# alexandrainst/coral

Hardware: AMD Instinct MI355X
Metric: audio-seconds/sec (CTC finetune step: fwd+bwd+allreduce+clip+AdamW), wav2vec2-large, 10 s utterances (higher is better)
Workload: dtype bf16; 1 GPU; wav2vec2-large (XLS-R shape d=1920 L=48 ffn=7680) CTC finetune, 8 x 10 s per GPU, SpecAugment on, activation_dropout 0.1, layerdrop 0 (multi-GPU rule), fp32 master + AdamW + clip 1.0; global_batch=8, frames_per_utt=499, parallelism=dp1

## Files before the change

### coral_amd/_lib.py

```python

from __future__ import annotations

import ctypes as C
import os
from pathlib import Path

_HERE = Path(__file__).resolve().parent
LIB_PATH = _HERE / "libcoral_amd.so"


class CoralAmdError(RuntimeError):
    """Raised when the HIP library is missing or a call into it fails."""


class CaGemmDesc(C.Structure):

    _fields_ = [
        ("A", C.c_void_p),
        ("B", C.c_void_p),
        ("C", C.c_void_p),
        ("C2", C.c_void_p),
        ("R", C.c_void_p),
        ("bias", C.c_void_p),
        ("M", C.c_int32),
# ... 18 lines not shown
        ("sC1", C.c_int64),
        ("sC2", C.c_int64),
        ("sR1", C.c_int64),
        ("sR2", C.c_int64),
        ("sBias1", C.c_int64),
        ("sBias2", C.c_int64),
        ("epilogue", C.c_int32),
        ("out_f32", C.c_int32),
        ("accumulate", C.c_int32),
        ("alpha", C.c_float),
        ("dropout_p", C.c_float),
        ("dropout_seed", C.c_uint64),
        ("a_colsum", C.c_void_p),
        ("a_colsum_ld", C.c_int64),
        ("c_row_index", C.c_void_p),
        ("c_row_mul", C.c_int64),
        ("c_split_n", C.c_int32),
        ("C_hi", C.c_void_p),
        ("ldc_hi", C.c_int64),
        ("a_scale", C.c_void_p),
        ("b_scale", C.c_void_p),
        ("a_row_scale", C.c_void_p),
        ("c_sumsq", C.c_void_p),
        ("c_stream_out", C.c_int32),
        ("C8", C.c_void_p),
        ("c8_scale", C.c_void_p),
        ("c8_amax", C.c_void_p),
        ("a_ln_gamma", C.c_void_p),
        ("a_ln_beta", C.c_void_p),
        ("a_ln_eps", C.c_float),
        ("xcd_balanced", C.c_int32),
    ]


class CaReduceDesc(C.Structure):
    _fields_ = [("partial", C.c_void_p), ("out", C.c_void_p), ("stride", C.c_int64), ("nparts", C.c_int32),
                ("n", C.c_int32), ("accumulate", C.c_int32)]


class CaDecodeLayer(C.Structure):

    FIELDS = ("ln1_g", "ln1_b", "wqkv", "bqkv", "wo", "bo", "ln2_g", "ln2_b", "wq2", "bq2", "wo2", "bo2", "ln3_g", "ln3_b",
              "w1", "b1", "w2", "b2", "self_kv", "cross_kv")
    _fields_ = [(n, C.c_void_p) for n in FIELDS]


class CaDecodeDesc(C.Structure):

    _fields_ = ([("layers", C.c_void_p)]
                + [(n, C.c_int32) for n in ("n_layers", "B", "d", "f", "H", "Te", "max_len", "V")]
                + [(n, C.c_void_p) for n in ("embed", "embed_pos", "lnf_g", "lnf_b")]
                + [("eps", C.c_float), ("logits", C.c_void_p), ("ld_logits", C.c_int64), ("suppress", C.c_void_p),
                   ("out", C.c_void_p), ("done", C.c_void_p), ("ids", C.c_void_p), ("ld_ids", C.c_int64),
                   ("tok", C.c_void_p), ("pos", C.c_void_p), ("klen", C.c_void_p), ("pad_id", C.c_int32),
                   ("eos_id", C.c_int32), ("ws", C.c_void_p), ("ws_bytes", C.c_int64), ("status", C.c_void_p),
                   ("cross_head_major", C.c_int32)])


DECODE_MAX_B = 16


def decode_ws_bytes(B, d, f, H, n_layers):
    return (8192 + n_layers * 16 * H * 4 + 16 * (7 * d + f) * 2 + 16 * H * 4 * 16 * 66 * 4 + 256 * 16 * 8 + 4096)


class CaAttnDesc(C.Structure):

    _fields_ = ([(n, C.c_void_p) for n in ("Q", "K", "V", "O", "dO", "dQ", "dK", "dV", "lse", "Dq", "klen", "key_slot", "kstart")]
                + [(n, C.c_int64) for n in ("ldq", "ldk", "ldv", "ldo", "lddo", "lddq", "lddk", "lddv",
                                             "sqb", "skb", "svb", "sob", "sdob", "sdqb", "sdkb", "sdvb")]
                + [(n, C.c_int32) for n in ("B", "H", "Tq", "Tk", "hd", "Tqp", "causal")]
                + [("scale", C.c_float), ("dropout_p", C.c_float), ("dropout_seed", C.c_uint64)]
                + [("O8", C.c_void_p), ("o8_scale", C.c_void_p), ("o8_amax", C.c_void_p),
                   ("split_ws", C.c_void_p), ("split_ws_bytes", C.c_int64), ("row_off", C.c_void_p)])


class CaFp8RefreshTask(C.Structure):

    _fields_ = ([(n, C.c_void_p) for n in ("x_bf16", "q_fp8", "q_fp8_t", "scale", "amax_next")]
                + [("rows", C.c_int32), ("cols", C.c_int32)])


class CaCtcBeamDesc(C.Structure):

    _fields_ = [("logits", C.c_void_p), ("ldv", C.c_int64), ("in_len", C.c_void_p),
                ("B", C.c_int32), ("T", C.c_int32), ("V", C.c_int32), ("blank", C.c_int32), ("delimiter", C.c_int32),
                ("forbidden", C.c_void_p), ("pfx_keys", C.c_void_p), ("pfx_wid", C.c_void_p), ("n_pfx", C.c_int64),
                ("ng_keys", C.c_void_p), ("ng_logp", C.c_void_p), ("ng_backoff", C.c_void_p),
                ("ng_count", C.c_int64 * 5),
                ("order", C.c_int32), ("bos_wid", C.c_int32), ("eos_wid", C.c_int32), ("unk_wid", C.c_int32),
                ("beam_width", C.c_int32),
                ("alpha", C.c_float), ("beta", C.c_float), ("unk_score_offset", C.c_float),
                ("token_min_logp", C.c_float), ("beam_prune_logp", C.c_float), ("score_boundary", C.c_int32),
                ("ids_out", C.c_void_p), ("out_len", C.c_void_p), ("score_out", C.c_void_p),
                ("ws", C.c_void_p), ("ws_bytes", C.c_int64)]


class CaBeamDesc(C.Structure):

    _fields_ = ([(n, C.c_int32) for n in ("B", "k", "max_len", "prompt_len", "max_length", "eos_id", "early_stopping")]
                + [(n, C.c_void_p) for n in ("len_pen", "cand_score", "cand_parent", "cand_token", "run_score", "tok", "pos",
                                              "klen", "anc_in", "anc_out", "ids_in", "ids_out", "fin_score", "fin_len",
                                              "fin_seq", "fin_ids", "fin_count", "heur", "done", "tr_parent", "tr_token",
                                              "tr_score")])


BEAM_MAX_BEAMS, BEAM_MAX_ROWS = 16, 128
ALIGN_MAX_TOKENS, ALIGN_MAX_FRAMES, ALIGN_MAX_HEADS, ALIGN_MAX_HEAD_DIM, ALIGN_MAX_FILTER_WIDTH = 447, 1500, 32, 128, 31


def align_ws_bytes_per_clip(A, Lw, Fmax):
    return A * Fmax * (Lw + 4) * 4


FP8_GROUP_MAX = 8
CTC_COLLAPSE_TILE = 4096
CTC_ALIGN_MAX_LABELS = 4095
KMAJOR, MNMAJOR = 0, 1
EPI_NONE, EPI_GELU, EPI_RESIDUAL, EPI_DGELU, EPI_GELU_RESIDUAL = 0, 1, 2, 3, 4

_vp, _i32, _i64, _f32, _u64 = C.c_void_p, C.c_int32, C.c_int64, C.c_float, C.c_uint64

SIGNATURES = {
    "ca_version": (C.c_int, []),
    "ca_last_error": (C.c_char_p, []),
    "ca_device_count": (C.c_int, []),
    "ca_gemm_bf16_group": (C.c_int, [_vp, _i32, _vp]),
    "ca_gemm_bf16": (C.c_int, [C.POINTER(CaGemmDesc), _vp]),
    "ca_gemm_fp8": (C.c_int, [C.POINTER(CaGemmDesc), _vp]),
    "ca_quantize_fp8": (C.c_int, [_vp, _i64, _vp, _vp, _vp, _vp]),
    "ca_quantize_fp8_delayed": (C.c_int, [_vp, _i64, _vp, _vp, _vp, _vp]),
    "ca_fp8_amax_rotate": (C.c_int, [_vp, _vp, _vp, _i32, _f32, _vp]),
    "ca_dropout_rows_fp8": (C.c_int, [_vp, _vp, _vp, _vp, _i64, _i32, _f32, _u64, _vp]),
    "ca_quantize_fp8_transposed": (C.c_int, [_vp, _i32, _i32, _vp, _vp, _vp]),
    "ca_fp8_refresh_group": (C.c_int, [_vp, _i32, _vp]),
    "ca_gemm_force_kernel": (C.c_int, [C.c_int]),
    "ca_gemm_debug_general_epilogue": (C.c_int, [C.c_int]),
    "ca_debug_cu_hog": (C.c_int, [_i32, _i32, _i32, C.c_double, _vp]),
    "ca_gemm_set_compute_cus": (C.c_int, [C.c_int]),
    "ca_background_update_fits": (C.c_int, [C.POINTER(C.c_int32)]),
    "ca_prof_begin": (C.c_int, []),
    "ca_prof_end": (C.c_int, [C.POINTER(C.c_double), C.POINTER(C.c_int64), C.POINTER(C.c_double)]),
    "ca_pack_rows": (C.c_int, [_vp, _vp, _vp, _i32, _i32, _i32, _i32, _vp]),
    "ca_unpack_rows": (C.c_int, [_vp, _vp, _vp, _i32, _i32, _i32, _i32, _vp]),
    "ca_attn_fwd": (C.c_int, [C.POINTER(CaAttnDesc), _vp]),
    "ca_attn_bwd": (C.c_int, [C.POINTER(CaAttnDesc), _vp]),
    "ca_decode_attn_qproj": (C.c_int, [C.POINTER(CaAttnDesc), _vp, _i64, _vp, _vp, _f32, _vp, _i64, _vp, _i32, _vp]),
    "ca_layernorm_fwd": (C.c_int, [_vp, _vp, _vp, _vp, _vp, _i64, _i32, _f32, _i32, _vp]),
    "ca_layernorm_fwd_ex": (C.c_int, [_vp, _vp, _vp, _vp, _vp, _i64, _i32, _f32, _i32, _i32, _i32, _vp]),
    "ca_layernorm_bwd_ex": (
        C.c_int,
        [_vp, _vp, _vp, _vp, _vp, _vp, _vp, _vp, _vp, _vp, _i64, _i32, _i32, _i32, _vp],
    ),
    "ca_layernorm_bwd_dropout": (
        C.c_int,
        [_vp, _vp, _vp, _vp, _vp, _vp, _vp, _vp, _f32, _u64, _vp, _vp, _vp, _i64, _i32, _i32, _vp],
    ),
    "ca_layernorm_fwd_fp8": (C.c_int, [_vp, _vp, _vp, _vp, _vp, _vp, _vp, _i64, _i32, _f32, _vp]),
    "ca_layernorm_bwd_partial_floats": (_i64, [_i64, _i32]),
    "ca_layernorm_bwd": (
        C.c_int,
        [_vp, _vp, _vp, _vp, _vp, _vp, _vp, _vp, _vp, _vp, _i64, _i32, _i32, _vp],
    ),
    "ca_colsum_partial_floats": (_i64, [_i64, _i32]),
    "ca_colsum_bf16": (C.c_int, [_vp, _i64, _i64, _i32, _vp, _vp, _i32, _vp, _vp]),
    "ca_dgelu_mul": (C.c_int, [_vp, _vp, _vp, _i64, _vp]),
    "ca_dropout_bf16": (C.c_int, [_vp, _vp, _i64, _f32, _u64, _vp]),
    "ca_reduce_rows_f32": (C.c_int, [_vp, _i32, _i64, _i32, _vp, _i32, _vp]),
    "ca_reduce_rows_multi": (C.c_int, [C.POINTER(CaReduceDesc), _i32, _vp]),
    "ca_wave_normalize": (C.c_int, [_vp, _vp, _vp, _i32, _i64, _f32, _vp]),
    "ca_frame_lengths": (C.c_int, [_vp, _i32, _i64, C.POINTER(C.c_int32), C.POINTER(C.c_int32), _i32, _vp, _vp]),
    "ca_wave_scale": (C.c_int, [_vp, _vp, _vp, _i32, _i64, _vp]),
    "ca_fir_filter": (C.c_int, [_vp, _vp, _vp, _vp, _vp, _i64, _i32, _vp, _i32, _i64, _vp]),
    "ca_mix_noise": (C.c_int, [_vp, _vp, _vp, _i64, _i64, _vp, _vp, _vp, _vp, _i32, _i64, _vp]),
    "ca_white_noise": (C.c_int, [_vp, _i64, C.c_uint64, _vp]),
    "ca_pcm_prepare": (C.c_int, [_vp, _i32, _i64, _vp, _vp, _vp, _i32, _i64, _i32, _i32, _f32, _vp]),
    "ca_conv0_ln_gelu_fwd": (
        C.c_int,
        [_vp, _vp, _vp, _vp, _vp, _vp, _i32, _i64, _i32, _i32, _i32, _f32, _vp],
    ),
    "ca_conv0_bwd_partial_floats": (_i64, [_i32, _i64, _i32, _i32, _i32]),
    "ca_conv0_ln_gelu_bwd": (
        C.c_int,
        [_vp] * 11 + [_i32, _i64, _i32, _i32, _i32, _f32, _vp],
    ),
    "ca_col2im_1d": (C.c_int, [_vp, _vp, _i32, _i64, _i64, _i32, _i32, _i32, _vp]),
    "ca_ctc_workspace_bytes": (_i64, [_i32, _i32, _i32]),
    "ca_ctc_loss_fwd_bwd": (
        C.c_int,
        [_vp, _vp, _vp, _vp, _vp, _vp, _vp, _i32, _i32, _i32, _i64, _i32, _i32, _i32, _vp],
    ),
    "ca_ctc_greedy_decode": (
        C.c_int,
        [_vp, _vp, _vp, _vp, _vp, _i32, _i32, _i32, _i64, _i32, _vp],
    ),
    "ca_ctc_stitch": (C.c_int, [_vp, _vp, _vp, _vp, _i32, _i32, _i32, _i64, _i32, _i32, _vp]),
    "ca_ctc_collapse_workspace_bytes": (_i64, [_i32, _i32]),
    "ca_ctc_collapse_offsets": (C.c_int, [_vp, _vp, _vp, _vp, _vp, _vp, _vp, _i64, _i32, _i32, _i32, _vp]),
    "ca_ctc_beam_workspace_bytes": (_i64, [_i32, _i32, _i32, _i32]),
    "ca_ctc_beam_decode": (C.c_int, [C.POINTER(CaCtcBeamDesc), _vp]),
    "ca_ctc_align_workspace_bytes": (_i64, [_i32, _i32, _i32]),
    "ca_ctc_align": (C.c_int, [_vp, _i64, _vp, _vp, _vp, _vp, _vp, _vp, _vp, _vp, _i64, _i32, _i32, _i32, _i32, _i32,
                               _vp]),
    "ca_beam_select_workspace_bytes": (_i64, [_i32, _i32, _i32]),
    "ca_beam_select": (C.c_int, [_vp, _i64, _vp, _vp, _i32, _i32, _i32, _vp, _vp, _vp, _vp, _i64, _vp]),
    "ca_beam_advance": (C.c_int, [C.POINTER(CaBeamDesc), _vp]),
    "ca_mask_frames": (C.c_int, [_vp, _vp, _vp, _vp, _vp, _i32, _i32, _i32, _vp]),
    "ca_regroup_pad": (C.c_int, [_vp, _vp, _i32, _i32, _i32, _i32, _i32, _vp]),
    "ca_posconv_partial_floats": (_i64, [_i32]),
    "ca_posconv_weight": (C.c_int, [_vp, _vp, _vp, _vp, _vp, _vp, _i32, _i32, _i32, _vp]),
    "ca_posconv_weight_bwd": (
        C.c_int,
        [_vp, _vp, _vp, _vp, _vp, _vp, _vp, _i32, _i32, _i32, _vp],
    ),
    "ca_cast_f32_bf16": (C.c_int, [_vp, _vp, _i64, _vp]),
    "ca_cast_bf16_f32": (C.c_int, [_vp, _vp, _i64, _vp]),
    "ca_transpose_f32_bf16": (C.c_int, [_vp, _vp, _i32, _i32, _vp]),
    "ca_conv_weight_reorder": (C.c_int, [_vp, _vp, _i32, _i32, _i32, _vp]),
    "ca_conv_weight_grad_reorder": (C.c_int, [_vp, _vp, _i32, _i32, _i32, _vp]),
    "ca_sumsq_f32": (C.c_int, [_vp, _i64, _vp, _i32, _vp, _vp]),
    "ca_sumsq_ranges_f32": (C.c_int, [_vp, _vp, _i32, _vp, _i32, _vp, _vp]),
    "ca_clear_ranges": (C.c_int, [_vp, _vp, _i32, _i64, _vp]),
    "ca_sum_f32": (C.c_int, [_vp, _i64, _vp, _i32, _vp, _vp]),
    "ca_adamw_step": (
        C.c_int,
        [_vp, _vp, _vp, _vp, _vp, _i64, _f32, _f32, _f32, _f32, _f32, _i32, _f32, _f32, _vp, _vp],
    ),
    "ca_adamw_step_ex": (
        C.c_int,
        [_vp, _vp, _vp, _vp, _vp, _i64, _f32, _f32, _f32, _f32, _f32, _i32, _f32, _f32, _vp, _i32, _vp],
    ),
    "ca_adamw_step_g16": (
        C.c_int,
        [_vp, _vp, _vp, _vp, _vp, _i64, _f32, _f32, _f32, _f32, _f32, _i32, _f32, _f32, _vp, _i32, _vp],
    ),
    "ca_logmel_workspace_bytes": (_i64, [_i32]),
    "ca_logmel": (C.c_int, [_vp, _vp, _vp, _vp, _i32, _i64, _i32, _vp]),
    "ca_cross_entropy_fwd_bwd": (
        C.c_int,
        [_vp, _vp, _vp, _vp, _vp, _i64, _i32, _i64, _i32, _vp],
    ),
    "ca_argmax_masked": (C.c_int, [_vp, _vp, _vp, _i64, _i32, _i64, _vp]),
    "ca_whisper_decode_token": (C.c_int, [C.POINTER(CaDecodeDesc), _vp]),
    "ca_whisper_decode_token_supported": (C.c_int, [_i32, _i32, _i32, _i32, _i32]),
    "ca_debug_decode_stamps": (C.c_int, [_vp, _i32]),
    "ca_argmax_advance": (C.c_int, [_vp, _vp, _vp, _i64, _i32, _i64, _vp, _vp, _i64, _vp, _vp, _vp, _i32, _i32, _vp]),
    "ca_argmax_timestamps": (C.c_int, [_vp, _vp, _vp, _i64, _i32, _i64, _vp, _i64, _vp, _i32, _i32, _i32, _i32, _vp]),
    "ca_argmax_timestamps_advance": (C.c_int, [_vp, _vp, _vp, _i64, _i32, _i64, _vp, _vp, _i64, _vp, _vp, _vp, _i32, _i32,
                                               _i32, _i32, _i32, _vp]),
    "ca_pick_scored_advance": (C.c_int, [_vp, _vp, _vp, _i64, _i32, _i64, _f32, _vp, _i64, _vp, _vp, _vp, _vp, _i64, _vp, _vp,
                                         _vp, _i32, _i32, _vp, _i32, _i32, _i32, _vp]),
    "ca_row_token_prob": (C.c_int, [_vp, _vp, _i64, _i32, _i64, _i32, _vp]),
    "ca_whisper_align_cost": (C.c_int, [_vp, C.POINTER(_vp), _i32, C.POINTER(_i32), _i32, _i32, _i32, _i32, _i32, _i32, _i64,
                                        _i64, _vp, _i32, _f32, _i32, _vp, _vp, _i64, _vp]),
    "ca_dtw_token_times": (C.c_int, [_vp, _i32, _i32, _vp, _i32, _vp, _vp, _vp, _vp, _vp, _vp]),
    "ca_embed_tokens": (C.c_int, [_vp, _vp, _vp, _vp, _vp, _i64, _i32, _vp]),
    "ca_embed_tokens_bwd": (C.c_int, [_vp, _vp, _vp, _vp, _vp, _i64, _i32, _vp]),
    "ca_comm_unique_id": (C.c_int, [_vp]),
    "ca_comm_init": (C.c_int, [C.POINTER(_vp), _vp, _i32, _i32]),
    "ca_comm_destroy": (C.c_int, [_vp]),
    "ca_comm_abort": (C.c_int, [_vp]),
    "ca_comm_stream": (_vp, [_vp]),
    "ca_comm_rank": (C.c_int, [_vp]),
    "ca_comm_world": (C.c_int, [_vp]),
    "ca_comm_after": (C.c_int, [_vp, _vp]),
    "ca_comm_before": (C.c_int, [_vp, _vp]),
    "ca_allreduce_bucket": (C.c_int, [_vp, _vp, _i64, _i32]),
    "ca_reduce_scatter_bucket": (C.c_int, [_vp, _vp, _i64, _i32]),
    "ca_allgather_bucket": (C.c_int, [_vp, _vp, _i64, _i32]),
}

_lib = None


def load() -> C.CDLL:
    global _lib
    if _lib is not None:
        return _lib
    path = Path(os.environ.get("CORAL_AMD_LIB", LIB_PATH))
    if not path.exists():
        raise CoralAmdError(
            f"{path} not found: build it with `python -c 'import __graft_entry__ as g; "
            "g.build()'` (or `make -C coral_amd/csrc`). There is no CPU fallback."
        )
    lib = C.CDLL(str(path))
    for name, (res, args) in SIGNATURES.items():
        fn = getattr(lib, name)
        fn.restype = res
        fn.argtypes = args
    _lib = lib
    return lib


def check(rc: int, what: str) -> None:
    if rc != 0:
        msg = load().ca_last_error()
        raise CoralAmdError(f"{what} failed ({rc}): {msg.decode() if msg else ''}")
```

### coral_amd/csrc/misc.hip

```cpp
#include "common.h"
#include <cstdlib>

__global__ __launch_bounds__(256) void mask_frames_kernel(unsigned short* __restrict__ h,
                                                          const uint8_t* __restrict__ tmask,
                                                          const uint8_t* __restrict__ fmask,
                                                          const unsigned short* __restrict__ embed,
                                                          const int32_t* __restrict__ flen, int B,
                                                          int T, int C) {
  const int cch = C >> 3;
  const int64_t total = (int64_t)B * T * cch;
  for (int64_t i = (int64_t)blockIdx.x * 256 + threadIdx.x; i < total;
       i += (int64_t)gridDim.x * 256) {
    const int c8 = (int)(i % cch);
    const int64_t bt = i / cch;
    const int t = (int)(bt % T), b = (int)(bt / T);
    const bool tm = tmask && tmask[bt];
    const bool pad = flen && t >= flen[b];
    bool anyf = false;
    if (fmask) {
#pragma unroll
      for (int e = 0; e < 8; ++e) anyf |= fmask[(int64_t)b * C + c8 * 8 + e] != 0;
    }
    if (!tm && !pad && !anyf) continue;
    unsigned short* p = h + bt * C + c8 * 8;
// ... 202 lines not shown
}

extern "C" int ca_posconv_weight_bwd(const float* dwf, const float* v, const float* g,
                                     const float* norm, float* dv, float* dg, float* partial,
                                     int32_t d, int32_t Cg, int32_t K, void* stream) {
  CA_CHECK_ARG(dwf && v && g && norm && dv && dg && partial, "ca_posconv_weight_bwd: null pointer");
  CA_CHECK_ARG(K > 0 && K <= 256 && (256 % K) == 0, "ca_posconv_weight_bwd: K must divide 256");
  hipStream_t s = (hipStream_t)stream;
  const int64_t nrows = (int64_t)d * Cg;
  float* dot = partial + (int64_t)PCW_SLABS * K;
  hipLaunchKernelGGL(tap_dot_kernel, dim3(PCW_SLABS), dim3(256), 0, s, v, dwf, partial, nrows, K,
                     1, Cg, d / Cg);
  hipLaunchKernelGGL(tap_finish_kernel, dim3((K + 15) / 16), dim3(256), 0, s, partial, PCW_SLABS, K, dot, 0);
  const size_t lds = (size_t)K * (Cg + 1) * sizeof(float);
  hipLaunchKernelGGL(posconv_wbwd_kernel, dim3(d), dim3(256), lds, s, dwf, v, g, norm, dot, dv,
                     Cg, K);
  hipLaunchKernelGGL(posconv_dg_kernel, dim3(1), dim3(256), 0, s, dot, norm, dg, K);
  CA_CHECK_LAUNCH("ca_posconv_weight_bwd");
  return CA_OK;
}

extern "C" int64_t ca_posconv_partial_floats(int32_t K) { return (int64_t)(PCW_SLABS + 1) * K; }

__global__ void cast_f32_bf16_kernel(const float* __restrict__ x, unsigned short* __restrict__ y,
                                     int64_t n) {
  const int64_t n4 = n >> 2;
  for (int64_t i = (int64_t)blockIdx.x * blockDim.x + threadIdx.x; i < n4;
       i += (int64_t)gridDim.x * blockDim.x) {
    const f32x4_t v = *(const f32x4_t*)(x + i * 4);
    *(u16x4_t*)(y + i * 4) = (u16x4_t){f2bf(v[0]), f2bf(v[1]), f2bf(v[2]), f2bf(v[3])};
  }
  if (blockIdx.x == 0 && threadIdx.x < (n & 3)) {
    const int64_t i = (n4 << 2) + threadIdx.x;
    y[i] = f2bf(x[i]);
  }
}
__global__ void cast_bf16_f32_kernel(const unsigned short* __restrict__ x, float* __restrict__ y,
                                     int64_t n) {
  for (int64_t i = (int64_t)blockIdx.x * blockDim.x + threadIdx.x; i < n;
       i += (int64_t)gridDim.x * blockDim.x)
    y[i] = bf2f(x[i]);
}
static int ew_grid(int64_t n, int per) {
  int64_t g = (n / per + 255) / 256;
  if (g > 8192) g = 8192;
  if (g < 1) g = 1;
  return (int)g;
}
extern "C" int ca_cast_f32_bf16(const float* x, void* y, int64_t n, void* stream) {
  CA_CHECK_ARG(x && y && n > 0, "ca_cast_f32_bf16: bad argument");
  CA_CHECK_ARG(((uintptr_t)x % 16) == 0 && ((uintptr_t)y % 8) == 0, "ca_cast_f32_bf16: alignment");
  hipLaunchKernelGGL(cast_f32_bf16_kernel, dim3(ew_grid(n, 4)), dim3(256), 0, (hipStream_t)stream,
                     x, (unsigned short*)y, n);
  CA_CHECK_LAUNCH("ca_cast_f32_bf16");
  return CA_OK;
}
extern "C" int ca_cast_bf16_f32(const void* x, float* y, int64_t n, void* stream) {
  CA_CHECK_ARG(x && y && n > 0, "ca_cast_bf16_f32: bad argument");
  hipLaunchKernelGGL(cast_bf16_f32_kernel, dim3(ew_grid(n, 1)), dim3(256), 0, (hipStream_t)stream,
                     (const unsigned short*)x, y, n);
  CA_CHECK_LAUNCH("ca_cast_bf16_f32");
  return CA_OK;
}

template <bool PACK>
__global__ __launch_bounds__(256) void pack_rows_kernel(const uint4* __restrict__ x, uint4* __restrict__ y,
                                                        const int32_t* __restrict__ row_off, int64_t total, int T, int CPR) {
  const int64_t i = (int64_t)blockIdx.x * 256 + threadIdx.x;
  if (i >= total) return;
  const int64_t row = i / CPR;
  const int ch = (int)(i - row * CPR);
  const int b = (int)(row / T), t = (int)(row - (int64_t)b * T);
  const int r0 = row_off[b];
  int len = row_off[b + 1] - r0;
  len = len < T ? len : T;
  const int64_t j = (int64_t)(r0 + t) * CPR + ch;
  if (PACK) {
    if (t < len) y[j] = x[i];
  } else {
    y[i] = t < len ? x[j] : make_uint4(0u, 0u, 0u, 0u);
  }
}
static int pack_rows_launch(bool pack, const void* x, void* y, const int32_t* row_off, int32_t B, int32_t T, int32_t C,
                            int32_t elt_bytes, void* stream, const char* who) {
  CA_CHECK_ARG(x && y && row_off && x != y && B > 0 && T > 0 && C > 0, "%s: bad argument", who);
  CA_CHECK_ARG(elt_bytes == 2 || elt_bytes == 4, "%s: rows of bf16 (2) or fp32 (4) elements", who);
  const int64_t row_bytes = (int64_t)C * elt_bytes;
  CA_CHECK_ARG((row_bytes % 16) == 0 && ((uintptr_t)x % 16) == 0 && ((uintptr_t)y % 16) == 0,
               "%s: rows must be multiples of 16 bytes, 16-byte aligned", who);
  const int cpr = (int)(row_bytes / 16);
  const int64_t total = (int64_t)B * T * cpr;
  const dim3 grid((unsigned)((total + 255) / 256));
  if (pack)
    hipLaunchKernelGGL(pack_rows_kernel<true>, grid, dim3(256), 0, (hipStream_t)stream, (const uint4*)x, (uint4*)y, row_off,
                       total, T, cpr);
  else
    hipLaunchKernelGGL(pack_rows_kernel<false>, grid, dim3(256), 0, (hipStream_t)stream, (const uint4*)x, (uint4*)y, row_off,
                       total, T, cpr);
  CA_CHECK_LAUNCH(who);
  return CA_OK;
}
extern "C" int ca_pack_rows(const void* x, void* y, const int32_t* row_off, int32_t B, int32_t T, int32_t C,
                            int32_t elt_bytes, void* stream) {
  return pack_rows_launch(true, x, y, row_off, B, T, C, elt_bytes, stream, "ca_pack_rows");
}
extern "C" int ca_unpack_rows(const void* x, void* y, const int32_t* row_off, int32_t B, int32_t T, int32_t C,
                              int32_t elt_bytes, void* stream) {
  return pack_rows_launch(false, x, y, row_off, B, T, C, elt_bytes, stream, "ca_unpack_rows");
}

__global__ __launch_bounds__(256) void transpose_f32_bf16_kernel(const float* __restrict__ x,
                                                                 unsigned short* __restrict__ y,
                                                                 int rows, int cols) {
  __shared__ float tile[32][33];
  const int c0 = blockIdx.x * 32, r0 = blockIdx.y * 32;
  const int tx = threadIdx.x & 31, ty = threadIdx.x >> 5;
  for (int k = ty; k < 32; k += 8) {
    const int r = r0 + k, c = c0 + tx;
    tile[k][tx] = (r < rows && c < cols) ? x[(int64_t)r * cols + c] : 0.f;
  }
  __syncthreads();
  for (int k = ty; k < 32; k += 8) {
    const int c = c0 + k, r = r0 + tx;
    if (c < cols && r < rows) y[(int64_t)c * rows + r] = f2bf(tile[tx][k]);
  }
}
extern "C" int ca_transpose_f32_bf16(const float* x, void* y, int32_t rows, int32_t cols,
                                     void* stream) {
  CA_CHECK_ARG(x && y && rows > 0 && cols > 0, "ca_transpose_f32_bf16: bad argument");
  hipLaunchKernelGGL(transpose_f32_bf16_kernel, dim3((cols + 31) / 32, (rows + 31) / 32),
                     dim3(256), 0, (hipStream_t)stream, x, (unsigned short*)y, rows, cols);
  CA_CHECK_LAUNCH("ca_transpose_f32_bf16");
  return CA_OK;
}

__global__ void conv_w_reorder_kernel(const float* __restrict__ w, unsigned short* __restrict__ wr,
                                      int64_t n, int Ci, int k) {
  for (int64_t i = (int64_t)blockIdx.x * blockDim.x + threadIdx.x; i < n;
       i += (int64_t)gridDim.x * blockDim.x) {
    const int ci = (int)(i % Ci);
    const int64_t r = i / Ci;
    const int j = (int)(r % k);
    const int64_t co = r / k;
    wr[i] = f2bf(w[(co * Ci + ci) * k + j]);
  }
}
extern "C" int ca_conv_weight_reorder(const float* w, void* wr, int32_t Co, int32_t Ci, int32_t k,
                                      void* stream) {
  CA_CHECK_ARG(w && wr && Co > 0 && Ci > 0 && k > 0, "ca_conv_weight_reorder: bad argument");
  const int64_t n = (int64_t)Co * Ci * k;
  hipLaunchKernelGGL(conv_w_reorder_kernel, dim3(ew_grid(n, 1)), dim3(256), 0,
                     (hipStream_t)stream, w, (unsigned short*)wr, n, Ci, k);
  CA_CHECK_LAUNCH("ca_conv_weight_reorder");
  return CA_OK;
}
__global__ void conv_w_grad_reorder_kernel(const float* __restrict__ dwr, float* __restrict__ dw,
                                           int64_t n, int Ci, int k) {
  for (int64_t i = (int64_t)blockIdx.x * blockDim.x + threadIdx.x; i < n;
       i += (int64_t)gridDim.x * blockDim.x) {
    const int ci = (int)(i % Ci);
    const int64_t r = i / Ci;
    const int j = (int)(r % k);
    const int64_t co = r / k;
    dw[(co * Ci + ci) * k + j] += dwr[i];
  }
}
extern "C" int ca_conv_weight_grad_reorder(const float* dwr, float* dw, int32_t Co, int32_t Ci,
                                           int32_t k, void* stream) {
  CA_CHECK_ARG(dwr && dw && Co > 0 && Ci > 0 && k > 0, "ca_conv_weight_grad_reorder: bad arg");
  const int64_t n = (int64_t)Co * Ci * k;
  hipLaunchKernelGGL(conv_w_grad_reorder_kernel, dim3(ew_grid(n, 1)), dim3(256), 0,
                     (hipStream_t)stream, dwr, dw, n, Ci, k);
  CA_CHECK_LAUNCH("ca_conv_weight_grad_reorder");
  return CA_OK;
}

__global__ __launch_bounds__(256) void clear_ranges_kernel(char* __restrict__ base, const int64_t* __restrict__ ranges,
                                                           int nranges) {
  for (int r = blockIdx.y; r < nranges; r += gridDim.y) {
    char* p = base + ranges[2 * r];
    const int64_t nb = ranges[2 * r + 1];
    int64_t head = (16 - ((uintptr_t)p & 15)) & 15;
    head = head < nb ? head : nb;
    const int64_t n16 = (nb - head) >> 4;
    const int64_t tail = nb - head - (n16 << 4);
    if (blockIdx.x == 0) {
      if ((int64_t)threadIdx.x * 4 < head) *(uint32_t*)(p + threadIdx.x * 4) = 0u;
      if ((int64_t)threadIdx.x * 4 < tail) *(uint32_t*)(p + head + (n16 << 4) + threadIdx.x * 4) = 0u;
    }
    uint4* q = (uint4*)(p + head);
    for (int64_t i = (int64_t)blockIdx.x * 256 + threadIdx.x; i < n16; i += (int64_t)gridDim.x * 256)
      q[i] = make_uint4(0, 0, 0, 0);
  }
}
extern "C" int ca_clear_ranges(void* base, const int64_t* ranges_bytes, int32_t nranges, int64_t max_bytes, void* stream) {
  CA_CHECK_ARG(base && ranges_bytes && nranges > 0 && max_bytes >= 0, "ca_clear_ranges: bad argument");
  int64_t gx = (max_bytes / 16 + 256 * 8 - 1) / (256 * 8);
  gx = gx < 1 ? 1 : (gx > 1024 ? 1024 : gx);
  const int gy = nranges < 1024 ? nranges : 1024;
  hipLaunchKernelGGL(clear_ranges_kernel, dim3((unsigned)gx, (unsigned)gy), dim3(256), 0, (hipStream_t)stream, (char*)base,
                     ranges_bytes, nranges);
  CA_CHECK_LAUNCH("ca_clear_ranges");
  return CA_OK;
}

#define SUMSQ_BLOCKS 1024
__global__ __launch_bounds__(256) void sumsq_kernel(const float* __restrict__ g, int64_t n,
                                                    float* __restrict__ partial) {
  __shared__ float red[4];
  float a = 0.f;
  const int64_t n4 = n >> 2;
  for (int64_t i = (int64_t)blockIdx.x * 256 + threadIdx.x; i < n4; i += (int64_t)gridDim.x * 256) {
    const f32x4_t v = *(const f32x4_t*)(g + i * 4);
    a += v[0] * v[0] + v[1] * v[1] + v[2] * v[2] + v[3] * v[3];
  }
  if (blockIdx.x == 0 && threadIdx.x < (n & 3)) {
    const float v = g[(n4 << 2) + threadIdx.x];
    a += v * v;
  }
  a = wave_sum(a);
  if ((threadIdx.x & 63) == 0) red[threadIdx.x >> 6] = a;
  __syncthreads();
  if (threadIdx.x == 0) partial[blockIdx.x] = red[0] + red[1] + red[2] + red[3];
}
__global__ __launch_bounds__(256) void sumsq_finish_kernel(const float* __restrict__ partial,
                                                           int nparts, float* __restrict__ out,
                                                           int accumulate) {
  __shared__ float red[4];
  float a = 0.f;
  for (int i = threadIdx.x; i < nparts; i += 256) a += partial[i];
  a = wave_sum(a);
  if ((threadIdx.x & 63) == 0) red[threadIdx.x >> 6] = a;
  __syncthreads();
  if (threadIdx.x == 0) {
    const float t = red[0] + red[1] + red[2] + red[3];
    out[0] = accumulate ? out[0] + t : t;
  }
}
extern "C" int ca_sumsq_f32(const float* g, int64_t n, float* out, int32_t accumulate,
                            float* partial, void* stream) {
  CA_CHECK_ARG(g && out && partial && n > 0, "ca_sumsq_f32: bad argument");
  CA_CHECK_ARG(((uintptr_t)g % 16) == 0, "ca_sumsq_f32: g must be 16-byte aligned");
  hipStream_t s = (hipStream_t)stream;
  hipLaunchKernelGGL(sumsq_kernel, dim3(SUMSQ_BLOCKS), dim3(256), 0, s, g, n, partial);
  hipLaunchKernelGGL(sumsq_finish_kernel, dim3(1), dim3(256), 0, s, partial, SUMSQ_BLOCKS, out,
                     accumulate);
  CA_CHECK_LAUNCH("ca_sumsq_f32");
  return CA_OK;
}

__global__ __launch_bounds__(256) void sumsq_chunks_kernel(const float* __restrict__ g, const int64_t* __restrict__ chunks,
                                                           int nchunks, float* __restrict__ partial) {
  __shared__ float red[4];
  for (int c = blockIdx.x; c < nchunks; c += gridDim.x) {
    const float* x = g + chunks[2 * c];
    const int64_t n = chunks[2 * c + 1];
    const int64_t n4 = n >> 2;
    float a = 0.f;
    for (int64_t i = threadIdx.x; i < n4; i += 256) {
      const f32x4_t v = *(const f32x4_t*)(x + i * 4);
      a += v[0] * v[0] + v[1] * v[1] + v[2] * v[2] + v[3] * v[3];
    }
    if (threadIdx.x < (n & 3)) {
      const float v = x[(n4 << 2) + threadIdx.x];
      a += v * v;
    }
    a = wave_sum(a);
    __syncthreads();
    if ((threadIdx.x & 63) == 0) red[threadIdx.x >> 6] = a;
    __syncthreads();
    if (threadIdx.x == 0) partial[c] = red[0] + red[1] + red[2] + red[3];
  }
}
extern "C" int ca_sumsq_ranges_f32(const float* g, const int64_t* chunks, int32_t nchunks, float* out,
                                   int32_t accumulate, float* partial, void* stream) {
  CA_CHECK_ARG(g && chunks && out && partial && nchunks > 0, "ca_sumsq_ranges_f32: bad argument");
  CA_CHECK_ARG(((uintptr_t)g % 16) == 0, "ca_sumsq_ranges_f32: g must be 16-byte aligned");
  hipStream_t s = (hipStream_t)stream;
  const int grid = nchunks < 2048 ? nchunks : 2048;
  hipLaunchKernelGGL(sumsq_chunks_kernel, dim3(grid), dim3(256), 0, s, g, chunks, nchunks, partial);
  hipLaunchKernelGGL(sumsq_finish_kernel, dim3(1), dim3(256), 0, s, partial, nchunks, out, accumulate);
  CA_CHECK_LAUNCH("ca_sumsq_ranges_f32");
  return CA_OK;
}
__global__ __launch_bounds__(256) void sum_kernel(const float* __restrict__ x, int64_t n, float* __restrict__ partial) {
  __shared__ float red[4];
  float a = 0.f;
  for (int64_t i = (int64_t)blockIdx.x * 256 + threadIdx.x; i < n; i += (int64_t)gridDim.x * 256) a += x[i];
  a = wave_sum(a);
  if ((threadIdx.x & 63) == 0) red[threadIdx.x >> 6] = a;
  __syncthreads();
  if (threadIdx.x == 0) partial[blockIdx.x] = red[0] + red[1] + red[2] + red[3];
}
extern "C" int ca_sum_f32(const float* x, int64_t n, float* out, int32_t accumulate, float* partial, void* stream) {
  CA_CHECK_ARG(x && out && partial && n > 0, "ca_sum_f32: bad argument");
  hipStream_t s = (hipStream_t)stream;
  const int grid = (int)((n + 255) / 256 < 256 ? (n + 255) / 256 : 256);
  hipLaunchKernelGGL(sum_kernel, dim3(grid), dim3(256), 0, s, x, n, partial);
  hipLaunchKernelGGL(sumsq_finish_kernel, dim3(1), dim3(256), 0, s, partial, grid, out, accumulate);
  CA_CHECK_LAUNCH("ca_sum_f32");
  return CA_OK;
}

template <bool NT, bool G16 = false>
__global__ __launch_bounds__(256) void adamw_kernel(float* __restrict__ p, float* __restrict__ m,
                                                    float* __restrict__ v,
// ... 182 lines not shown
```

### coral_amd/csrc/norm.hip

```cpp
#include "common.h"
#include <cstdlib>

#define LN_MAXCH 8

template <bool F32>
struct LnRow;
template <>
struct LnRow<false> {
  typedef u16x8_t V;
  static __device__ __forceinline__ V load(const void* base, int64_t idx) {
    return *(const u16x8_t*)((const unsigned short*)base + idx);
  }
  static __device__ __forceinline__ V zero() { return (u16x8_t){0, 0, 0, 0, 0, 0, 0, 0}; }
  static __device__ __forceinline__ float at(const V& v, int e) { return bf2f(v[e]); }
};
typedef __attribute__((ext_vector_type(8))) float f32x8_t;
template <>
struct LnRow<true> {
  typedef f32x8_t V;
  static __device__ __forceinline__ V load(const void* base, int64_t idx) {
    const f32x4_t a = *(const f32x4_t*)((const float*)base + idx), b = *(const f32x4_t*)((const float*)base + idx + 4);
    return (f32x8_t){a[0], a[1], a[2], a[3], b[0], b[1], b[2], b[3]};
  }
  static __device__ __forceinline__ V zero() { return (f32x8_t){0.f, 0.f, 0.f, 0.f, 0.f, 0.f, 0.f, 0.f}; }
// ... 123 lines not shown
    if (x_f32 && y_f32) LN_FWD_(N, true, true);    \
    else if (x_f32) LN_FWD_(N, true, false);       \
    else if (y_f32) LN_FWD_(N, false, true);       \
    else LN_FWD_(N, false, false);                 \
  } while (0)
#define LN_FWD(N) LN_FWD_(N, false, false)
  switch (nch) {
    case 1: LN_FWD_T(1); break;
    case 2: LN_FWD_T(2); break;
    case 3: LN_FWD(3); break;
    case 4: LN_FWD(4); break;
    default: LN_FWD(8); break;
  }
#undef LN_FWD
#undef LN_FWD_T
#undef LN_FWD_
  CA_CHECK_LAUNCH("ca_layernorm_fwd");
  return CA_OK;
}
extern "C" int ca_layernorm_fwd(const void* x, const float* gamma, const float* beta, void* y,
                                float* stats, int64_t rows, int32_t C, float eps, int32_t act,
                                void* stream) {
  return ca_layernorm_fwd_ex(x, gamma, beta, y, stats, rows, C, eps, act, 0, 0, stream);
}

template <int NCH>
__global__ __launch_bounds__(256) void ln_fwd_fp8_kernel(const unsigned short* __restrict__ x,
                                                         const float* __restrict__ gamma,
                                                         const float* __restrict__ beta,
                                                         unsigned short* __restrict__ y, unsigned int* __restrict__ q,
                                                         float* __restrict__ row_scale, float* __restrict__ stats,
                                                         int64_t rows, int C, float eps) {
  const int lane = threadIdx.x & 63;
  const int wave = threadIdx.x >> 6;
  const int nchunk = C >> 3;
  for (int64_t row = (int64_t)blockIdx.x * 4 + wave; row < rows; row += (int64_t)gridDim.x * 4) {
    const unsigned short* xr = x + row * C;
    float v[NCH][8];
    float s = 0.f;
#pragma unroll
    for (int c = 0; c < NCH; ++c) {
      const int ch = lane + c * 64;
      if (ch < nchunk) {
        const u16x8_t u = *(const u16x8_t*)(xr + ch * 8);
#pragma unroll
        for (int e = 0; e < 8; ++e) {
          v[c][e] = bf2f(u[e]);
          s += v[c][e];
        }
      } else {
#pragma unroll
        for (int e = 0; e < 8; ++e) v[c][e] = 0.f;
      }
    }
    const float mean = wave_sum(s) / (float)C;
    float s2 = 0.f;
#pragma unroll
    for (int c = 0; c < NCH; ++c) {
      const int ch = lane + c * 64;
      if (ch < nchunk) {
#pragma unroll
        for (int e = 0; e < 8; ++e) {
          const float dlt = v[c][e] - mean;
          s2 += dlt * dlt;
        }
      }
    }
    const float rstd = rsqrtf(wave_sum(s2) / (float)C + eps);
    if (lane == 0 && stats) {
      stats[row * 2] = mean;
      stats[row * 2 + 1] = rstd;
    }
    float am = 0.f;
#pragma unroll
    for (int c = 0; c < NCH; ++c) {
      const int ch = lane + c * 64;
      if (ch < nchunk) {
        const f32x4_t g0 = *(const f32x4_t*)(gamma + ch * 8);
        const f32x4_t g1 = *(const f32x4_t*)(gamma + ch * 8 + 4);
        const f32x4_t b0 = *(const f32x4_t*)(beta + ch * 8);
        const f32x4_t b1 = *(const f32x4_t*)(beta + ch * 8 + 4);
        u16x8_t o;
#pragma unroll
        for (int e = 0; e < 8; ++e) {
          o[e] = f2bf(ln_apply(v[c][e], mean, rstd, e < 4 ? g0[e] : g1[e - 4], e < 4 ? b0[e] : b1[e - 4]));
          v[c][e] = bf2f(o[e]);
          am = fmaxf(am, fabsf(v[c][e]));
        }
        if (y) *(u16x8_t*)(y + row * C + ch * 8) = o;
      }
    }
    am = wave_max(am);
    const float scale = am > 0.f ? 448.0f / am : 1.f;
    if (lane == 0) row_scale[row] = am > 0.f ? am / 448.0f : 1.f;
#pragma unroll
    for (int c = 0; c < NCH; ++c) {
      const int ch = lane + c * 64;
      if (ch < nchunk) {
        float t[8];
#pragma unroll
        for (int e = 0; e < 8; ++e) t[e] = fminf(fmaxf(v[c][e] * scale, -448.0f), 448.0f);
        unsigned int w0 = 0, w1 = 0;
        w0 = __builtin_amdgcn_cvt_pk_fp8_f32(t[0], t[1], w0, false);
        w0 = __builtin_amdgcn_cvt_pk_fp8_f32(t[2], t[3], w0, true);
        w1 = __builtin_amdgcn_cvt_pk_fp8_f32(t[4], t[5], w1, false);
        w1 = __builtin_amdgcn_cvt_pk_fp8_f32(t[6], t[7], w1, true);
        q[(row * C + ch * 8) / 4] = w0;
        q[(row * C + ch * 8) / 4 + 1] = w1;
      }
    }
  }
}

extern "C" int ca_layernorm_fwd_fp8(const void* x, const float* gamma, const float* beta, void* y, void* q_fp8,
                                    float* row_scale, float* stats, int64_t rows, int32_t C, float eps, void* stream) {
  CA_CHECK_ARG(x && gamma && beta && q_fp8 && row_scale, "ca_layernorm_fwd_fp8: null pointer");
  CA_CHECK_ARG(rows > 0 && C > 0 && (C % 16) == 0 && C <= LN_MAXCH * 512,
               "ca_layernorm_fwd_fp8: C=%d must be a multiple of 16 and <= %d", C, LN_MAXCH * 512);
  const int nch = (C / 8 + 63) / 64;
  dim3 grid(ln_grid(rows)), block(256);
  hipStream_t s = (hipStream_t)stream;
#define LN_FP8(N)                                                                                 \
  hipLaunchKernelGGL((ln_fwd_fp8_kernel<N>), grid, block, 0, s, (const unsigned short*)x, gamma, beta, \
                     (unsigned short*)y, (unsigned int*)q_fp8, row_scale, stats, rows, C, eps)
  switch (nch) {
    case 1: LN_FP8(1); break;
    case 2: LN_FP8(2); break;
    case 3: LN_FP8(3); break;
    case 4: LN_FP8(4); break;
    default: LN_FP8(8); break;
  }
#undef LN_FP8
  CA_CHECK_LAUNCH("ca_layernorm_fwd_fp8");
  return CA_OK;
}

static int ln_bwd_grid_max(int C) {
  static const int wide = [] { const char* e = getenv("CA_LN_BWD_GRID"); return e ? atoi(e) : 512; }();
  return C >= 1024 ? wide : 1024;
}
static int ln_bwd_grid(int64_t rows, int C) {
  int64_t g = (rows + 3) / 4;
  if (g > ln_bwd_grid_max(C)) g = ln_bwd_grid_max(C);
  if (g < 1) g = 1;
  return (int)g;
}

template <int NCH, bool ACT, bool DPP, bool XF32 = false, bool DROP = false>
__global__ __launch_bounds__(256, 2) void ln_bwd_kernel(
    const unsigned short* __restrict__ dy, const void* __restrict__ x,
    const float* __restrict__ gamma, const float* __restrict__ beta,
    const float* __restrict__ stats, const unsigned short* __restrict__ dres,
    unsigned short* __restrict__ dx, float* __restrict__ partial, int64_t rows, int C,
    unsigned short* __restrict__ dxd, float drop_p, uint64_t drop_seed) {
  extern __shared__ __attribute__((aligned(16))) char smem_raw[];
  float* red = (float*)smem_raw;
  const int lane = threadIdx.x & 63;
  const int wave = threadIdx.x >> 6;
  const int nchunk = C >> 3;
  float dg[NCH][8], db[NCH][8];
#pragma unroll
  for (int c = 0; c < NCH; ++c)
#pragma unroll
    for (int e = 0; e < 8; ++e) dg[c][e] = db[c][e] = 0.f;
  auto load_gamma = [&](int c, float (&g8)[8]) {
    const int ch = lane + c * 64;
    if (ch < nchunk) {
      const f32x4_t g0 = *(const f32x4_t*)(gamma + ch * 8), g1 = *(const f32x4_t*)(gamma + ch * 8 + 4);
#pragma unroll
      for (int e = 0; e < 8; ++e) g8[e] = e < 4 ? g0[e] : g1[e - 4];
    } else {
#pragma unroll
      for (int e = 0; e < 8; ++e) g8[e] = 0.f;
    }
  };
  auto load_beta = [&](int c, float (&b8)[8]) {
    const int ch = lane + c * 64;
#pragma unroll
    for (int e = 0; e < 8; ++e) b8[e] = 0.f;
    if (ACT && ch < nchunk) {
      const f32x4_t b0 = *(const f32x4_t*)(beta + ch * 8), b1 = *(const f32x4_t*)(beta + ch * 8 + 4);
#pragma unroll
      for (int e = 0; e < 8; ++e) b8[e] = e < 4 ? b0[e] : b1[e - 4];
    }
  };
  const int64_t stride = (int64_t)gridDim.x * 4;
  const u16x8_t zero8 = {0, 0, 0, 0, 0, 0, 0, 0};
  typedef LnRow<XF32> XR;
  typedef typename XR::V xv_t;
  xv_t cx[NCH];
  u16x8_t cd[NCH], cr[NCH];
  float cmean = 0.f, crstd = 0.f;
  auto request = [&](int64_t row, xv_t (&ux)[NCH], u16x8_t (&ud)[NCH], float& mean, float& rstd) {
    mean = stats[row * 2];
    rstd = stats[row * 2 + 1];
#pragma unroll
    for (int c = 0; c < NCH; ++c) {
      const int ch = lane + c * 64;
      ux[c] = XR::zero();
      ud[c] = zero8;
      if (ch < nchunk) {
        ux[c] = XR::load(x, row * C + ch * 8);
        ud[c] = *(const u16x8_t*)(dy + row * C + ch * 8);
      }
    }
  };
  constexpr bool PIPE = NCH <= 4;
  int64_t row = (int64_t)blockIdx.x * 4 + wave;
  if (PIPE && row < rows) request(row, cx, cd, cmean, crstd);
  while (row < rows) {
    const int64_t nrow = row + stride;
    if (!PIPE) request(row, cx, cd, cmean, crstd);
#pragma unroll
    for (int c = 0; c < NCH; ++c) {
      const int ch = lane + c * 64;
      cr[c] = zero8;
      if (dres && ch < nchunk) cr[c] = *(const u16x8_t*)(dres + row * C + ch * 8);
    }
    xv_t nx[PIPE ? NCH : 1];
    u16x8_t nd[PIPE ? NCH : 1];
    float nmean = 0.f, nrstd = 0.f;
    if constexpr (PIPE) {
      if (nrow < rows) request(nrow, nx, nd, nmean, nrstd);
    }
    float du_[ACT ? NCH : 1][8];
    float s1 = 0.f, s2 = 0.f;
#pragma unroll
    for (int c = 0; c < NCH; ++c) {
      float g8[8], b8[8];
      load_gamma(c, g8);
      load_beta(c, b8);
#pragma unroll
      for (int e = 0; e < 8; ++e) {
        const float h = (XR::at(cx[c], e) - cmean) * crstd;
        float du = bf2f(cd[c][e]);
        if (ACT) {
          du *= dgelu_erf(h * g8[e] + b8[e]);
          du_[ACT ? c : 0][e] = du;
        }
        dg[c][e] += du * h;
        db[c][e] += du;
        const float d = du * g8[e];
        s1 += d;
        s2 += d * h;
      }
    }
    const float m1 = (DPP ? wave_sum_dpp(s1) : wave_sum(s1)) / (float)C;
    const float m2 = (DPP ? wave_sum_dpp(s2) : wave_sum(s2)) / (float)C;
    unsigned short* dxr = dx + row * C;
#pragma unroll
    for (int c = 0; c < NCH; ++c) {
      const int ch = lane + c * 64;
      if (ch < nchunk) {
        u16x8_t o;
        float g8[8];
        load_gamma(c, g8);
#pragma unroll
        for (int e = 0; e < 8; ++e) {
          const float h = (XR::at(cx[c], e) - cmean) * crstd;
          const float du = ACT ? du_[ACT ? c : 0][e] : bf2f(cd[c][e]);
          o[e] = f2bf(crstd * (du * g8[e] - m1 - h * m2) + bf2f(cr[c][e]));
        }
        *(u16x8_t*)(dxr + ch * 8) = o;
        if constexpr (DROP) {
          const uint64_t i8 = (uint64_t)row * C + ch * 8;
          const unsigned int keep = ca_dropout_keep4(drop_seed, i8, drop_p) | (ca_dropout_keep4(drop_seed, i8 + 4, drop_p) << 4);
          const float ks = 1.f / (1.f - drop_p);
          u16x8_t od;
#pragma unroll
          for (int e = 0; e < 8; ++e) od[e] = ((keep >> e) & 1u) ? f2bf(bf2f(o[e]) * ks) : (unsigned short)0;
          *(u16x8_t*)(dxd + row * C + ch * 8) = od;
        }
      }
    }
    if constexpr (PIPE) {
#pragma unroll
      for (int c = 0; c < NCH; ++c) {
        cx[c] = nx[c];
        cd[c] = nd[c];
      }
      cmean = nmean;
      crstd = nrstd;
    }
    row = nrow;
  }
#pragma unroll
  for (int c = 0; c < NCH; ++c) {
    const int ch = lane + c * 64;
    if (ch < nchunk) {
#pragma unroll
      for (int e = 0; e < 8; ++e) {
        red[(wave * 2 + 0) * C + ch * 8 + e] = dg[c][e];
        red[(wave * 2 + 1) * C + ch * 8 + e] = db[c][e];
      }
    }
  }
  __syncthreads();
  float* pout = partial + (int64_t)blockIdx.x * 2 * C;
  for (int i = threadIdx.x; i < 2 * C; i += 256) {
    const int which = i / C, ch = i % C;
    float a = 0.f;
#pragma unroll
    for (int w = 0; w < 4; ++w) a += red[(w * 2 + which) * C + ch];
    pout[i] = a;
  }
}

__global__ __launch_bounds__(1024) void reduce_partials_kernel(const float* __restrict__ partial,
                                                               int nparts, int64_t stride, int n,
                                                               float* __restrict__ out,
                                                               int accumulate) {
  __shared__ float red[16][64];
  const int cl = threadIdx.x & 63, pl = threadIdx.x >> 6;
  const int i = blockIdx.x * 64 + cl;
  float a0 = 0.f, a1 = 0.f, a2 = 0.f, a3 = 0.f;
  if (i < n) {
    int p = pl;
    for (; p + 48 < nparts; p += 64) {
      a0 += partial[(int64_t)p * stride + i];
      a1 += partial[(int64_t)(p + 16) * stride + i];
      a2 += partial[(int64_t)(p + 32) * stride + i];
      a3 += partial[(int64_t)(p + 48) * stride + i];
    }
    for (; p < nparts; p += 16) a0 += partial[(int64_t)p * stride + i];
  }
  red[pl][cl] = (a0 + a1) + (a2 + a3);
  __syncthreads();
  if (pl == 0 && i < n) {
    float t = 0.f;
#pragma unroll
    for (int q = 0; q < 16; ++q) t += red[q][cl];
    out[i] = accumulate ? out[i] + t : t;
  }
}

__global__ __launch_bounds__(256) void reduce_few_parts_kernel(const float* __restrict__ partial, int nparts,
                                                               int64_t stride, int n, float* __restrict__ out,
                                                               int accumulate) {
  const int64_t i4 = ((int64_t)blockIdx.x * 256 + threadIdx.x) * 4;
  if (i4 >= n) return;
  if (i4 + 4 <= n) {
    f32x4_t acc = *(const f32x4_t*)(partial + i4);
    for (int p = 1; p < nparts; ++p) {
      const f32x4_t v = *(const f32x4_t*)(partial + (int64_t)p * stride + i4);
      acc[0] += v[0];
      acc[1] += v[1];
      acc[2] += v[2];
      acc[3] += v[3];
    }
    if (accumulate) {
      const f32x4_t o = *(const f32x4_t*)(out + i4);
      acc[0] += o[0];
      acc[1] += o[1];
      acc[2] += o[2];
      acc[3] += o[3];
    }
    *(f32x4_t*)(out + i4) = acc;
  } else {
    for (int64_t i = i4; i < n; ++i) {
      float a = partial[i];
      for (int p = 1; p < nparts; ++p) a += partial[(int64_t)p * stride + i];
      out[i] = accumulate ? out[i] + a : a;
    }
  }
}

void ca_reduce_partials_launch(const float* partial, int nparts, int64_t stride, int n, float* out,
                               int accumulate, hipStream_t s) {
  const bool aligned = ((uintptr_t)partial % 16) == 0 && ((uintptr_t)out % 16) == 0 && (stride % 4) == 0;
  if (nparts <= 16 && n >= 65536 && aligned) {
    hipLaunchKernelGGL(reduce_few_parts_kernel, dim3((unsigned)(((int64_t)n + 1023) / 1024)), dim3(256), 0, s, partial,
                       nparts, stride, n, out, accumulate);
    return;
  }
  hipLaunchKernelGGL(reduce_partials_kernel, dim3((n + 63) / 64), dim3(1024), 0, s, partial, nparts,
                     stride, n, out, accumulate);
}

extern "C" int64_t ca_layernorm_bwd_partial_floats(int64_t rows, int32_t C) {
  return (int64_t)ln_bwd_grid(rows, C) * 2 * C;
}

static int ln_bwd_launch(const void* dy, const void* x, const float* gamma, const float* beta, const float* stats,
                         const void* dres, void* dx, void* dxd, float drop_p, uint64_t drop_seed, float* dgamma,
                         float* dbeta, float* partial, int64_t rows, int32_t C, int32_t act, int32_t x_f32,
                         void* stream) {
  CA_CHECK_ARG(dy && x && gamma && stats && dx && partial, "ca_layernorm_bwd: null pointer");
  CA_CHECK_ARG(!x_f32 || C <= 1024, "ca_layernorm_bwd_ex: fp32 rows are served up to C = 1024 (C=%d)", C);
  CA_CHECK_ARG(!act || beta, "ca_layernorm_bwd: act needs beta");
  CA_CHECK_ARG(rows > 0 && C > 0 && (C % 8) == 0 && C <= LN_MAXCH * 512,
               "ca_layernorm_bwd: bad C=%d", C);
  const int nch = (C / 8 + 63) / 64;
  const int g = ln_bwd_grid(rows, C);
  dim3 grid(g), block(256);
  const size_t lds = (size_t)4 * 2 * C * sizeof(float);
  hipStream_t s = (hipStream_t)stream;
#define LN_BWD_(N, A, D, R)                                                                           \
  do {                                                                                                \
    if (x_f32 && N <= 2)                                                                              \
      hipLaunchKernelGGL((ln_bwd_kernel<(N <= 2 ? N : 1), A, D, true, R>), grid, block, lds, s,       \
                         (const unsigned short*)dy, x, gamma, beta, stats, (const unsigned short*)dres, \
                         (unsigned short*)dx, partial, rows, C, (unsigned short*)dxd, drop_p, drop_seed); \
    else                                                                                              \
      hipLaunchKernelGGL((ln_bwd_kernel<N, A, D, false, R>), grid, block, lds, s,                     \
                         (const unsigned short*)dy, x, gamma, beta, stats, (const unsigned short*)dres, \
                         (unsigned short*)dx, partial, rows, C, (unsigned short*)dxd, drop_p, drop_seed); \
  } while (0)
  static const int use_dpp = [] { const char* e = getenv("CA_LN_BWD_DPP"); return e ? atoi(e) : 1; }();
#define LN_BWD(N)                          \
  do {                                     \
    if (act)                               \
      LN_BWD_(N, true, true, false);       \
    else if (dxd && use_dpp)               \
      LN_BWD_(N, false, true, true);       \
    else if (dxd)                          \
      LN_BWD_(N, false, false, true);      \
    else if (use_dpp)                      \
      LN_BWD_(N, false, true, false);      \
    else                                   \
      LN_BWD_(N, false, false, false);     \
  } while (0)
  switch (nch) {
    case 1: LN_BWD(1); break;
    case 2: LN_BWD(2); break;
    case 3: LN_BWD(3); break;
    case 4: LN_BWD(4); break;
    default: LN_BWD(8); break;
  }
#undef LN_BWD
#undef LN_BWD_
  CA_CHECK_LAUNCH("ca_layernorm_bwd");
  if (dgamma && dbeta == dgamma + C) {
    ca_reduce_partials_launch(partial, g, (int64_t)2 * C, 2 * C, dgamma, 1, s);
  } else {
    if (dgamma) ca_reduce_partials_launch(partial, g, (int64_t)2 * C, C, dgamma, 1, s);
    if (dbeta) ca_reduce_partials_launch(partial + C, g, (int64_t)2 * C, C, dbeta, 1, s);
  }
  CA_CHECK_LAUNCH("ca_layernorm_bwd(reduce)");
  return CA_OK;
}
extern "C" int ca_layernorm_bwd_ex(const void* dy, const void* x, const float* gamma,
                                   const float* beta, const float* stats, const void* dres,
                                   void* dx, float* dgamma, float* dbeta, float* partial,
                                   int64_t rows, int32_t C, int32_t act, int32_t x_f32, void* stream) {
  return ln_bwd_launch(dy, x, gamma, beta, stats, dres, dx, nullptr, 0.f, 0, dgamma, dbeta, partial, rows, C, act, x_f32,
                       stream);
}
extern "C" int ca_layernorm_bwd(const void* dy, const void* x, const float* gamma,
                                const float* beta, const float* stats, const void* dres,
                                void* dx, float* dgamma, float* dbeta, float* partial,
                                int64_t rows, int32_t C, int32_t act, void* stream) {
  return ca_layernorm_bwd_ex(dy, x, gamma, beta, stats, dres, dx, dgamma, dbeta, partial, rows, C, act, 0, stream);
}
extern "C" int ca_layernorm_bwd_dropout(const void* dy, const void* x, const float* gamma, const float* beta,
                                        const float* stats, const void* dres, void* dx, void* dx_drop, float p,
                                        uint64_t seed, float* dgamma, float* dbeta, float* partial, int64_t rows,
                                        int32_t C, int32_t x_f32, void* stream) {
  CA_CHECK_ARG(dx_drop != nullptr && dx_drop != dx, "ca_layernorm_bwd_dropout: dx_drop must be its own buffer");
  CA_CHECK_ARG(p >= 0.f && p < 1.f, "ca_layernorm_bwd_dropout: bad p");
  return ln_bwd_launch(dy, x, gamma, beta, stats, dres, dx, dx_drop, p, seed, dgamma, dbeta, partial, rows, C, 0, x_f32,
                       stream);
}

#define CS_SLAB_MAX 512
static int cs_slabs(int64_t rows) {
  int64_t s = (rows + 63) / 64;
  if (s > CS_SLAB_MAX) s = CS_SLAB_MAX;
  if (s < 1) s = 1;
  return (int)s;
}
__global__ __launch_bounds__(256) void colsum_kernel(const unsigned short* __restrict__ x,
                                                     int64_t ld, int64_t rows, int N,
                                                     const uint8_t* __restrict__ rowmask,
                                                     float* __restrict__ partial) {
  __shared__ float red[8][256 + 8];
  const int cl = threadIdx.x & 31, rl = threadIdx.x >> 5;
  const int col = (blockIdx.x * 32 + cl) * 8;
  const int nslab = gridDim.y;
  const int64_t per = (rows + nslab - 1) / nslab;
  const int64_t r0 = (int64_t)blockIdx.y * per;
  int64_t r1 = r0 + per;
  if (r1 > rows) r1 = rows;
  float a[8] = {0.f, 0.f, 0.f, 0.f, 0.f, 0.f, 0.f, 0.f};
  if (col < N) {
    int64_t r = r0 + rl;
    for (; r + 24 < r1; r += 32) {
      u16x8_t u[4];
#pragma unroll
      for (int k = 0; k < 4; ++k) {
        const bool on = !rowmask || rowmask[r + 8 * k];
        u[k] = on ? *(const u16x8_t*)(x + (r + 8 * k) * ld + col) : (u16x8_t){0, 0, 0, 0, 0, 0, 0, 0};
      }
#pragma unroll
      for (int k = 0; k < 4; ++k)
#pragma unroll
        for (int e = 0; e < 8; ++e) a[e] += bf2f(u[k][e]);
    }
    for (; r < r1; r += 8) {
      if (rowmask && !rowmask[r]) continue;
      const u16x8_t u = *(const u16x8_t*)(x + r * ld + col);
#pragma unroll
      for (int e = 0; e < 8; ++e) a[e] += bf2f(u[e]);
    }
  }
#pragma unroll
  for (int e = 0; e < 8; ++e) red[rl][cl * 8 + e] = a[e];
  __syncthreads();
  const int c = threadIdx.x;
  const int gc = blockIdx.x * 256 + c;
  if (gc < N) {
    float t = 0.f;
#pragma unroll
    for (int r = 0; r < 8; ++r) t += red[r][c];
    partial[(int64_t)blockIdx.y * N + gc] = t;
  }
}

extern "C" int64_t ca_colsum_partial_floats(int64_t rows, int32_t N) {
  return (int64_t)cs_slabs(rows) * N;
}

extern "C" int ca_colsum_bf16(const void* x, int64_t ld, int64_t rows, int32_t N,
                              const uint8_t* rowmask, float* out, int32_t accumulate,
                              float* partial, void* stream) {
  CA_CHECK_ARG(x && out && partial, "ca_colsum_bf16: null pointer");
  CA_CHECK_ARG(rows > 0 && N > 0 && (N % 8) == 0 && (ld % 8) == 0,
               "ca_colsum_bf16: N and ld must be multiples of 8");
  const int ns = cs_slabs(rows);
  hipStream_t s = (hipStream_t)stream;
  hipLaunchKernelGGL(colsum_kernel, dim3((N + 255) / 256, ns), dim3(256), 0, s,
                     (const unsigned short*)x, ld, rows, N, rowmask, partial);
  ca_reduce_partials_launch(partial, ns, (int64_t)N, N, out, accumulate, s);
  CA_CHECK_LAUNCH("ca_colsum_bf16");
  return CA_OK;
}

__global__ void dgelu_mul_kernel(const unsigned short* __restrict__ dy,
                                 const unsigned short* __restrict__ u,
                                 unsigned short* __restrict__ out, int64_t n8) {
  for (int64_t i = (int64_t)blockIdx.x * blockDim.x + threadIdx.x; i < n8;
       i += (int64_t)gridDim.x * blockDim.x) {
    const u16x8_t a = *(const u16x8_t*)(dy + i * 8);
    const u16x8_t b = *(const u16x8_t*)(u + i * 8);
    u16x8_t o;
#pragma unroll
    for (int e = 0; e < 8; ++e) o[e] = f2bf(bf2f(a[e]) * dgelu_erf(bf2f(b[e])));
    *(u16x8_t*)(out + i * 8) = o;
  }
}
extern "C" int ca_dgelu_mul(const void* dy, const void* u, void* out, int64_t n, void* stream) {
  CA_CHECK_ARG(dy && u && out && n > 0 && (n % 8) == 0, "ca_dgelu_mul: n must be a multiple of 8");
  int64_t g = (n / 8 + 255) / 256;
  if (g > 8192) g = 8192;
  hipLaunchKernelGGL(dgelu_mul_kernel, dim3((int)g), dim3(256), 0, (hipStream_t)stream,
                     (const unsigned short*)dy, (const unsigned short*)u, (unsigned short*)out,
                     n / 8);
  CA_CHECK_LAUNCH("ca_dgelu_mul");
  return CA_OK;
}

__global__ void dropout_bf16_kernel(const unsigned short* __restrict__ x, unsigned short* __restrict__ y, int64_t n8,
                                    float p, uint64_t seed) {
  const float ks = 1.f / (1.f - p);
  for (int64_t i = (int64_t)blockIdx.x * blockDim.x + threadIdx.x; i < n8; i += (int64_t)gridDim.x * blockDim.x) {
    const u16x8_t a = *(const u16x8_t*)(x + i * 8);
    const unsigned int keep = ca_dropout_keep4(seed, (uint64_t)i * 8, p) | (ca_dropout_keep4(seed, (uint64_t)i * 8 + 4, p) << 4);
    u16x8_t o;
#pragma unroll
    for (int e = 0; e < 8; ++e) o[e] = ((keep >> e) & 1u) ? f2bf(bf2f(a[e]) * ks) : (unsigned short)0;
    *(u16x8_t*)(y + i * 8) = o;
  }
}
extern "C" int ca_dropout_bf16(const void* x, void* y, int64_t n, float p, uint64_t seed, void* stream) {
  CA_CHECK_ARG(x && y && n > 0 && (n % 8) == 0, "ca_dropout_bf16: n must be a positive multiple of 8");
  CA_CHECK_ARG(p >= 0.f && p < 1.f, "ca_dropout_bf16: bad p");
  int64_t g = (n / 8 + 255) / 256;
  if (g > 8192) g = 8192;
  hipLaunchKernelGGL(dropout_bf16_kernel, dim3((int)g), dim3(256), 0, (hipStream_t)stream, (const unsigned short*)x,
                     (unsigned short*)y, n / 8, p, seed);
  CA_CHECK_LAUNCH("ca_dropout_bf16");
  return CA_OK;
}

struct ReduceMulti {
  CaReduceDesc d[CA_REDUCE_MAX];
  int first[CA_REDUCE_MAX + 1];
  int count;
};
__global__ __launch_bounds__(1024) void reduce_partials_multi_kernel(const ReduceMulti m) {
  __shared__ float red[16][64];
  int which = 0;
#pragma unroll
  for (int i = 1; i < CA_REDUCE_MAX; ++i)
    if (i < m.count && (int)blockIdx.x >= m.first[i]) which = i;
  const CaReduceDesc d = m.d[which];
  const int cl = threadIdx.x & 63, pl = threadIdx.x >> 6;
  const int i = ((int)blockIdx.x - m.first[which]) * 64 + cl;
  float a0 = 0.f, a1 = 0.f, a2 = 0.f, a3 = 0.f;
  if (i < d.n) {
    int p = pl;
    for (; p + 48 < d.nparts; p += 64) {
      a0 += d.partial[(int64_t)p * d.stride + i];
      a1 += d.partial[(int64_t)(p + 16) * d.stride + i];
      a2 += d.partial[(int64_t)(p + 32) * d.stride + i];
      a3 += d.partial[(int64_t)(p + 48) * d.stride + i];
    }
    for (; p < d.nparts; p += 16) a0 += d.partial[(int64_t)p * d.stride + i];
  }
  red[pl][cl] = (a0 + a1) + (a2 + a3);
  __syncthreads();
  if (pl == 0 && i < d.n) {
    float t = 0.f;
#pragma unroll
    for (int q = 0; q < 16; ++q) t += red[q][cl];
    d.out[i] = d.accumulate ? d.out[i] + t : t;
  }
}
extern "C" int ca_reduce_rows_multi(const CaReduceDesc* descs, int32_t count, void* stream) {
  CA_CHECK_ARG(descs && count >= 1 && count <= CA_REDUCE_MAX, "ca_reduce_rows_multi: 1..%d reductions", CA_REDUCE_MAX);
  ReduceMulti m;
  int blocks = 0;
  for (int i = 0; i < count; ++i) {
    CA_CHECK_ARG(descs[i].partial && descs[i].out && descs[i].nparts > 0 && descs[i].n > 0 && descs[i].stride >= descs[i].n,
                 "ca_reduce_rows_multi: bad reduction %d", i);
    m.d[i] = descs[i];
    m.first[i] = blocks;
    blocks += (descs[i].n + 63) / 64;
  }
  for (int i = count; i < CA_REDUCE_MAX; ++i) {
    m.d[i] = descs[0];
    m.first[i] = blocks;
  }
  m.first[CA_REDUCE_MAX] = blocks;
  m.count = count;
  hipLaunchKernelGGL(reduce_partials_multi_kernel, dim3(blocks), dim3(1024), 0, (hipStream_t)stream, m);
  CA_CHECK_LAUNCH("ca_reduce_rows_multi");
  return CA_OK;
}

extern "C" int ca_reduce_rows_f32(const float* partial, int32_t nparts, int64_t stride, int32_t n, float* out,
                                  int32_t accumulate, void* stream) {
  CA_CHECK_ARG(partial && out && nparts > 0 && n > 0 && stride >= n, "ca_reduce_rows_f32: bad argument");
  ca_reduce_partials_launch(partial, nparts, stride, n, out, accumulate, (hipStream_t)stream);
  CA_CHECK_LAUNCH("ca_reduce_rows_f32");
  return CA_OK;
}
```

### coral_amd/ops.py

```python

from __future__ import annotations

import ctypes as C
import os

import torch

from . import _lib
from ._lib import (CaAttnDesc, EPI_DGELU, EPI_GELU, EPI_GELU_RESIDUAL, EPI_NONE, EPI_RESIDUAL, KMAJOR,
                   MNMAJOR, CaGemmDesc, CoralAmdError, check)

__all__ = ["KMAJOR", "MNMAJOR", "EPI_NONE", "EPI_GELU", "EPI_RESIDUAL", "EPI_DGELU",
           "EPI_GELU_RESIDUAL", "CoralAmdError"]

_ELT = {torch.bfloat16: 2, torch.float32: 4, torch.int32: 4, torch.uint8: 1, torch.int64: 8, torch.int16: 2,
        torch.uint32: 4}


def _stream() -> int:
    return torch.cuda.current_stream().cuda_stream


def _p(t: torch.Tensor | None, off: int = 0) -> int | None:
    if t is None:
# ... 159 lines not shown
    if g16 and accumulate:
        raise CoralAmdError("wgrad_gemm: a bf16 gradient buffer is written, never accumulated into")
    if bias_off is not None:
        colsum(dY, lda, K, M, Gb if g16 else G, part, x_off=a_off, out_off=bias_off)
    if splits == 1:
        kw = dict(a_colsum=cs[0], a_colsum_off=cs[1], a_colsum_ld=cs[2]) if cs is not None else {}
        if sq is not None:
            kw.update(c_sumsq=sq[0], c_sumsq_off=sq[1])
        gemm(dY, X, G, M=M, N=N, K=K, a_layout=MNMAJOR, lda=lda, b_layout=MNMAJOR, ldb=ldb, ldc=N, c_off=c_off,
             a_off=a_off, b_off=b_off, out_f32=not g16, accumulate=accumulate, stream_out=STREAM_WGRAD, **kw)
        return
    ws = _SPLITK_WS.get(G.device)
    need = max(splits * M * N, M * N + 4096)
    if ws is None or ws.numel() < need:
        ws = torch.empty(need, dtype=torch.float32, device=G.device)
        _SPLITK_WS[G.device] = ws
    Kc = K // splits
    gemm(dY, X, ws, M=M, N=N, K=Kc, a_layout=MNMAJOR, lda=lda, b_layout=MNMAJOR, ldb=ldb, ldc=N, a_off=a_off,
         b_off=b_off, out_f32=True, batch2=splits, sA=(0, Kc * lda), sB=(0, Kc * ldb), sC=(0, M * N))
    if g16:
        reduce_rows(ws, splits, M * N, M * N, ws, accumulate=False)
        cast_f32_bf16(ws, G, M * N, y_off=c_off)
        if sq is not None:
            cast_bf16_f32(G[c_off:], ws, M * N)
            sumsq(ws, M * N, sq[0][sq[1]:], ws[M * N:])
    else:
        reduce_rows(ws, splits, M * N, M * N, G[c_off:], accumulate=accumulate)
        if sq is not None:
            sumsq(G[c_off:], M * N, sq[0][sq[1]:], ws)
    if sq is not None:
        ns = sumsq_slots(M, N)
        if ns > 1:
            clear_f32(sq[0], ns - 1, off=sq[1] + 1)


def _xtiles(p):
    return ((p["M"] + 255) // 256) * ((p["N"] + 255) // 256)


def _fill(t):
    return t / (256.0 * ((t + 255) // 256))


GROUP_MAX = 8


_PLAN_CACHE: dict = {}
_CS_DIRTY: dict = {}


def _wgrad_plan_idx(shapes: tuple):
    import itertools

    xt = [((m + 255) // 256) * ((n + 255) // 256) for m, n, _ in shapes]
    big = [i for i, (_, _, k) in enumerate(shapes) if _fill(xt[i]) >= 0.85 and k >= 512]
    rest = [i for i in range(len(shapes)) if i not in big and shapes[i][2] >= 512]
    small_k = [i for i in range(len(shapes)) if i not in big and shapes[i][2] < 512]
    groups = []
    if 1 < len(rest) <= GROUP_MAX and _fill(sum(xt[i] for i in rest)) >= 0.6:
        groups.append(list(rest))
        rest = []
    while len(rest) > 1:
        best, best_fill = None, 0.0
        for r in range(min(GROUP_MAX, len(rest)), 1, -1):
            for combo in itertools.combinations(rest, r):
                total = sum(xt[i] for i in combo)
                alone = sum(xt[i] / _fill(xt[i]) for i in combo)
                f = _fill(total)
                if f >= 0.7 and total / f < 0.9 * alone and (f > best_fill + 1e-9 or (abs(f - best_fill) < 1e-9 and best is not None
                                                                                 and len(combo) > len(best))):
                    best, best_fill = combo, f
        if best is None:
            break
        groups.append(list(best))
        rest = [i for i in rest if i not in best]
    return big, groups, rest + small_k


def wgrad_plan(problems: list):
    key = tuple((p["M"], p["N"], p["K"]) for p in problems)
    plan = _PLAN_CACHE.get(key)
    if plan is None:
        if len(_PLAN_CACHE) > 4096:
            _PLAN_CACHE.clear()
        plan = _PLAN_CACHE[key] = _wgrad_plan_idx(key)
    solo, groups, fallback = plan
    return [problems[i] for i in solo], [[problems[i] for i in g] for g in groups], [problems[i] for i in fallback]


def wgrad_gemm_group(problems: list, G, colsum_ws=None, colsum_ld=0, Gb=None) -> bool:
    solo, groups, fallback = wgrad_plan(problems)
    fused = (FUSE_BIAS_GRAD and colsum_ws is not None and bool(solo or groups) and all("cs_off" in p for p in problems)
             and (not fallback or min(p["K"] for p in problems) >= FUSE_BIAS_PARTIAL_MIN_K))

    def bias_kw(p):
        return dict(cs=(colsum_ws, p["cs_off"], colsum_ld)) if fused else dict(bias_off=p.get("bias_off"), part=p.get("part"))

    def base(p):
        return {k: p[k] for k in ("M", "N", "K", "lda", "ldb", "c_off", "accumulate", "sq") if p.get(k) is not None or k != "sq"}

    dirty = _CS_DIRTY.setdefault(colsum_ws.data_ptr(), set()) if fused else None
    g16 = G.dtype == torch.bfloat16
    Gbias = Gb if g16 else G
    for p in solo:
        wgrad_gemm(p["dY"], p["X"], G, **base(p), **bias_kw(p), Gb=Gbias)
        if fused:
            dirty.add((p["cs_off"], p["M"]))
    for p in fallback:
        if fused:
            key = (p["cs_off"], p["M"])
            if key in dirty:
                clear_ranges(colsum_ws, tuple((r * colsum_ld + p["cs_off"], p["M"]) for r in range(1, COLSUM_PARTS)))
                dirty.discard(key)
            colsum(p["dY"], p["lda"], p["K"], p["M"], colsum_ws, p["part"], accumulate=False, out_off=p["cs_off"])
            wgrad_gemm(p["dY"], p["X"], G, **base(p), Gb=Gbias)
        else:
            wgrad_gemm(p["dY"], p["X"], G, **base(p), **bias_kw(p), Gb=Gbias)
    for chunk in groups:
        arr = (CaGemmDesc * len(chunk))()
        for i, p in enumerate(chunk):
            if not fused and p.get("bias_off") is not None:
                colsum(p["dY"], p["lda"], p["K"], p["M"], Gbias, p["part"], out_off=p["bias_off"])
            kw = dict(a_colsum=colsum_ws, a_colsum_off=p["cs_off"], a_colsum_ld=colsum_ld) if fused else {}
            if p.get("sq") is not None:
                kw.update(c_sumsq=p["sq"][0], c_sumsq_off=p["sq"][1])
            arr[i] = _gemm_desc(p["dY"], p["X"], G, M=p["M"], N=p["N"], K=p["K"], a_layout=MNMAJOR, lda=p["lda"],
                                b_layout=MNMAJOR, ldb=p["ldb"], ldc=p["N"], c_off=p["c_off"], out_f32=not g16,
                                accumulate=p["accumulate"], stream_out=STREAM_WGRAD, **kw)
        check(lib().ca_gemm_bf16_group(arr, len(chunk), _stream()), "ca_gemm_bf16_group")
        if fused:
            dirty.update((p["cs_off"], p["M"]) for p in chunk)
    return fused


def layernorm_fwd(x, gamma, beta, y, stats, rows, Cn, eps=1e-5, act=0, x_off=0, y_off=0):
    xf, yf = x.dtype == torch.float32, y.dtype == torch.float32
    if xf or yf:
        check(lib().ca_layernorm_fwd_ex(_p(x, x_off), _p(gamma), _p(beta), _p(y, y_off), _p(stats), rows, Cn, eps, act,
                                        int(xf), int(yf), _stream()), "ca_layernorm_fwd_ex")
        return
    check(lib().ca_layernorm_fwd(_p(x, x_off), _p(gamma), _p(beta), _p(y, y_off), _p(stats), rows,
                                 Cn, eps, act, _stream()), "ca_layernorm_fwd")


def layernorm_fwd_fp8(x, gamma, beta, y, q, row_scale, rows, Cn, eps=1e-5, stats=None):
    check(lib().ca_layernorm_fwd_fp8(_p(x), _p(gamma), _p(beta), _p(y), _p(q), _p(row_scale), _p(stats), rows, Cn, eps,
                                     _stream()), "ca_layernorm_fwd_fp8")


def layernorm_bwd_partial_floats(rows, Cn):
    return lib().ca_layernorm_bwd_partial_floats(rows, Cn)


def layernorm_bwd(dy, x, gamma, beta, stats, dres, dx, dgamma, dbeta, partial, rows, Cn, act=0):
    if x.dtype == torch.float32:
        check(lib().ca_layernorm_bwd_ex(_p(dy), _p(x), _p(gamma), _p(beta), _p(stats), _p(dres), _p(dx), _p(dgamma),
                                        _p(dbeta), _p(partial), rows, Cn, act, 1, _stream()), "ca_layernorm_bwd_ex")
        return
    check(lib().ca_layernorm_bwd(_p(dy), _p(x), _p(gamma), _p(beta), _p(stats), _p(dres), _p(dx),
                                 _p(dgamma), _p(dbeta), _p(partial), rows, Cn, act, _stream()),
          "ca_layernorm_bwd")


def layernorm_bwd_dropout(dy, x, gamma, beta, stats, dres, dx, dx_drop, p, seed, dgamma, dbeta, partial, rows, Cn):
    check(lib().ca_layernorm_bwd_dropout(_p(dy), _p(x), _p(gamma), _p(beta), _p(stats), _p(dres), _p(dx), _p(dx_drop),
                                         float(p), int(seed), _p(dgamma), _p(dbeta), _p(partial), rows, Cn,
                                         int(x.dtype == torch.float32), _stream()), "ca_layernorm_bwd_dropout")


def colsum_partial_floats(rows, N):
    return lib().ca_colsum_partial_floats(rows, N)


def colsum(x, ld, rows, N, out, partial, accumulate=True, rowmask=None, x_off=0, out_off=0):
    check(lib().ca_colsum_bf16(_p(x, x_off), ld, rows, N, _p(rowmask), _p(out, out_off),
                               int(accumulate), _p(partial), _stream()), "ca_colsum_bf16")


def reduce_rows(partial, nparts, stride, n, out, accumulate=False):
    check(lib().ca_reduce_rows_f32(_p(partial), nparts, stride, n, _p(out), int(accumulate), _stream()),
          "ca_reduce_rows_f32")


def reduce_rows_multi(items):
    from ._lib import CaReduceDesc

    arr = (CaReduceDesc * len(items))()
    for k, (partial, nparts, stride, n, out, accumulate) in enumerate(items):
        arr[k].partial, arr[k].out = _p(partial), _p(out)
        arr[k].stride, arr[k].nparts, arr[k].n, arr[k].accumulate = stride, nparts, n, int(accumulate)
    check(lib().ca_reduce_rows_multi(arr, len(items), _stream()), "ca_reduce_rows_multi")


def dgelu_mul(dy, u, out, n):
    check(lib().ca_dgelu_mul(_p(dy), _p(u), _p(out), n, _stream()), "ca_dgelu_mul")


def dropout(x, y, n, p, seed):
    check(lib().ca_dropout_bf16(_p(x), _p(y), n, float(p), int(seed), _stream()), "ca_dropout_bf16")


def wave_normalize(x, lengths, y, B, N, eps=1e-7):
    check(lib().ca_wave_normalize(_p(x), _p(lengths), _p(y), B, N, eps, _stream()),
          "ca_wave_normalize")


def frame_lengths(attention_mask, kernels, strides, out):
    B, N = attention_mask.shape
    n = len(kernels)
    k = (C.c_int32 * n)(*kernels)
    s = (C.c_int32 * n)(*strides)
    check(lib().ca_frame_lengths(_p(attention_mask), B, N, k, s, n, _p(out), _stream()), "ca_frame_lengths")


def pcm_prepare(pcm, lengths, y, mask, B, N, ld_in, peak_normalize=False, zero_mean_unit_var=True, eps=1e-7):
    if pcm.dtype not in (torch.int16, torch.float32):
        raise CoralAmdError("pcm_prepare: PCM must be int16 or float32")
    check(lib().ca_pcm_prepare(_p(pcm), int(pcm.dtype == torch.int16), ld_in, _p(lengths), _p(y), _p(mask), B, N,
                               int(peak_normalize), int(zero_mean_unit_var), eps, _stream()), "ca_pcm_prepare")


def wave_scale(x, scale, y, B, N):
    check(lib().ca_wave_scale(_p(x), _p(scale), _p(y), B, N, _stream()), "ca_wave_scale")


def fir_filter(x, lengths, taps, ntaps, mode, y, B, N, max_taps):
    check(lib().ca_fir_filter(_p(x), _p(lengths), _p(taps), _p(ntaps), _p(mode), taps.shape[1], max_taps, _p(y), B, N,
                              _stream()), "ca_fir_filter")


def mix_noise(x, lengths, noise, noise_ld, noise_len, noise_off, snr_db, active, y, B, N):
    check(lib().ca_mix_noise(_p(x), _p(lengths), _p(noise), noise_ld, noise_len, _p(noise_off), _p(snr_db), _p(active),
                             _p(y), B, N, _stream()), "ca_mix_noise")


def white_noise(out, n, seed):
    check(lib().ca_white_noise(_p(out), n, seed, _stream()), "ca_white_noise")


def conv0_fwd(x, w, bias, gamma, beta, y, B, N, Cn, k, stride, eps=1e-5):
    check(lib().ca_conv0_ln_gelu_fwd(_p(x), _p(w), _p(bias), _p(gamma), _p(beta), _p(y), B, N, Cn,
                                     k, stride, eps, _stream()), "ca_conv0_ln_gelu_fwd")


def conv0_bwd_partial_floats(B, N, Cn, k, stride):
    return lib().ca_conv0_bwd_partial_floats(B, N, Cn, k, stride)


def conv0_bwd(x, w, bias, gamma, beta, dy, dw, dbias, dgamma, dbeta, partial, B, N, Cn, k,
              stride, eps=1e-5):
    check(lib().ca_conv0_ln_gelu_bwd(_p(x), _p(w), _p(bias), _p(gamma), _p(beta), _p(dy), _p(dw),
                                     _p(dbias), _p(dgamma), _p(dbeta), _p(partial), B, N, Cn, k,
                                     stride, eps, _stream()), "ca_conv0_ln_gelu_bwd")


def col2im_1d(dcol, dx, B, T, L, Cn, k, stride):
    check(lib().ca_col2im_1d(_p(dcol), _p(dx), B, T, L, Cn, k, stride, _stream()), "ca_col2im_1d")


def ctc_workspace_bytes(B, T, Lmax):
    return lib().ca_ctc_workspace_bytes(B, T, Lmax)


def ctc_loss_fwd_bwd(logits, labels, in_len, nll, grad, gscale, ws, B, T, V, ldv, Lmax, blank,
                     zero_infinity=True):
    check(lib().ca_ctc_loss_fwd_bwd(_p(logits), _p(labels), _p(in_len), _p(nll), _p(grad),
                                    _p(gscale), _p(ws), B, T, V, ldv, Lmax, blank,
                                    int(zero_infinity), _stream()), "ca_ctc_loss_fwd_bwd")


def ctc_greedy_decode(logits, in_len, raw, ids, out_len, B, T, V, ldv, blank):
    check(lib().ca_ctc_greedy_decode(_p(logits), _p(in_len), _p(raw), _p(ids), _p(out_len), B, T,
                                     V, ldv, blank, _stream()), "ca_ctc_greedy_decode")


def ctc_stitch(logits, seg, raw_out, logits_out, C_, T, V, ldv, R, Tout):
    check(lib().ca_ctc_stitch(_p(logits), _p(seg), _p(raw_out), _p(logits_out), C_, T, V, ldv, R, Tout, _stream()),
          "ca_ctc_stitch")


def ctc_collapse_workspace_bytes(B, T):
    return lib().ca_ctc_collapse_workspace_bytes(B, T)


def ctc_collapse_offsets(raw, in_len, ids, start, end, out_len, ws, B, T, blank):
    check(lib().ca_ctc_collapse_offsets(_p(raw), _p(in_len), _p(ids), _p(start), _p(end), _p(out_len), _p(ws),
                                        ws.numel() * _ELT[ws.dtype], B, T, blank, _stream()), "ca_ctc_collapse_offsets")


def ctc_beam_workspace_bytes(B, T, V, beam_width):
    return lib().ca_ctc_beam_workspace_bytes(B, T, V, beam_width)


def ctc_beam_decode(logits, in_len, ids_out, out_len, score_out, ws, B, T, V, ldv, blank, delimiter, forbidden=None,
                    tables=None, beam_width=100, alpha=0.5, beta=1.5, unk_score_offset=-10.0, token_min_logp=-5.0,
                    beam_prune_logp=-10.0, score_boundary=True):
    d = _lib.CaCtcBeamDesc()
    d.logits, d.ldv, d.in_len = _p(logits), ldv, _p(in_len)
    d.B, d.T, d.V, d.blank, d.delimiter = B, T, V, blank, delimiter
    d.forbidden = _p(forbidden)
    if tables is not None:
        d.pfx_keys, d.pfx_wid, d.n_pfx = _p(tables["pfx_keys"]), _p(tables["pfx_wid"]), tables["pfx_keys"].numel()
        d.ng_keys, d.ng_logp, d.ng_backoff = _p(tables["ng_keys"]), _p(tables["ng_logp"]), _p(tables["ng_backoff"])
        for k, n in enumerate(tables["ng_count"]):
            d.ng_count[k] = n
        d.order, d.bos_wid, d.eos_wid, d.unk_wid = tables["order"], tables["bos_wid"], tables["eos_wid"], tables["unk_wid"]
    else:
        d.order, d.bos_wid, d.eos_wid, d.unk_wid = 0, -1, -1, -1
    d.beam_width = beam_width
    d.alpha, d.beta, d.unk_score_offset = alpha, beta, unk_score_offset
    d.token_min_logp, d.beam_prune_logp, d.score_boundary = token_min_logp, beam_prune_logp, int(bool(score_boundary))
    d.ids_out, d.out_len, d.score_out = _p(ids_out), _p(out_len), _p(score_out)
    d.ws, d.ws_bytes = _p(ws), ws.numel() * _ELT[ws.dtype]
    check(lib().ca_ctc_beam_decode(C.byref(d), _stream()), "ca_ctc_beam_decode")


def ctc_align_workspace_bytes(B, T, Lmax):
    return lib().ca_ctc_align_workspace_bytes(B, T, Lmax)


def ctc_align(logits, in_len, labels, lab_len, start, end, tok_score, score, ws, B, T, V, ldv, Lmax, blank):
    labels = torch.as_tensor(labels, dtype=torch.int32).reshape(B, Lmax)
    lab_len = torch.as_tensor(lab_len, dtype=torch.int32).reshape(B)
    if labels.is_cuda or lab_len.is_cuda:
        raise ValueError("ctc_align: labels and lab_len are host tensors (their values are checked on the host)")
    if Lmax > _lib.CTC_ALIGN_MAX_LABELS:
        raise ValueError(f"ctc_align: {Lmax} labels per row, the limit is {_lib.CTC_ALIGN_MAX_LABELS}")
    if B and (int(lab_len.min()) < 0 or int(lab_len.max()) > Lmax):
        raise ValueError(f"ctc_align: lab_len must lie in [0, Lmax = {Lmax}]")
    used = labels[torch.arange(Lmax)[None, :] < lab_len[:, None]]
    if used.numel() and (int(used.min()) < 0 or int(used.max()) >= V or bool((used == blank).any())):
        raise ValueError(f"ctc_align: labels must lie in [0, {V}) and differ from the blank id {blank}")
    dev = logits.device
    lab_d, len_d = labels.contiguous().to(dev), lab_len.to(dev)
    check(lib().ca_ctc_align(_p(logits), ldv, _p(in_len), _p(lab_d), _p(len_d), _p(start), _p(end), _p(tok_score),
                             _p(score), _p(ws), ws.numel() * _ELT[ws.dtype], B, T, V, Lmax, blank, _stream()),
          "ca_ctc_align")


def mask_frames(h, tmask, fmask, embed, flen, B, T, Cn):
    check(lib().ca_mask_frames(_p(h), _p(tmask), _p(fmask), _p(embed), _p(flen), B, T, Cn,
                               _stream()), "ca_mask_frames")


def regroup_pad(x, xg, B, T, G, Cg, pad):
    check(lib().ca_regroup_pad(_p(x), _p(xg), B, T, G, Cg, pad, _stream()), "ca_regroup_pad")


def posconv_partial_floats(K):
    return lib().ca_posconv_partial_floats(K)


def posconv_weight(v, g, wf, wb, norm, partial, d, Cg, K):
    check(lib().ca_posconv_weight(_p(v), _p(g), _p(wf), _p(wb), _p(norm), _p(partial), d, Cg, K,
                                  _stream()), "ca_posconv_weight")


def posconv_weight_bwd(dwf, v, g, norm, dv, dg, partial, d, Cg, K):
    check(lib().ca_posconv_weight_bwd(_p(dwf), _p(v), _p(g), _p(norm), _p(dv), _p(dg),
                                      _p(partial), d, Cg, K, _stream()), "ca_posconv_weight_bwd")


def cast_f32_bf16(x, y, n, x_off=0, y_off=0):
    check(lib().ca_cast_f32_bf16(_p(x, x_off), _p(y, y_off), n, _stream()), "ca_cast_f32_bf16")


def pack_rows(x, y, row_off, B, T, Cn):
    if x.dtype != y.dtype:
        raise CoralAmdError("pack_rows: x and y must have the same dtype")
    check(lib().ca_pack_rows(_p(x), _p(y), _p(row_off), B, T, Cn, _ELT[x.dtype], _stream()), "ca_pack_rows")


def unpack_rows(x, y, row_off, B, T, Cn):
    if x.dtype != y.dtype:
        raise CoralAmdError("unpack_rows: x and y must have the same dtype")
    check(lib().ca_unpack_rows(_p(x), _p(y), _p(row_off), B, T, Cn, _ELT[x.dtype], _stream()), "ca_unpack_rows")


def cast_bf16_f32(x, y, n):
    check(lib().ca_cast_bf16_f32(_p(x), _p(y), n, _stream()), "ca_cast_bf16_f32")


def transpose_f32_bf16(x, y, rows, cols):
    check(lib().ca_transpose_f32_bf16(_p(x), _p(y), rows, cols, _stream()), "ca_transpose_f32_bf16")


def conv_weight_reorder(w, wr, Co, Ci, k, w_off=0):
    check(lib().ca_conv_weight_reorder(_p(w, w_off), _p(wr), Co, Ci, k, _stream()),
          "ca_conv_weight_reorder")


def conv_weight_grad_reorder(dwr, dw, Co, Ci, k, dw_off=0):
    check(lib().ca_conv_weight_grad_reorder(_p(dwr), _p(dw, dw_off), Co, Ci, k, _stream()),
          "ca_conv_weight_grad_reorder")


def clear_f32(x, n, off=0):
    clear_ranges(x, [(off, n)])


_CLEAR_TABLES: dict = {}


def clear_ranges(x, ranges):
    elt = _ELT[x.dtype]
    key = (x.data_ptr(), elt, tuple(ranges))
    ent = _CLEAR_TABLES.get(key)
    if ent is None:
        if len(_CLEAR_TABLES) > 4096:
            torch.cuda.synchronize()
            _CLEAR_TABLES.clear()
        rows = [[int(a) * elt, int(n) * elt] for a, n in ranges if n > 0]
        if any(a % 4 or n % 4 for a, n in rows):
            raise CoralAmdError("clear_ranges: ranges must be multiples of 4 bytes")
        big = [r for r in rows if r[1] >= (1 << 20)]
        small = [r for r in rows if r[1] < (1 << 20)]
        ent = tuple((torch.tensor(part, dtype=torch.int64, device=x.device), len(part), max(n for _, n in part))
                    for part in (big, small) if part)
        _CLEAR_TABLES[key] = ent
    for table, count, longest in ent:
        check(lib().ca_clear_ranges(_p(x), _p(table), count, longest, _stream()), "ca_clear_ranges")


def sumsq(g, n, out, partial, accumulate=False):
    check(lib().ca_sumsq_f32(_p(g), n, _p(out), int(accumulate), _p(partial), _stream()),
          "ca_sumsq_f32")


def sumsq_ranges(g, chunks, nchunks, out, partial, accumulate=False):
    check(lib().ca_sumsq_ranges_f32(_p(g), _p(chunks), nchunks, _p(out), int(accumulate), _p(partial), _stream()),
          "ca_sumsq_ranges_f32")


def sum_f32(x, n, out, partial, accumulate=False):
    check(lib().ca_sum_f32(_p(x), n, _p(out), int(accumulate), _p(partial), _stream()), "ca_sum_f32")


def adamw_step(p, m, v, g, p16, n, lr, beta1, beta2, eps, weight_decay, step, grad_scale=1.0,
               max_norm=0.0, gnorm_sq=None, max_blocks=0):
    fn = lib().ca_adamw_step_g16 if g.dtype == torch.bfloat16 else lib().ca_adamw_step_ex
    check(fn(_p(p), _p(m), _p(v), _p(g), _p(p16), n, lr, beta1, beta2, eps,
             weight_decay, step, grad_scale, max_norm, _p(gnorm_sq), int(max_blocks), _stream()),
          "ca_adamw_step")


def logmel_workspace_bytes(B):
    return lib().ca_logmel_workspace_bytes(B)


def logmel(wave, mel_filters, out, ws, B, N, n_mels):
    check(lib().ca_logmel(_p(wave), _p(mel_filters), _p(out), _p(ws), B, N, n_mels, _stream()),
          "ca_logmel")


def cross_entropy_fwd_bwd(logits, labels, loss_sum, count, grad, rows, V, ldv, ignore_index=-100):
    check(lib().ca_cross_entropy_fwd_bwd(_p(logits), _p(labels), _p(loss_sum), _p(count), _p(grad),
                                         rows, V, ldv, ignore_index, _stream()),
          "ca_cross_entropy_fwd_bwd")


def argmax_masked(logits, suppress, out, rows, V, ldv):
    check(lib().ca_argmax_masked(_p(logits), _p(suppress), _p(out), rows, V, ldv, _stream()),
          "ca_argmax_masked")


def argmax_advance(logits, suppress, out, rows, V, ldv, done, ids, tok, pos, klen, pad_id, eos_id):
    if done.dtype != torch.bool or ids.dtype != torch.int64 or ids.dim() != 2 or ids.stride(1) != 1:
        raise CoralAmdError("argmax_advance: done must be bool, ids a row-major int64 matrix")
    check(lib().ca_argmax_advance(_p(logits), _p(suppress), _p(out), rows, V, ldv, done.data_ptr(), _p(ids), ids.stride(0),
                                  _p(tok), _p(pos), _p(klen), int(pad_id), int(eos_id), _stream()), "ca_argmax_advance")


def _cap(max_initial_timestamp_index):
    return -1 if max_initial_timestamp_index is None else int(max_initial_timestamp_index)


def argmax_timestamps(logits, suppress, out, rows, V, ldv, ids, pos, begin_index, timestamp_begin, eos_id,
                      max_initial_timestamp_index=None):
    if ids.dtype != torch.int64 or ids.dim() != 2 or ids.stride(1) != 1 or pos.dtype != torch.int32:
        raise CoralAmdError("argmax_timestamps: ids must be a row-major int64 matrix, pos int32")
    check(lib().ca_argmax_timestamps(_p(logits), _p(suppress), _p(out), rows, V, ldv, _p(ids), ids.stride(0), _p(pos),
                                     int(begin_index), int(timestamp_begin), int(eos_id),
                                     _cap(max_initial_timestamp_index), _stream()), "ca_argmax_timestamps")


def argmax_timestamps_advance(logits, suppress, out, rows, V, ldv, done, ids, tok, pos, klen, pad_id, eos_id, begin_index,
                              timestamp_begin, max_initial_timestamp_index=None):
    if done.dtype != torch.bool or ids.dtype != torch.int64 or ids.dim() != 2 or ids.stride(1) != 1:
        raise CoralAmdError("argmax_timestamps_advance: done must be bool, ids a row-major int64 matrix")
    check(lib().ca_argmax_timestamps_advance(_p(logits), _p(suppress), _p(out), rows, V, ldv, done.data_ptr(), _p(ids),
                                             ids.stride(0), _p(tok), _p(pos), _p(klen), int(pad_id), int(eos_id),
                                             int(begin_index), int(timestamp_begin), _cap(max_initial_timestamp_index),
                                             _stream()), "ca_argmax_timestamps_advance")


def pick_scored_advance(logits, suppress, out, rows, V, ldv, inv_temperature, uniforms, sum_logprob, n_scored, done, ids, tok,
                        pos, klen, pad_id, eos_id, timestamps=None):
    if done.dtype != torch.bool or ids.dtype != torch.int64 or ids.dim() != 2 or ids.stride(1) != 1:
        raise CoralAmdError("pick_scored_advance: done must be bool, ids a row-major int64 matrix")
    if sum_logprob.dtype != torch.float32 or n_scored.dtype != torch.int32 or pos.dtype != torch.int32:
        raise CoralAmdError("pick_scored_advance: sum_logprob must be float32, n_scored and pos int32")
    ld_u = 0
    if inv_temperature > 0:
        if uniforms is None or uniforms.dtype != torch.float32 or uniforms.dim() != 2 or uniforms.stride(1) != 1 \
                or uniforms.shape[0] < rows:
            raise CoralAmdError("pick_scored_advance: sampling needs uniforms, a row-major float32 matrix [rows, length]")
        ld_u = uniforms.stride(0)
    begin, tb, cap = timestamps if timestamps is not None else (0, 0, None)
    check(lib().ca_pick_scored_advance(_p(logits), _p(suppress), _p(out), rows, V, ldv, float(inv_temperature), _p(uniforms),
                                       ld_u, _p(sum_logprob), _p(n_scored), done.data_ptr(), _p(ids), ids.stride(0), _p(tok),
                                       _p(pos), _p(klen), int(pad_id), int(eos_id),
                                       _p(ids) if timestamps is not None else None, int(begin), int(tb), _cap(cap), _stream()),
          "ca_pick_scored_advance")


def row_token_prob(logits, out, rows, V, ldv, token):
    check(lib().ca_row_token_prob(_p(logits), _p(out), rows, V, ldv, int(token), _stream()), "ca_row_token_prob")


ALIGN_WS_CAP_BYTES = 64 << 20


def whisper_align_cost(q, cross_k, layer_head, B, Lw, Te, H, hd, ldk, skb, frames, Fmax, scale, filter_width,
                       ws_cap_bytes=None):
    from .whisper_align import check_align_limits

    A = len(layer_head)
    check_align_limits(A, Lw, Fmax, hd, Te, filter_width)
    if q.dtype != torch.bfloat16 or not q.is_contiguous() or q.numel() != A * B * Lw * hd:
        raise CoralAmdError("whisper_align_cost: q must be a contiguous bf16 [A, B, Lw, hd]")
    if frames.dtype != torch.int32 or frames.numel() != B or any(k.dtype != torch.bfloat16 for k in cross_k):
        raise CoralAmdError("whisper_align_cost: frames must be int32 [B], the keys bf16")
    per_clip = _lib.align_ws_bytes_per_clip(A, Lw, Fmax)
    cap = ALIGN_WS_CAP_BYTES if ws_cap_bytes is None else int(ws_cap_bytes)
    nbytes = per_clip * max(1, min(B, cap // per_clip))
    ws = torch.empty(nbytes, dtype=torch.uint8, device=q.device)
    cost = torch.empty(B, Lw, Fmax, dtype=torch.float32, device=q.device)
    kptr = (C.c_void_p * len(cross_k))(*[_p(k) for k in cross_k])
    lh = (C.c_int32 * (2 * A))(*[int(v) for pair in layer_head for v in pair])
    check(lib().ca_whisper_align_cost(_p(q), kptr, len(cross_k), lh, A, B, Lw, Te, H, hd, ldk, skb, _p(frames), Fmax,
                                      float(scale), int(filter_width), _p(cost), _p(ws), nbytes, _stream()),
          "ca_whisper_align_cost")
    return cost

# ... 120 lines not shown
```

### coral_amd/stem_blocks.py

```python

from __future__ import annotations

import torch

from . import ops
from .blocks import layernorm_bwd
from .ops import EPI_GELU_RESIDUAL, EPI_RESIDUAL, MNMAJOR

F32 = torch.float32


class ConvScratch:

    def __init__(self, z, B, wgrad, dgrad, part):
        nw = max(c.Co * c.k * c.Ci for c in wgrad)
        self.dwr_part, self.dwr = z(B * nw, F32), z(nw, F32)
        self.dcol = z(max(B * c.T * c.k * c.Ci for c in dgrad))
        self.part = part


class StridedConvBlock:

    def __init__(self, store, weight: str, bias: str, Ci: int, Co: int, k: int, stride: int, rows_in=None, rows_out=None,
                 y_off: int = 0):
        self.st, self.Ci, self.Co, self.k, self.stride, self.y_off = store, Ci, Co, k, stride, y_off
        self.w_off, self.b_off = store.off(weight), store.off(bias)
        self.wr = torch.zeros(Co * k * Ci, dtype=torch.bfloat16, device=store.device)
        if rows_in is not None:
            self.set_rows(rows_in, rows_out)

    def set_rows(self, rows_in: int, rows_out=None):
        self.rows_in = rows_in
        self.T = (rows_in - self.k) // self.stride + 1
        self.rows_out = self.T if rows_out is None else rows_out
        assert self.y_off + self.T <= self.rows_out

    def refresh(self):
        ops.conv_weight_reorder(self.st.p32, self.wr, self.Co, self.Ci, self.k, w_off=self.w_off)

    def forward(self, x, y, B, **epilogue):
        Ci, Co, k = self.Ci, self.Co, self.k
        ops.gemm(x, self.wr, y, c_off=self.y_off * Co, M=self.T, N=Co, K=k * Ci, lda=self.stride * Ci, ldb=k * Ci, ldc=Co,
                 bias=self.st.p32, bias_off=self.b_off, batch2=B, sA=(0, self.rows_in * Ci), sC=(0, self.rows_out * Co),
                 **epilogue)

    def backward(self, dy, x, B, sc: ConvScratch, dx=None):
        Ci, Co, k, T = self.Ci, self.Co, self.k, self.T
        g32, nw = self.st.g32, Co * k * Ci
        clips, rows = (1, B * T) if self.rows_out == T else (B, T)
        for b in range(clips):
            ops.colsum(dy, Co, rows, Co, g32, sc.part, x_off=(b * self.rows_out + self.y_off) * Co, out_off=self.b_off)
        ops.gemm(dy, x, sc.dwr_part, M=Co, N=k * Ci, K=T, a_layout=MNMAJOR, lda=Co, a_off=self.y_off * Co, b_layout=MNMAJOR,
                 ldb=self.stride * Ci, ldc=k * Ci, out_f32=True, batch2=B, sA=(0, self.rows_out * Co),
                 sB=(0, self.rows_in * Ci), sC=(0, nw))
        ops.reduce_rows(sc.dwr_part, B, nw, nw, sc.dwr)
        ops.conv_weight_grad_reorder(sc.dwr, g32, Co, Ci, k, dw_off=self.w_off)
        if dx is not None:
            assert self.rows_out == T, "the data gradient reads dy as one [B * T, Co] matrix"
            ops.gemm(dy, self.wr, sc.dcol, M=B * T, N=k * Ci, K=Co, lda=Co, b_layout=MNMAJOR, ldb=k * Ci, ldc=k * Ci)
            ops.col2im_1d(sc.dcol, dx, B, T, self.rows_in, Ci, k, self.stride)


class ConvFeatureEncoder:

    def __init__(self, store, prefix: str, conv_dim, conv_kernel, conv_stride, eps: float, f32: bool):
        assert conv_dim[0] == 512 and conv_kernel[0] == 10, "layer-0 kernel expects C=512,k=10"
        self.st, self.eps, self.f32 = store, eps, f32
        self.dims, self.k0, self.stride0 = tuple(conv_dim), conv_kernel[0], conv_stride[0]
        names = [[f"{prefix}{i}.{n}" for n in ("conv.weight", "conv.bias", "layer_norm.weight", "layer_norm.bias")]
                 for i in range(len(conv_dim))]
        self.p = [[store.view(n) for n in ns] for ns in names]
        self.g = [[store.view(n, "g32") for n in ns] for ns in names]
        self.convs = [None] + [StridedConvBlock(store, names[i][0], names[i][1], conv_dim[i - 1], conv_dim[i], conv_kernel[i],
                                                conv_stride[i]) for i in range(1, len(conv_dim))]

    def refresh(self):
        for c in self.convs[1:]:
            c.refresh()

    def alloc(self, B, Ts, z, part):
        n = [B * T * C for T, C in zip(Ts, self.dims)]
        bf, cdt = torch.bfloat16, F32 if self.f32 else torch.bfloat16
        for i, c in enumerate(self.convs[1:], 1):
            c.set_rows(Ts[i - 1])
        return dict(Ts=Ts, a=[z(m, dt=bf) for m in n[:-1]] + [z(n[-1], dt=cdt)], y=[None] + [z(m, dt=cdt) for m in n[1:]],
                    cstats=[None] + [z(B * T * 2, dt=F32) for T in Ts[1:]], dconv=[z(m) for m in n], dy=z(max(n[1:])),
                    sc=ConvScratch(z, B, self.convs[1:], self.convs[1:], part))

    def forward(self, x, sv, B, N):
        a, y, Ts = sv["a"], sv["y"], sv["Ts"]
        ops.conv0_fwd(x, *self.p[0], a[0], B, N, self.dims[0], self.k0, self.stride0, self.eps)
        for i, c in enumerate(self.convs[1:], 1):
            c.set_rows(Ts[i - 1])
            c.forward(a[i - 1], y[i], B)
            ops.layernorm_fwd(y[i], self.p[i][2], self.p[i][3], a[i], sv["cstats"][i], B * Ts[i], c.Co, self.eps, act=1)
        return a[-1]

    def backward(self, x, sv, B, N):
        dconv, dy, sc, Ts = sv["dconv"], sv["dy"], sv["sc"], sv["Ts"]
        for i in range(len(self.convs) - 1, 0, -1):
            c, (_, _, gamma, beta), (_, _, dgamma, dbeta) = self.convs[i], self.p[i], self.g[i]
            ops.layernorm_bwd(dconv[i], sv["y"][i], gamma, beta, sv["cstats"][i], None, dy, dgamma, dbeta, sc.part,
                              B * Ts[i], c.Co, act=1)
            c.backward(dy, sv["a"][i - 1], B, sc, dx=dconv[i - 1])
        ops.conv0_bwd(x, *self.p[0], dconv[0], *self.g[0], sc.part, B, N, self.dims[0], self.k0, self.stride0, self.eps)


class FeatureProjection:

    def __init__(self, store, prefix: str, C: int, d: int, eps: float):
        self.st, self.C, self.d, self.eps = store, C, d, eps
        ln = prefix + "layer_norm."
        self.gamma, self.beta = store.view(ln + "weight"), store.view(ln + "bias")
        self.dgamma, self.dbeta = store.view(ln + "weight", "g32"), store.view(ln + "bias", "g32")
        self.w_off, self.b_off = store.off(prefix + "projection.weight"), store.off(prefix + "projection.bias")

    def alloc(self, M, z):
        return dict(xln=z(M * self.C), st=z(M * 2, dt=F32))

    def forward(self, x, h0, sv, M, drop=(0.0, 0)):
        st, C, d = self.st, self.C, self.d
        ops.layernorm_fwd(x, self.gamma, self.beta, sv["xln"], sv["st"], M, C, self.eps)
        ops.gemm(sv["xln"], st.p16, h0, M=M, N=d, K=C, lda=C, ldb=C, ldc=d, b_off=self.w_off, bias=st.p32, bias_off=self.b_off)
        if drop[0] > 0:
            ops.dropout(h0, h0, M * d, *drop)

    def backward(self, dh0, x, dxln, dx, sv, M, part, drop=(0.0, 0)):
        st, C, d = self.st, self.C, self.d
        if drop[0] > 0:
            ops.dropout(dh0, dh0, M * d, *drop)
        ops.colsum(dh0, d, M, d, st.g32, part, out_off=self.b_off)
        ops.gemm(dh0, sv["xln"], st.g32, M=d, N=C, K=M, a_layout=MNMAJOR, lda=d, b_layout=MNMAJOR, ldb=C, ldc=C,
                 c_off=self.w_off, out_f32=True, accumulate=True)
        ops.gemm(dh0, st.p16, dxln, M=M, N=C, K=d, lda=d, b_layout=MNMAJOR, ldb=C, ldc=C, b_off=self.w_off)
        ops.layernorm_bwd(dxln, x, self.gamma, None, sv["st"], None, dx, self.dgamma, self.dbeta, part, M, C)


class PosConvEmbed:

    def __init__(self, store, prefix: str, d: int, G: int, K: int):
        self.st, self.d, self.G, self.K, self.Cg = store, d, G, K, d // G
        dev = store.device
        self.wf = torch.zeros(d * K * self.Cg, dtype=torch.bfloat16, device=dev)
        self.wb = torch.zeros(d * K * self.Cg, dtype=torch.bfloat16, device=dev)
        self.norm = torch.zeros(K, dtype=F32, device=dev)
        self.partial = torch.zeros(ops.posconv_partial_floats(K), dtype=F32, device=dev)
        w = prefix + "parametrizations.weight."
        self.v, self.g = store.view(w + "original1"), store.view(w + "original0")
        self.dv, self.dg = store.view(w + "original1", "g32"), store.view(w + "original0", "g32")
        self.b_off = store.off(prefix + "bias")

    def refresh(self):
        ops.posconv_weight(self.v, self.g, self.wf, self.wb, self.norm, self.partial, self.d, self.Cg, self.K)

    def alloc(self, B, T, z):
        n = B * self.G * (T + self.K) * self.Cg + 8 * self.Cg
        return dict(xg=z(n), pc_pre=z(B * T * self.d), dxg=z(n), dwf=z(self.d * self.K * self.Cg, dt=F32))

    def _conv(self, T, Tpad):
        G, K, Cg, d = self.G, self.K, self.Cg, self.d
        return dict(M=T, N=Cg, K=K * Cg, lda=Cg, ldb=K * Cg, ldc=d, ldr=d, batch2=G, sA=(G * Tpad * Cg, Tpad * Cg),
                    sB=(0, Cg * K * Cg), sC=(T * d, Cg), sR=(T * d, Cg))

    def forward(self, h0, h, sv, B, T):
        st, G, K, Cg = self.st, self.G, self.K, self.Cg
        ops.regroup_pad(h0, sv["xg"], B, T, G, Cg, K // 2)
        ops.gemm(sv["xg"], self.wf, sv["pc_pre"], C2=h, R=h0, bias=st.p32, bias_off=self.b_off, epilogue=EPI_GELU_RESIDUAL,
                 batch1=B, sBias=(0, Cg), **self._conv(T, T + K))

    def backward(self, dh, dpc, dh0, sv, B, T, part):
        st, d, G, K, Cg = self.st, self.d, self.G, self.K, self.Cg
        M, Tpad = B * T, T + K
        ops.dgelu_mul(dh, sv["pc_pre"], dpc, M * d)
        ops.colsum(dpc, d, M, d, st.g32, part, out_off=self.b_off)
        ops.gemm(dpc, sv["xg"], sv["dwf"], M=Cg, N=K * Cg, K=M, a_layout=MNMAJOR, lda=d, b_layout=MNMAJOR, ldb=Cg, b_kseg=T,
                 b_kseg_stride=G * Tpad * Cg, ldc=K * Cg, batch2=G, sA=(0, Cg), sB=(0, Tpad * Cg), sC=(0, Cg * K * Cg),
                 out_f32=True)
        ops.posconv_weight_bwd(sv["dwf"], self.v, self.g, self.norm, self.dv, self.dg, self.partial, d, Cg, K)
        ops.regroup_pad(dpc, sv["dxg"], B, T, G, Cg, K // 2)
        ops.gemm(sv["dxg"], self.wb, dh0, a_off=Cg, epilogue=EPI_RESIDUAL, R=dh, batch1=B, **self._conv(T, Tpad))


class LMHead:

    def __init__(self, store, ln: str, weight: str, bias: str | None, d: int, V: int, eps: float):
        self.st, self.d, self.V, self.Vp, self.eps = store, d, V, (V + 7) // 8 * 8, eps
        self.gamma, self.beta = store.view(ln + ".weight"), store.view(ln + ".bias")
        self.dgamma, self.dbeta = store.view(ln + ".weight", "g32"), store.view(ln + ".bias", "g32")
        self.w_off = store.off(weight)
        self.b_off = store.off(bias) if bias is not None else None

    def alloc(self, M, z, train=True):
        return dict(hf=z(M * self.d), st=z(M * 2, dt=F32) if train else None)

    def forward(self, h, sv, M, logits=None, last_of=None, drop=(0.0, 0)):
        d, hf = self.d, sv["hf"]
        ops.layernorm_fwd(h, self.gamma, self.beta, hf, sv["st"], M, d, self.eps)
        if drop[0] > 0:
            ops.dropout(hf, hf, M * d, *drop)
        if last_of is None:
            return self.project(hf, M, logits)
        return self.project(hf.view(last_of, M // last_of, d)[:, -1, :].contiguous(), last_of, logits)

    def project(self, rows, n, logits=None):
        if logits is None:
            logits = torch.empty(n, self.Vp, dtype=F32, device=rows.device)
        d = self.d
        ops.gemm(rows, self.st.p16, logits, M=n, N=self.V, K=d, lda=d, ldb=d, ldc=self.Vp, b_off=self.w_off,
                 bias=None if self.b_off is None else self.st.p32, bias_off=self.b_off or 0)
        return logits

    def backward(self, dl, h, dhf, dh, sv, M, part, freeze=False, drop=(0.0, 0), xdrop=None):
        st, d, V, Vp = self.st, self.d, self.V, self.Vp
        ops.gemm(dl, sv["hf"], st.g32, M=V, N=d, K=M, a_layout=MNMAJOR, lda=Vp, b_layout=MNMAJOR, ldb=d, ldc=d,
                 c_off=self.w_off, out_f32=True, accumulate=True)
        if self.b_off is not None:
            ops.colsum(dl, Vp, M, Vp, st.g32, part, out_off=self.b_off)
        if freeze:
            return
        ops.gemm(dl, st.p16, dhf, M=M, N=d, K=V, lda=Vp, b_layout=MNMAJOR, ldb=d, ldc=d, b_off=self.w_off)
        if drop[0] > 0:
            ops.dropout(dhf, dhf, M * d, *drop)
        layernorm_bwd(dhf, h, self.gamma, sv["st"], None, dh, self.dgamma, self.dbeta, part, M, d, xdrop)
```

### coral_amd/wav2vec2.py

```python

from __future__ import annotations

import math
import os
from dataclasses import dataclass

import torch

from . import ops
from .blocks import FFNBlock, Scratch, SelfAttnBlock, encoder_backward, wgrad_stream
from .engine import Engine
from .staging import PinnedStager
from .stem_blocks import ConvFeatureEncoder, FeatureProjection, LMHead, PosConvEmbed


@dataclass
class Wav2Vec2Shape:

    hidden_size: int = 1024
    num_hidden_layers: int = 24
    num_attention_heads: int = 16
    intermediate_size: int = 4096
    conv_dim: tuple = (512,) * 7
    conv_kernel: tuple = (10, 3, 3, 3, 3, 2, 2)
# ... 190 lines not shown
                           s.layer_norm_eps)
        self.blocks = []
        for l in range(s.num_hidden_layers):
            p = f"wav2vec2.encoder.layers.{l}."
            self.blocks.append((
                SelfAttnBlock(self.store, p + "layer_norm", p + "attention.", s.num_attention_heads, s.hidden_size,
                              s.layer_norm_eps, False, p + "attention.q_proj.bias"),
                FFNBlock(self.store, p + "final_layer_norm", p + "feed_forward.intermediate_dense",
                         p + "feed_forward.output_dense", s.hidden_size, s.intermediate_size, s.layer_norm_eps)))
        self.freeze_base = freeze_base
        self.pack_frames = os.environ.get("CA_PACK_FRAMES", "0") not in ("", "0")
        self.last_rows = 0
        self.last_frames = 0
        self._ws = None
        self._ws_key = None
        self._ctc_key = None
        self._stager = PinnedStager(self.device)
        self._saved = None
        self.zero_embed = torch.zeros(d, dtype=torch.bfloat16, device=self.device)

    def load_state_dict(self, P: dict, strict: bool = True, seed: int = 4242, init_missing: bool = True) -> dict:
        if not strict:
            if not any(k.startswith("wav2vec2.") or k.startswith("lm_head.") for k in P):
                P = {"wav2vec2." + k: v for k, v in P.items()}
            ren = {}
            for k, v in P.items():
                if k.endswith("pos_conv_embed.conv.weight_g"):
                    k = k[:-len("weight_g")] + "parametrizations.weight.original0"
                elif k.endswith("pos_conv_embed.conv.weight_v"):
                    k = k[:-len("weight_v")] + "parametrizations.weight.original1"
                ren[k] = v
            P = ren
        names = self.store.names()
        fresh_ok = ("lm_head.weight", "lm_head.bias", "wav2vec2.masked_spec_embed")
        missing = [n for n in names if n not in P]
        if not strict:
            missing += [n for n in fresh_ok if n in P and int(P[n].numel()) != int(math.prod(self.store.index[n][1]))]
        hard = [n for n in missing if strict or n not in fresh_ok]
        if hard:
            raise KeyError(f"missing parameters: {hard[:4]}...")
        g = torch.Generator(device=self.device).manual_seed(seed)
        for n in names:
            v = self.store.view(n)
            if n in missing:
                if not init_missing:
                    continue
                if n == "lm_head.weight":
                    v.normal_(0.0, 0.02, generator=g)
                elif n == "lm_head.bias":
                    v.zero_()
                else:
                    v.uniform_(0.0, 1.0, generator=g)
                continue
            v.copy_(P[n].to(self.device, torch.float32).reshape(self.store.index[n][1]))
        self.refresh_compute_weights()
        return dict(missing=missing, unexpected=[k for k in P if k not in self.store.index])

    def state_dict(self) -> dict:
        return {n: self.store.view(n).detach().clone() for n in self.store.names()}

    def grad_dict(self) -> dict:
        return {n: self.store.view(n, "g32") for n in self.store.names()}

    def _layer_matrices(self, l: int):
        d, f = self.s.hidden_size, self.s.intermediate_size
        pl = f"wav2vec2.encoder.layers.{l}."
        return [("qkv", pl + "attention.q_proj.weight", 3 * d, d), ("o", pl + "attention.out_proj.weight", d, d),
                ("fc1", pl + "feed_forward.intermediate_dense.weight", f, d),
                ("fc2", pl + "feed_forward.output_dense.weight", d, f)]

    def norm_matrices(self):
        return [(l, *m) for l in range(self.s.num_hidden_layers) for m in self._layer_matrices(l)]

    def shard_ranges(self) -> dict:
        st = self.store
        return {f"layer{l}": (st.off(f"wav2vec2.encoder.layers.{l}.attention.q_proj.weight"), st.buckets[f"layer{l}"][1])
                for l in range(self.s.num_hidden_layers)}

    def bf16_grad_ranges(self) -> dict:
        return self.shard_ranges()

    def zero_grad(self, matrices: bool = True):
        st = self.store
        if matrices:
            st.g32.zero_()
            self.pre_zeroed = False
            return
        if self.pre_zeroed:
            self.pre_zeroed = False
            return
        self.clear_small_grads()

    preclear_small_grads = True

    def clear_small_grads(self):
        st = self.store
        if self._small_ranges is None:
            rs = [(lo, hi - lo) for lo, hi in (st.buckets[n] for n in ("front", "head"))]
            for l in range(self.s.num_hidden_layers):
                lo = st.off(f"wav2vec2.encoder.layers.{l}.layer_norm.weight")
                rs.append((lo, st.off(f"wav2vec2.encoder.layers.{l}.attention.q_proj.weight") - lo))
            self._small_ranges = tuple(rs)
        ops.clear_ranges(st.g32, self._small_ranges)

    def dropout_site(self, site: str, l: int = 0, training: bool | None = None) -> tuple:
        code, key = DROPOUT_SITES[site]
        shape = self.s
        p = float(getattr(shape, key)) if (self.training if training is None else training) else 0.0
        if p <= 0.0:
            return 0.0, 0
        return p, self.step_seed * 1000 + 100 * code + l

    def refresh_compute_weights(self):
        self.store.refresh_bf16()
        self.refresh_derived()

    derived_parts = ("conv", "posconv")

    def refresh_derived(self, part: str | None = None):
        if part in (None, "conv"):
            self.feature_encoder.refresh()
        if part in (None, "posconv"):
            self.pos_conv.refresh()

    def conv_lengths(self, N: int) -> list[int]:
        out, n = [], N
        for k, st in zip(self.s.conv_kernel, self.s.conv_stride):
            n = (n - k) // st + 1
            out.append(n)
        return out

    def feat_lengths(self, sample_lengths: torch.Tensor) -> torch.Tensor:
        n = sample_lengths.clone().long()
        for k, st in zip(self.s.conv_kernel, self.s.conv_stride):
            n = torch.div(n - k, st, rounding_mode="floor") + 1
        return n

    def _workspace(self, B: int, N: int):
        key = (B, N)
        if self._ws_key == key:
            return self._ws
        s, dev = self.s, self.device
        d, f = s.hidden_size, s.intermediate_size
        L = s.num_hidden_layers
        Ts = self.conv_lengths(N)
        T = Ts[-1]
        M = B * T
        bf, f32 = torch.bfloat16, torch.float32

        def build(z):
            w = {"B": B, "N": N, "Ts": Ts, "T": T, "M": M}
            pf = max(
                ops.layernorm_bwd_partial_floats(B * Ts[1], 512), ops.layernorm_bwd_partial_floats(M, d),
                ops.colsum_partial_floats(M, max(f, 3 * d)), ops.colsum_partial_floats(B * Ts[1], 512),
                ops.conv0_bwd_partial_floats(B, N, s.conv_dim[0], s.conv_kernel[0], s.conv_stride[0]), 4096)
            w["partial"] = z(pf, dt=f32)
            w["fe"] = self.feature_encoder.alloc(B, Ts, z, w["partial"])
            w["fp"] = self.feature_projection.alloc(M, z)
            w["h0"] = z(M * d)
            w["pc"] = self.pos_conv.alloc(B, T, z)
            w["h"] = [z(M * d) for _ in range(L + 1)]
            w["hpk"] = z(M * d)
            w["h1"] = [z(M * d) for _ in range(L)]
            w["sv"] = [(sa.alloc(B, T, z), ff.alloc(M, z)) for sa, ff in self.blocks]
            w["head"] = self.head.alloc(M, z)
            Vp = w["Vp"] = self.head.Vp
            w["logits"] = z(M * Vp, dt=f32)
            w["dlogits"] = z(M * Vp, dt=f32)
            w["dlogits16"] = z(M * Vp)
            w["dlogits16p"] = z(M * Vp)
            w["nll"] = z(B, dt=f32)
            w["dA"] = z(M * d)
            w["ring"] = [z(M * d) for _ in range(6)]
            w["mring"] = [z(M * d) for _ in range(6)] if s.hidden_dropout > 0 else None
            w["scs"] = [Scratch(M, d, f, z, masks=False) for _ in range(2)]
            w["bias_ws"] = [z(ops.COLSUM_PARTS * (5 * d + f), dt=f32) for _ in range(2)]
            w["ln_partial"] = [[z(ops.layernorm_bwd_partial_floats(M, d), dt=f32) for _ in range(2)] for _ in range(2)]
            return w

        w = _arena_build(build, dev, bf)
        self._ws, self._ws_key = w, key
        return w

    def __call__(self, input_values, attention_mask=None, labels=None, mask_time=None,
                 mask_feature=None, layer_keep=None):
        return self.forward(input_values, attention_mask, labels, mask_time, mask_feature, layer_keep)

    def forward(self, input_values, attention_mask=None, labels=None, mask_time=None,
                mask_feature=None, layer_keep=None) -> CTCOutput:
        s, st = self.s, self.store
        dev = self.device
        x = self._stager.to_device(input_values, torch.float32, "x")
        B, N = x.shape
        w = self._workspace(B, N)
        d = s.hidden_size
        L = s.num_hidden_layers
        T, M, Vp = w["T"], w["M"], w["Vp"]

        if attention_mask is not None:
            am = self._stager.to_device(attention_mask, torch.int32, "am")
            flen = torch.empty(B, dtype=torch.int32, device=dev)
            ops.frame_lengths(am, s.conv_kernel, s.conv_stride, flen)
        else:
            if w.get("flen_full") is None:
                w["flen_full"] = torch.full((B,), T, dtype=torch.int32, device=dev)
            flen = w["flen_full"]
        keep = [True] * L if layer_keep is None else list(layer_keep)
        w["flen"] = flen
        rows = None
        if self.pack_frames and self.training and labels is not None and attention_mask is not None:
            if attention_mask.device.type == "cpu":
                fl, row_off = frame_row_offsets(attention_mask, s.conv_kernel, s.conv_stride)
            else:
                fl = flen.cpu().to(torch.int64)
                row_off = torch.zeros(B + 1, dtype=torch.int32)
                row_off[1:] = torch.cumsum(fl, 0)
            Mp = int(row_off[B])
            if int(fl.min()) >= 1 and int(fl.max()) <= T and Mp < M:
                rows = (self._stager.to_device(row_off, torch.int32, "row_off"), Mp)
        Me = M if rows is None else rows[1]
        kw_rows = {} if rows is None else dict(rows=rows)
        self.last_rows, self.last_frames = Me, M
        self._await("front")

        feats = self.feature_encoder.forward(x, w["fe"], B, N)
        self.feature_projection.forward(feats, w["h0"], w["fp"], M, self.dropout_site("feat_proj"))
        tm = self._stager.to_device(mask_time, torch.uint8, "tm") if mask_time is not None else None
        fm = self._stager.to_device(mask_feature, torch.uint8, "fm") if mask_feature is not None else None
        ops.mask_frames(w["h0"], tm, fm, st.p16[st.off("wav2vec2.masked_spec_embed"):], flen, B, T, d)
        self._await("front_posconv")
        self.pos_conv.forward(w["h0"], w["h"][0], w["pc"], B, T)
        pa = self.dropout_site("pos_conv")
        if pa[0] > 0:
            ops.dropout(w["h"][0], w["h"][0], M * d, *pa)
        hs = w["h"]
        if rows is not None:
            ops.pack_rows(w["h"][0], w["hpk"], rows[0], B, T, d)
            hs = [w["hpk"]] + w["h"][1:]
        drop_p = s.activation_dropout if self.training else 0.0
        for l, (sa, ff) in enumerate(self.blocks):
            hin, hout = hs[l], hs[l + 1]
            if not keep[l]:
                hout[:Me * d].copy_(hin[:Me * d])
                continue
            self._await(f"layer{l}")
            sv_a, sv_f = w["sv"][l]
            sa.forward(hin, w["h1"][l], sv_a, B, T, klen=flen, hdrop=self.dropout_site("attn_out", l),
                       adrop=self.dropout_site("attention", l), **kw_rows)
            ff.forward(w["h1"][l], hout, sv_f, Me, drop_p, self.step_seed * 1000 + l, hdrop=self.dropout_site("ffn_out", l))
        self._await("head")
        for l in range(L):
            if not keep[l]:
                self._await(f"layer{l}")
        V = s.vocab_size
        self.head.forward(hs[L], w["head"], Me, logits=w["logits"] if rows is None else w["dlogits"],
                          drop=self.dropout_site("final"))
        if rows is not None:
            ops.unpack_rows(w["dlogits"], w["logits"], rows[0], B, T, Vp)
        logits = w["logits"].view(B, T, Vp)[:, :, :V]
        out = CTCOutput(logits=logits, loss=None)
        self._saved = dict(w=w, x=x, flen=flen, keep=keep, tm=tm, fm=fm, B=B, N=N,
                           has_loss=False, training=self.training, rows=rows, hs=hs)
        if labels is not None:
            lab = self._stager.to_device(labels, torch.int32, "lab")
            Lmax = lab.shape[1]
            in_len = flen
            key = (B, T, Lmax)
            if self._ctc_key != key:
                self._ctc_ws = torch.zeros(ops.ctc_workspace_bytes(B, T, Lmax), dtype=torch.uint8, device=dev)
                self._ctc_key = key
            gscale = None
            if s.ctc_loss_reduction == "mean":
                tl = (lab >= 0).sum(-1).clamp(min=1).to(torch.float32)
                gscale = (1.0 / (tl * B)).contiguous()
            ops.ctc_loss_fwd_bwd(w["logits"], lab, in_len, w["nll"], w["dlogits"], gscale, self._ctc_ws,
                                 B, T, V, Vp, Lmax, s.pad_token_id, s.ctc_zero_infinity)
            nll = w["nll"]
            out["nll"] = nll
            out["loss"] = nll.sum() if gscale is None else (nll * gscale).sum()
            self._saved["has_loss"] = True
        return out

    def backward(self, loss_scale: float = 1.0, overwrite_matrices: bool = False, bucket_done=None):
        done = bucket_done if bucket_done is not None else (lambda name: None)
        sv = self._saved
        if sv is None or not sv["has_loss"]:
            raise RuntimeError("backward() needs a forward pass with labels")
        s, st = self.s, self.store
        w, x, flen, keep = sv["w"], sv["x"], sv["flen"], sv["keep"]
        B, N = sv["B"], sv["N"]
        d = s.hidden_size
        L = s.num_hidden_layers
        T, M, Vp = w["T"], w["M"], w["Vp"]
        part = w["partial"]
        lacc = not overwrite_matrices
        self.matrix_grads_bf16 = bool(overwrite_matrices and self.wgrad_bf16)
        gm = st.g16 if self.matrix_grads_bf16 else st.g32

        dl = w["dlogits"]
        if isinstance(loss_scale, torch.Tensor):
            ops.wave_scale(dl, loss_scale.reshape(1).to(torch.float32), dl, 1, M * Vp)
        elif loss_scale != 1.0:
            ops.wave_scale(dl, self._scale_scalar(loss_scale), dl, 1, M * Vp)
        ops.cast_f32_bf16(dl, w["dlogits16"], M * Vp)
        d16 = w["dlogits16"]
        rows, hs = sv["rows"], sv["hs"]
        Me = M if rows is None else rows[1]
# ... 140 lines not shown
```

### coral_amd/whisper_train.py

```python

from __future__ import annotations

import torch

from . import ops
from .staging import PinnedStager
from .blocks import Scratch, _z, encoder_backward, wgrad_stream, zeros_on
from .stem_blocks import ConvScratch
from .whisper import WhisperEngine, WhisperShape, shift_tokens_right


class WhisperTrainEngine(WhisperEngine):

    def __init__(self, shape: WhisperShape, device="cuda:0", activation_dropout: float = 0.0,
                 freeze_base: bool = False, dropout: float = 0.0, attention_dropout: float = 0.0):
        super().__init__(shape, device)
        self.dropout = dropout
        self.attention_dropout = attention_dropout
        self._stager = PinnedStager(self.device)
        self.freeze_base = freeze_base
        self.activation_dropout = activation_dropout
        self.training = True
        self._tw = None
        self._tw_key = None

    _fp8_train = None

    def enable_fp8_forward(self, on: bool = True, ffn2: bool | None = None):
        import os

        self.background_optimizer = not on
        if not on:
            self._fp8_train = None
            return
        st, dev, L = self.store, self.device, self.s.encoder_layers
        if ffn2 is None:
            ffn2 = os.environ.get("CA_FP8_FC2", "1") == "1"
        out8 = os.environ.get("CA_FP8_OUT", "1") == "1"
        dgrad = os.environ.get("CA_FP8_DGRAD", "1") == "1" and ffn2 and out8
        d_, f_ = self.s.d_model, self.s.encoder_ffn_dim
        nw = 4 * L
        na = 3 * L
        f8 = dict(p8=torch.zeros(st.numel, dtype=torch.uint8, device=dev), nw=nw, na=na, ffn2=ffn2, out8=out8,
                  amax=torch.zeros((nw + na) * ops.FP8_AMAX_SLOTS, dtype=torch.int32, device=dev),
                  scale=torch.ones(nw + na, dtype=torch.float32, device=dev),
                  inv=torch.ones(nw + na, dtype=torch.float32, device=dev), x8=None, rs=None, g8=None, c8=None,
                  dgrad=dgrad, dy8=None, drs=None, du8=None, du_ready=[False], bwd_seen=False,
                  dgrad_fc1=dgrad and os.environ.get("CA_FP8_DGRAD_FC1", "1") == "1",
                  p8t=torch.zeros(L * (2 * f_ * d_ + d_ * d_), dtype=torch.uint8, device=dev) if dgrad else None)
        f8["scale"][nw:] = 448.0 / 16.0
        f8["inv"][nw:] = 16.0 / 448.0
        self._fp8_train = f8
        self._tw_key = None
        self.refresh_fp8()
        ops.fp8_amax_rotate(f8["amax"], f8["scale"], f8["inv"], nw, margin=1.0)
        self.refresh_fp8()
        ops.fp8_amax_rotate(f8["amax"], f8["scale"], f8["inv"], nw, margin=1.0)

    def _fp8_weights(self, l: int):
        s = self.s
        d, f = s.d_model, s.encoder_ffn_dim
        p = f"model.encoder.layers.{l}."
        return ((p + "self_attn.q_proj.weight", 3 * d * d), (p + "self_attn.out_proj.weight", d * d), (p + "fc1.weight", f * d),
                (p + "fc2.weight", f * d))

    def refresh_fp8(self, layer: int | None = None):
        f8 = self._fp8_train
        if f8 is None:
            return
        st = self.store
        d, f = self.s.d_model, self.s.encoder_ffn_dim
        S = ops.FP8_AMAX_SLOTS
        shapes = ((3 * d, d), (d, d), (f, d), (d, f))
        for l in (range(self.s.encoder_layers) if layer is None else (layer,)):
            tasks = []
            base = l * (2 * f * d + d * d)
            t_off = {3: base, 1: base + f * d, 2: base + f * d + d * d}
            for k, (name, n) in enumerate(self._fp8_weights(l)):
                if (k == 3 and not f8["ffn2"]) or (k == 1 and not f8["out8"]):
                    continue
                off, i = st.off(name), 4 * l + k
                tr = f8["dgrad"] and (k in (1, 3) or (k == 2 and f8["dgrad_fc1"]))
                rows, cols = shapes[k]
                tasks.append((st.p16, off, rows, cols, f8["p8"], off, f8["p8t"] if tr else None, t_off.get(k, 0),
                              f8["scale"][i:i + 1], f8["amax"][i * S:]))
            ops.fp8_refresh_group(tasks)

    bucket_copies = True

    def refresh_bucket(self, name: str):
        f8 = self._fp8_train
        if f8 is None:
            return
        if name == next(iter(self.store.buckets)):
            nw, L = f8["nw"], self.s.encoder_layers
            S = ops.FP8_AMAX_SLOTS
            ops.fp8_amax_rotate(f8["amax"], f8["scale"], f8["inv"], nw, margin=1.0)
            ops.fp8_amax_rotate(f8["amax"][nw * S:], f8["scale"][nw:], f8["inv"][nw:], 2 * L, margin=2.0)
            ops.fp8_amax_rotate(f8["amax"][(nw + 2 * L) * S:], f8["scale"][nw + 2 * L:], f8["inv"][nw + 2 * L:], L, margin=4.0)
            if f8["bwd_seen"]:
                f8["du_ready"][0] = True
        if name.startswith("enc") and name[3:].isdigit():
            self.refresh_fp8(int(name[3:]))

    def trainable_range(self):
        if not self.freeze_base:
            return 0, self.store.numel
        lo = self.store.off("model.decoder.embed_tokens.weight")
        return lo, lo + self.s.vocab_size * self.s.d_model

    def _enc_matrix_range(self, l: int):
        st = self.store
        p = f"model.encoder.layers.{l}."
        lo = st.off(p + "self_attn.q_proj.weight")
        hi = st.off(p + "fc2.weight") + self.s.d_model * self.s.encoder_ffn_dim
        return lo, hi

    def _dec_matrix_range(self, l: int):
        st = self.store
        return st.off(f"model.decoder.layers.{l}.self_attn.q_proj.weight"), st.buckets[f"dec{l}"][1]

    def shard_ranges(self) -> dict:
        st = self.store
        out = {}
        for l in range(self.s.encoder_layers):
            lo, hi = self._enc_matrix_range(l)
            if hi == st.buckets[f"enc{l}"][1]:
                out[f"enc{l}"] = (lo, hi)
        for l in range(self.s.decoder_layers):
            out[f"dec{l}"] = (st.off(f"model.decoder.layers.{l}.self_attn.q_proj.weight"), st.buckets[f"dec{l}"][1])
        return out

    def bf16_grad_ranges(self) -> dict:
        return {f"enc{l}": self._enc_matrix_range(l) for l in range(self.s.encoder_layers)}

    def _enc_matrices(self, l: int):
        d, f = self.s.d_model, self.s.encoder_ffn_dim
        p = f"model.encoder.layers.{l}."
        return [("qkv", p + "self_attn.q_proj.weight", 3 * d, d), ("o", p + "self_attn.out_proj.weight", d, d),
                ("fc1", p + "fc1.weight", f, d), ("fc2", p + "fc2.weight", d, f)]

    def zero_grad(self, matrices: bool = True):
        st, Le = self.store, self.s.encoder_layers
        if matrices or self.freeze_base or Le == 0:
            st.g32.zero_()
        else:
            if self._small_ranges is None:
                rs, pos = [], 0
                spans = [self._enc_matrix_range(l) for l in range(Le)] + [self._dec_matrix_range(l) for l in range(self.s.decoder_layers)]
                for lo, hi in sorted(spans):
                    rs.append((pos, lo - pos))
                    pos = hi
                rs.append((pos, st.numel - pos))
                self._small_ranges = tuple(r for r in rs if r[1] > 0)
            ops.clear_ranges(st.g32, self._small_ranges)
        if self._norm_plan is not None:
            ops.clear_f32(self._norm_plan["slots"], self._norm_plan["nslots"])

    def norm_matrices(self):
        return [(l, *m) for l in range(self.s.encoder_layers) for m in self._enc_matrices(l)]

    def __call__(self, input_features, labels, mask_time=None, mask_feature=None, enc_keep=None, dec_keep=None):
        from .wav2vec2 import CTCOutput

        out = self.forward_train(input_features, labels, mask_time, mask_feature, enc_keep, dec_keep)
        return CTCOutput(loss=out["loss"], logits=out["logits"])

    def clear_internal_grads(self):
        for n in self.store.names():
            if n.endswith("__zero"):
                self.store.view(n, "g32").zero_()

    def _train_ws(self, B, L):
        key = (B, L)
        if self._tw_key == key:
            return self._tw
        s, dev = self.s, self.device
        d, T = s.d_model, s.max_source_positions
        Tin = 2 * T
        Me, Md = B * T, B * L
        f32 = torch.float32
        z = zeros_on(dev)
        w = dict(
            xin=_z(B * (Tin + 2) * s.num_mel_bins + 64, dev), pre1=_z(B * (Tin + 2) * d + 64, dev),
            c1=_z(B * (Tin + 2) * d + 64, dev), pre2=_z(Me * d, dev),
            eh=[_z(Me * d, dev) for _ in range(2 * s.encoder_layers + 1)], enc_out=_z(Me * d, dev),
            enc_st=_z(Me * 2, dev, f32),
            enc_sv=[(sa.alloc(B, T, z), ff.alloc(Me, z)) for sa, ff in self.enc_blocks],
            dh=[_z(Md * d, dev) for _ in range(3 * s.decoder_layers + 1)], head=self.head.alloc(Md, z),
            dec_sv=[(sa.alloc(B, L, z), ca.alloc(B, L, T, z), ff.alloc(Md, z)) for sa, ca, ff in self.dec_blocks],
            logits=_z(Md * self.head.Vp, dev, f32), dlogits=_z(Md * self.head.Vp, dev, f32),
            dlogits16=_z(Md * self.head.Vp, dev),
            loss_cnt=_z(2, dev, f32),
            sc_e=Scratch(Me, d, s.encoder_ffn_dim, z), sc_d=Scratch(Md, d, s.decoder_ffn_dim, z, Mkv=Me),
            sc_e2=Scratch(Me, d, s.encoder_ffn_dim, z),
            g_e=[_z(Me * d, dev) for _ in range(6)], g_d=[_z(Md * d, dev) for _ in range(4)], dec_bias_ws=_z(ops.COLSUM_PARTS * (9 * d + s.decoder_ffn_dim), dev, f32),
            ln_part_e=[[_z(ops.layernorm_bwd_partial_floats(Me, d), dev, f32) for _ in range(2)] for _ in range(2)],
            ln_part_d=[_z(ops.layernorm_bwd_partial_floats(Md, d), dev, f32) for _ in range(3)],
            bias_ws=_z(ops.COLSUM_PARTS * (5 * d + s.encoder_ffn_dim), dev, f32),
            bias_ws2=_z(ops.COLSUM_PARTS * (5 * d + s.encoder_ffn_dim), dev, f32), denc32=_z(Me * d, dev, f32), dpre=_z(B * (Tin + 2) * d + 64, dev))
        w["conv_sc"] = ConvScratch(z, B, (self.conv1, self.conv2), (self.conv2,), w["sc_e"].part)
        f8 = self._fp8_train
        if f8 is not None:
            Me = B * s.max_source_positions
            f8["x8"] = torch.zeros(Me * s.d_model, dtype=torch.uint8, device=dev)
            f8["rs"] = torch.zeros(Me, dtype=torch.float32, device=dev)
            f8["g8"] = torch.zeros(Me * s.encoder_ffn_dim, dtype=torch.uint8, device=dev) if f8["ffn2"] else None
            f8["c8"] = torch.zeros(Me * s.d_model, dtype=torch.uint8, device=dev) if f8["out8"] else None
            f8["dy8"] = torch.zeros(Me * s.d_model, dtype=torch.uint8, device=dev) if f8["dgrad"] else None
            f8["drs"] = torch.zeros(Me, dtype=torch.float32, device=dev) if f8["dgrad"] else None
            f8["du8"] = torch.zeros(Me * s.encoder_ffn_dim, dtype=torch.uint8, device=dev) if f8["dgrad_fc1"] else None
            nw, S = f8["nw"], ops.FP8_AMAX_SLOTS

            def act(i, buf, w):
                return (buf, f8["scale"][nw + i:nw + i + 1], f8["inv"][nw + i:nw + i + 1], f8["amax"][(nw + i) * S:], f8["inv"][w:w + 1])

            f8["blocks"] = []
            for l in range(s.encoder_layers):
                a8 = dict(w=(f8["p8"], f8["inv"][4 * l:4 * l + 1], f8["x8"], f8["rs"]),
                          out=act(2 * l + 1, f8["c8"], 4 * l + 1) if f8["out8"] else None)
                m8 = dict(w=(f8["p8"], f8["inv"][4 * l + 2:4 * l + 3], f8["x8"], f8["rs"]),
                          fc2=act(2 * l, f8["g8"], 4 * l + 3) if f8["ffn2"] else None)
                if f8["dgrad"]:
                    fd, dd = s.encoder_ffn_dim * s.d_model, s.d_model * s.d_model
                    base = l * (2 * fd + dd)
                    m8["bwd"] = (f8["p8t"], base, f8["dy8"], f8["drs"], f8["inv"][4 * l + 3:4 * l + 4])
                    a8["bwd"] = (f8["p8t"], base + fd, f8["dy8"], f8["drs"], f8["inv"][4 * l + 1:4 * l + 2])
                    if f8["dgrad_fc1"]:
                        i = nw + 2 * s.encoder_layers + l
                        m8["du"] = dict(buf=f8["du8"], scale=f8["scale"][i:i + 1], inv=f8["inv"][i:i + 1], amax=f8["amax"][i * S:],
                                        inv_w=f8["inv"][4 * l + 2:4 * l + 3], w_off=base + fd + dd, ready=f8["du_ready"])
                f8["blocks"].append((a8, m8))
        self._tw, self._tw_key = w, key
        return w

    def forward_train(self, input_features, labels, mask_time=None, mask_feature=None, enc_keep=None, dec_keep=None):
        s, st = self.s, self.store
        dev = self.device
        x = self._stager.to_device(input_features, torch.float32, "x")
        B, mels, Tin = x.shape
        T, d = s.max_source_positions, s.d_model
        if mels != s.num_mel_bins or Tin != 2 * T:
            raise ValueError(f"Whisper expects mel input features of shape [B, {s.num_mel_bins}, {2 * T}]")
        lab = labels.to(torch.int64)
        L = lab.shape[1]
        if L > s.max_target_positions:
            raise ValueError(f"Labels' sequence length {L} cannot exceed the maximum allowed length of {s.max_target_positions} tokens.")
        dec_in = shift_tokens_right(lab, s.pad_token_id, s.decoder_start_token_id)
        w = self._train_ws(B, L)
        Me, Md = B * T, B * L
        drop = self.activation_dropout if self.training else 0.0
        hp = self.dropout if self.training else 0.0
        base = self.step_seed * 4096

        def hd(site):
            return (hp, base + site)

        apd = self.attention_dropout if self.training else 0.0

        def ad(site):
            return (apd, base + site)
        mask_time_d = self._stager.to_device(mask_time, torch.uint8, "tm") if mask_time is not None else None
        mask_feature_d = self._stager.to_device(mask_feature, torch.uint8, "fm") if mask_feature is not None else None
        self._await("front")
        self.encoder_stem(x, w, w["eh"][0], pre=(w["pre1"], w["pre2"]), mask_time=mask_time_d, mask_feature=mask_feature_d)
        if hp > 0.0:
            ops.dropout(w["eh"][0], w["eh"][0], Me * d, *hd(1000))
        ek = [True] * s.encoder_layers if enc_keep is None else [bool(k) for k in enc_keep]
        dk = [True] * s.decoder_layers if dec_keep is None else [bool(k) for k in dec_keep]
        f8 = self._fp8_train
        for l, (sa, ff) in enumerate(self.enc_blocks):
            self._await(f"enc{l}")
            if not ek[l]:
                w["eh"][2 * l + 2].copy_(w["eh"][2 * l])
                continue
            sv_a, sv_f = w["enc_sv"][l]
            a8, m8 = f8["blocks"][l] if f8 is not None else (None, None)
            sa.forward(w["eh"][2 * l], w["eh"][2 * l + 1], sv_a, B, T, hdrop=hd(256 + l), adrop=ad(768 + l), fp8=a8)
            ff.forward(w["eh"][2 * l + 1], w["eh"][2 * l + 2], sv_f, Me, drop, self.step_seed * 4096 + l, hdrop=hd(512 + l),
                       fp8=m8)
        self._await("encf")
        self._await("emb")
        ops.layernorm_fwd(w["eh"][-1], st.view("model.encoder.layer_norm.weight"), st.view("model.encoder.layer_norm.bias"),
                          w["enc_out"], w["enc_st"], Me, d, s.layer_norm_eps)
        ids = self._stager.to_device(dec_in, torch.int32, "ids").view(-1)
        pos = torch.arange(L, dtype=torch.int32, device=dev).repeat(B)
        self._embed(ids, pos, w["dh"][0], Md)
        if hp > 0.0:
            ops.dropout(w["dh"][0], w["dh"][0], Md * d, *hd(3000))
        for l, (sa, ca, ff) in enumerate(self.dec_blocks):
            self._await(f"dec{l}")
            if not dk[l]:
                w["dh"][3 * l + 3].copy_(w["dh"][3 * l])
                continue
            sv_a, sv_c, sv_f = w["dec_sv"][l]
            ca.project_kv(w["enc_out"], sv_c, B, T)
            sa.forward(w["dh"][3 * l], w["dh"][3 * l + 1], sv_a, B, L, hdrop=hd(2304 + l), adrop=ad(3072 + l))
            ca.forward(w["dh"][3 * l + 1], w["dh"][3 * l + 2], sv_c, B, L, T, hdrop=hd(2560 + l), adrop=ad(3328 + l))
            ff.forward(w["dh"][3 * l + 2], w["dh"][3 * l + 3], sv_f, Md, drop, self.step_seed * 4096 + 2048 + l,
                       hdrop=hd(2816 + l))
        self._await_all()
        self.head.forward(w["dh"][-1], w["head"], Md, logits=w["logits"])
        V, Vp = s.vocab_size, self.head.Vp
        ops.clear_ranges(w["loss_cnt"], ((0, 2),))
        w["loss_sum"], w["count"] = w["loss_cnt"][0:1], w["loss_cnt"][1:2].view(torch.int32)
        lab32 = self._stager.to_device(lab, torch.int32, "lab").view(-1)
        ops.cross_entropy_fwd_bwd(w["logits"], lab32, w["loss_sum"], w["count"], w["dlogits"], Md, V, Vp, -100)
        cnt = w["count"].clamp(min=1).to(torch.float32)
        loss = (w["loss_sum"] / cnt)[0]
        self._saved = dict(w=w, B=B, L=L, ids=ids, pos=pos, inv_count=(1.0 / cnt), x=x, ek=ek, dk=dk,
                           embed_drop=(hd(1000), hd(3000)))
        return dict(loss=loss, logits=w["logits"].view(B, L, Vp)[:, :, :V])

    def backward(self, loss_scale: float = 1.0, overwrite_matrices: bool = False, bucket_done=None):
        done = bucket_done if bucket_done is not None else (lambda name: None)
        sv = self._saved
        s, st = self.s, self.store
        w, B, L = sv["w"], sv["B"], sv["L"]
        g32, o = st.g32, st.off
        if self._fp8_train is not None:
            self._fp8_train["bwd_seen"] = True
        T, d = s.max_source_positions, s.d_model
        Tin = 2 * T
        Me, Md = B * T, B * L
        Vp = self.head.Vp
        sc_e, sc_d = w["sc_e"], w["sc_d"]
        w["dlogits"].mul_(sv["inv_count"] * loss_scale)
        ops.cast_f32_bf16(w["dlogits"], w["dlogits16"], Md * Vp)
        dl = w["dlogits16"]
        ga, gb = w["g_d"][:2]
        self.head.backward(dl, w["dh"][-1], ga, gb, w["head"], Md, sc_d.part)
        ops.clear_f32(w["denc32"], w["denc32"].numel())
        ringd, r = w["g_d"], 1
        nbd = 9 * d + s.decoder_ffn_dim
        dacc = not overwrite_matrices
        for l in reversed(range(s.decoder_layers)):
            if not sv["dk"][l]:
                if overwrite_matrices:
                    lo, hi = self._dec_matrix_range(l)
                    g32[lo:hi].zero_()
                done(f"dec{l}")
                continue
            sa, ca, ff = self.dec_blocks[l]
            sv_a, sv_c, sv_f = w["dec_sv"][l]
            g0, g1, g2, g3 = (ringd[(r + i) % 4] for i in range(4))
            wg, second = [], []
            lpd = w["ln_part_d"]
            ff.backward(g0, g1, sv_f, sc_d, Md, defer=wg, acc=dacc, ln_part=lpd[0], pending=second)
            ca.backward(g1, g2, sv_c, sc_d, w["denc32"], B, L, T, defer=wg, cs=ca.cs, ln_part=lpd[1], pending=second, acc=dacc)
            sa.backward(g2, g3, sv_a, sc_d, B, L, defer=wg, acc=dacc, ln_part=lpd[2], pending=second)
            if ops.wgrad_gemm_group(wg, g32, colsum_ws=w["dec_bias_ws"], colsum_ld=nbd):
                second.append((w["dec_bias_ws"], ops.COLSUM_PARTS, nbd, nbd,
                               g32[o(f"model.decoder.layers.{l}.self_attn.q_proj.bias"):], True))
            ops.reduce_rows_multi(second)
            r = (r + 3) % 4
            self.clear_internal_grads_of(f"model.decoder.layers.{l}.")
            done(f"dec{l}")
        cur = ringd[r]
        done("decf")
        (ep, eseed), (dp, dseed) = sv["embed_drop"]
        if dp > 0.0:
            ops.dropout(cur, cur, Md * d, dp, dseed)
        ops.embed_tokens_bwd(cur, sv["ids"], sv["pos"], g32, g32, Md, d, dtable_off=o("model.decoder.embed_tokens.weight"),
                             dpos_off=o("model.decoder.embed_positions.weight"))
        done("emb")
        ring = w["g_e"]
        ea = ring[1]
        ops.cast_f32_bf16(w["denc32"], ea, Me * d)
        ops.layernorm_bwd(ea, w["eh"][-1], st.view("model.encoder.layer_norm.weight"), None, w["enc_st"], None, ring[0],
                          st.view("model.encoder.layer_norm.weight", "g32"), st.view("model.encoder.layer_norm.bias", "g32"),
                          sc_e.part, Me, d)
        xt = lambda m, n: ((m + 255) // 256) * ((n + 255) // 256)
        fe = s.encoder_ffn_dim
        group_tiles = xt(3 * d, d) + xt(d, d) + xt(fe, d) + xt(d, fe)
        plan = self.norm_plan()
        self.matrix_grads_bf16 = bool(overwrite_matrices and self.wgrad_bf16 and plan is not None)
        cur, _, other = encoder_backward(
            self.enc_blocks, w["enc_sv"], sv["ek"], B, T, ring, (sc_e, w["sc_e2"]), (w["bias_ws"], w["bias_ws2"]),
            w["ln_part_e"], gm=st.g16 if self.matrix_grads_bf16 else g32, acc=not overwrite_matrices, plan=plan,
            names=[f"enc{l}" for l in range(s.encoder_layers)], side=wgrad_stream(self) if group_tiles >= 256 else None,
            wgrad_early=False, matrix_range=self._enc_matrix_range, done=done,
            epilogue=lambda l: self.clear_internal_grads_of(f"model.encoder.layers.{l}."))
        done("encf")
        if ep > 0.0:
            ops.dropout(cur, cur, Me * d, ep, eseed)
        dpre2 = other
        ops.dgelu_mul(cur, w["pre2"], dpre2, Me * d)
        self.conv2.backward(dpre2, w["c1"], B, w["conv_sc"], dx=w["dpre"])
        ops.dgelu_mul(w["dpre"], w["pre1"], w["dpre"], B * (Tin + 2) * d)
        self.conv1.backward(w["dpre"], w["xin"], B, w["conv_sc"])
        done("front")

    def clear_internal_grads_of(self, prefix: str):
        cache = self.__dict__.setdefault("_zero_slot_ranges", {})
        rs = cache.get(prefix)
        if rs is None:
            st = self.store
            rs = cache[prefix] = tuple((st.off(n), int(st.view(n).numel())) for n in st.names()
                                       if n.startswith(prefix) and n.endswith("__zero"))
        if rs:
            ops.clear_ranges(self.store.g32, rs)

    def grad_dict(self):
        return {n: self.store.view(n, "g32") for n in self.exported_names()}
```

### include/coral_amd.h

```cpp
#ifndef CORAL_AMD_H
#define CORAL_AMD_H

#include <stdint.h>

#ifdef __cplusplus
extern "C" {
#endif

#define CA_OK 0
#define CA_ERR_ARG (-1)
#define CA_ERR_LAUNCH (-2)
#define CA_ERR_UNSUPPORTED (-3)

int ca_version(void);
const char* ca_last_error(void);
int ca_device_count(void);

#define CA_KMAJOR 0
#define CA_MNMAJOR 1

#define CA_EPI_NONE 0
#define CA_EPI_GELU 1
#define CA_EPI_RESIDUAL 2
#define CA_EPI_DGELU 3
#define CA_EPI_GELU_RESIDUAL 4

typedef struct CaGemmDesc {
  const void* A;
  const void* B;
  void* C;
  void* C2;
  const void* R;
  const float* bias;
  int32_t M, N, K;
  int32_t a_layout, b_layout;
  int64_t lda, ldb, ldc, ldr;
  int32_t a_kseg, b_kseg;
  int64_t a_kseg_stride, b_kseg_stride;
  int32_t batch1, batch2;
  int64_t sA1, sA2, sB1, sB2, sC1, sC2, sR1, sR2;
  int64_t sBias1, sBias2;
  int32_t epilogue;
  int32_t out_f32;
  int32_t accumulate;
  float alpha;
  float dropout_p;
  uint64_t dropout_seed;
  float* a_colsum;
  int64_t a_colsum_ld;
  const int32_t* c_row_index;
  int64_t c_row_mul;
  int32_t c_split_n;
  void* C_hi;
  int64_t ldc_hi;
  const float* a_scale;
  const float* b_scale;
  const float* a_row_scale;
  float* c_sumsq;
  int32_t c_stream_out;
  void* C8;
  const float* c8_scale;
  uint32_t* c8_amax;
  const float* a_ln_gamma;
  const float* a_ln_beta;
  float a_ln_eps;
  int32_t xcd_balanced;
} CaGemmDesc;

int ca_gemm_bf16(const CaGemmDesc* desc, void* stream);
int ca_gemm_fp8(const CaGemmDesc* desc, void* stream);
int ca_quantize_fp8(const void* x_bf16, int64_t n, void* q_fp8, float* inv_scale, float* amax_ws, void* stream);
#define CA_FP8_AMAX_SLOTS 64
int ca_quantize_fp8_delayed(const void* x_bf16, int64_t n, void* q_fp8, const float* scale, uint32_t* amax_next,
                            void* stream);
int ca_fp8_amax_rotate(uint32_t* amax_next, float* scale, float* inv_scale, int32_t count, float margin, void* stream);
int ca_dropout_rows_fp8(const void* x, void* y, void* q_fp8, float* row_scale, int64_t rows, int32_t C, float p,
                        uint64_t seed, void* stream);
int ca_quantize_fp8_transposed(const void* x_bf16, int32_t rows, int32_t cols, void* q_fp8_t, const float* scale,
                               void* stream);
#define CA_FP8_GROUP_MAX 8
typedef struct CaFp8RefreshTask {
  const void* x_bf16;
  void* q_fp8;
  void* q_fp8_t;
  const float* scale;
  uint32_t* amax_next;
  int32_t rows, cols;
} CaFp8RefreshTask;
int ca_fp8_refresh_group(const CaFp8RefreshTask* tasks, int32_t count, void* stream);
int ca_gemm_bf16_group(const CaGemmDesc* descs, int32_t count, void* stream);

int ca_prof_begin(void);
int ca_prof_end(double* ms, int64_t* count, double* flops);

int ca_gemm_force_kernel(int which);
int ca_gemm_debug_general_epilogue(int on);
int ca_debug_cu_hog(int32_t blocks, int32_t threads, int32_t lds_bytes, double ms, void* stream);

int ca_gemm_set_compute_cus(int n);

int ca_layernorm_fwd(const void* x, const float* gamma, const float* beta, void* y,
                     float* stats, int64_t rows, int32_t C, float eps, int32_t act,
                     void* stream);
int ca_layernorm_fwd_ex(const void* x, const float* gamma, const float* beta, void* y,
                        float* stats, int64_t rows, int32_t C, float eps, int32_t act,
                        int32_t x_f32, int32_t y_f32, void* stream);
int ca_layernorm_fwd_fp8(const void* x, const float* gamma, const float* beta, void* y, void* q_fp8,
                         float* row_scale, float* stats, int64_t rows, int32_t C, float eps, void* stream);
int64_t ca_layernorm_bwd_partial_floats(int64_t rows, int32_t C);
int ca_layernorm_bwd(const void* dy, const void* x, const float* gamma, const float* beta,
                     const float* stats, const void* dres, void* dx, float* dgamma,
                     float* dbeta, float* partial, int64_t rows, int32_t C, int32_t act,
                     void* stream);

int ca_layernorm_bwd_ex(const void* dy, const void* x, const float* gamma, const float* beta,
                        const float* stats, const void* dres, void* dx, float* dgamma,
                        float* dbeta, float* partial, int64_t rows, int32_t C, int32_t act,
                        int32_t x_f32, void* stream);

int ca_layernorm_bwd_dropout(const void* dy, const void* x, const float* gamma, const float* beta,
                             const float* stats, const void* dres, void* dx, void* dx_drop, float p, uint64_t seed,
                             float* dgamma, float* dbeta, float* partial, int64_t rows, int32_t C, int32_t x_f32,
                             void* stream);

int64_t ca_colsum_partial_floats(int64_t rows, int32_t N);
int ca_colsum_bf16(const void* x, int64_t ld, int64_t rows, int32_t N, const uint8_t* rowmask,
                   float* out, int32_t accumulate, float* partial, void* stream);
int ca_reduce_rows_f32(const float* partial, int32_t nparts, int64_t stride, int32_t n, float* out,
                       int32_t accumulate, void* stream);
#define CA_REDUCE_MAX 4
typedef struct CaReduceDesc {
  const float* partial;
  float* out;
  int64_t stride;
  int32_t nparts, n, accumulate;
} CaReduceDesc;
int ca_reduce_rows_multi(const CaReduceDesc* descs, int32_t count, void* stream);
int ca_dgelu_mul(const void* dy, const void* u, void* out, int64_t n, void* stream);
int ca_dropout_bf16(const void* x, void* y, int64_t n, float p, uint64_t seed, void* stream);

int ca_wave_normalize(const float* x, const int32_t* lengths, float* y, int32_t B,
                      int64_t N, float eps, void* stream);

int ca_frame_lengths(const int32_t* attention_mask, int32_t B, int64_t N, const int32_t* kernels,
                     const int32_t* strides, int32_t nconv, int32_t* out, void* stream);
int ca_pcm_prepare(const void* pcm, int32_t is_int16, int64_t ld_in, const int32_t* lengths, float* y,
                   int32_t* mask, int32_t B, int64_t N, int32_t peak_normalize, int32_t zero_mean_unit_var,
                   float eps, void* stream);
int ca_wave_scale(const float* x, const float* scale, float* y, int32_t B, int64_t N, void* stream);
int ca_fir_filter(const float* x, const int32_t* lengths, const float* taps, const int32_t* ntaps,
                  const int32_t* mode, int64_t ld_taps, int32_t max_taps, float* y, int32_t B, int64_t N,
                  void* stream);
int ca_mix_noise(const float* x, const int32_t* lengths, const float* noise, int64_t noise_ld, int64_t noise_len,
                 const int64_t* noise_off, const float* snr_db, const int32_t* active, float* y, int32_t B,
                 int64_t N, void* stream);
int ca_white_noise(float* out, int64_t n, uint64_t seed, void* stream);

int ca_conv0_ln_gelu_fwd(const float* x, const float* w, const float* bias,
                         const float* gamma, const float* beta, void* y, int32_t B,
                         int64_t N, int32_t C, int32_t k, int32_t stride, float eps,
                         void* stream);
int64_t ca_conv0_bwd_partial_floats(int32_t B, int64_t N, int32_t C, int32_t k,
                                    int32_t stride);
int ca_conv0_ln_gelu_bwd(const float* x, const float* w, const float* bias,
                         const float* gamma, const float* beta, const void* dy, float* dw,
                         float* dbias, float* dgamma, float* dbeta, float* partial,
                         int32_t B, int64_t N, int32_t C, int32_t k, int32_t stride,
                         float eps, void* stream);

int ca_col2im_1d(const void* dcol, void* dx, int32_t B, int64_t T, int64_t L, int32_t C,
                 int32_t k, int32_t stride, void* stream);

typedef struct CaAttnDesc {
  const void *Q, *K, *V;
  void* O;
  const void* dO;
  void *dQ, *dK, *dV;
  float* lse;
  float* Dq;
  const int32_t* klen;
  const int32_t* key_slot;
  const int32_t* kstart;
  int64_t ldq, ldk, ldv, ldo, lddo, lddq, lddk, lddv;
  int64_t sqb, skb, svb, sob, sdob, sdqb, sdkb, sdvb;
  int32_t B, H, Tq, Tk, hd, Tqp, causal;
  float scale;
  float dropout_p;
  uint64_t dropout_seed;
  void* O8;
  const float* o8_scale;
  uint32_t* o8_amax;
  void* split_ws;
  int64_t split_ws_bytes;
  const int32_t* row_off;
} CaAttnDesc;
#define CA_ATTN_SPLIT_MAX 4
#define CA_ATTN_SPLIT_WS_BYTES(B, H) \
  ((((int64_t)(B) * (H) * 4 + 255) / 256 * 256) + (int64_t)(B) * (H) * CA_ATTN_SPLIT_MAX * 16 * 66 * 4)
int ca_attn_fwd(const CaAttnDesc* desc, void* stream);
int ca_attn_bwd(const CaAttnDesc* desc, void* stream);
int ca_decode_attn_qproj(const CaAttnDesc* desc, const void* x, int64_t ldx, const float* ln_gamma,
                         const float* ln_beta, float ln_eps, const void* Wq, int64_t ldw, const float* bq,
                         int32_t d_model, void* stream);

#define CA_BEAM_MAX_BEAMS 16
#define CA_BEAM_MAX_ROWS 128
typedef struct CaBeamDesc {
  int32_t B, k, max_len, prompt_len, max_length, eos_id, early_stopping;
  const float* len_pen;
  const float* cand_score;
  const int32_t* cand_parent;
  const int32_t* cand_token;
  float* run_score;
  int32_t *tok, *pos, *klen;
  const int32_t* anc_in;
  int32_t* anc_out;
  const int32_t* ids_in;
  int32_t* ids_out;
  float* fin_score;
  int32_t *fin_len, *fin_seq;
  int32_t* fin_ids;
  int32_t* fin_count;
  int32_t* heur;
  uint8_t* done;
  int32_t *tr_parent, *tr_token;
  float* tr_score;
} CaBeamDesc;
int64_t ca_beam_select_workspace_bytes(int32_t B, int32_t k, int32_t V);
int ca_beam_select(const float* logits, int64_t ldv, const uint8_t* suppress, const float* run_score, int32_t B,
                   int32_t k, int32_t V, float* cand_score, int32_t* cand_parent, int32_t* cand_token, void* ws,
                   int64_t ws_bytes, void* stream);
int ca_beam_advance(const CaBeamDesc* desc, void* stream);

int64_t ca_ctc_workspace_bytes(int32_t B, int32_t T, int32_t Lmax);
int ca_ctc_loss_fwd_bwd(const float* logits, const int32_t* labels, const int32_t* in_len,
                        float* nll, float* grad, const float* gscale, void* ws, int32_t B,
                        int32_t T, int32_t V, int64_t ldv, int32_t Lmax, int32_t blank,
                        int32_t zero_infinity, void* stream);
int ca_ctc_greedy_decode(const float* logits, const int32_t* in_len, int32_t* raw,
                         int32_t* ids, int32_t* out_len, int32_t B, int32_t T, int32_t V,
                         int64_t ldv, int32_t blank, void* stream);

#define CA_CTC_COLLAPSE_TILE 4096
int ca_ctc_stitch(const float* logits, const int32_t* seg, int32_t* raw_out, float* logits_out, int32_t C, int32_t T,
                  int32_t V, int64_t ldv, int32_t R, int32_t Tout, void* stream);
int64_t ca_ctc_collapse_workspace_bytes(int32_t B, int32_t T);
int ca_ctc_collapse_offsets(const int32_t* raw, const int32_t* in_len, int32_t* ids, int32_t* start, int32_t* end,
                            int32_t* out_len, void* ws, int64_t ws_bytes, int32_t B, int32_t T, int32_t blank,
                            void* stream);

typedef struct CaCtcBeamDesc {
  const float* logits;
  int64_t ldv;
  const int32_t* in_len;
  int32_t B, T, V, blank, delimiter;
  const uint8_t* forbidden;
  const uint64_t* pfx_keys;
  const int32_t* pfx_wid;
  int64_t n_pfx;
  const uint64_t* ng_keys;
  const float* ng_logp;
  const float* ng_backoff;
  int64_t ng_count[5];
  int32_t order, bos_wid, eos_wid, unk_wid;
  int32_t beam_width;
  float alpha, beta, unk_score_offset, token_min_logp, beam_prune_logp;
  int32_t score_boundary;
  int32_t* ids_out;
  int32_t* out_len;
  float* score_out;
  void* ws;
  int64_t ws_bytes;
} CaCtcBeamDesc;
int64_t ca_ctc_beam_workspace_bytes(int32_t B, int32_t T, int32_t V, int32_t beam_width);
int ca_ctc_beam_decode(const CaCtcBeamDesc* desc, void* stream);

#define CA_CTC_ALIGN_MAX_LABELS 4095
int64_t ca_ctc_align_workspace_bytes(int32_t B, int32_t T, int32_t Lmax);
int ca_ctc_align(const float* logits, int64_t ldv, const int32_t* in_len, const int32_t* labels,
                 const int32_t* lab_len, int32_t* start, int32_t* end, float* tok_score, float* score, void* ws,
                 int64_t ws_bytes, int32_t B, int32_t T, int32_t V, int32_t Lmax, int32_t blank, void* stream);

int ca_mask_frames(void* h, const uint8_t* tmask, const uint8_t* fmask, const void* embed,
                   const int32_t* flen, int32_t B, int32_t T, int32_t C, void* stream);
int ca_regroup_pad(const void* x, void* xg, int32_t B, int32_t T, int32_t G, int32_t Cg,
                   int32_t pad, void* stream);
int64_t ca_posconv_partial_floats(int32_t K);
int ca_posconv_weight(const float* v, const float* g, void* wf, void* wb, float* norm,
                      float* partial, int32_t d, int32_t Cg, int32_t K, void* stream);
int ca_posconv_weight_bwd(const float* dwf, const float* v, const float* g,
                          const float* norm, float* dv, float* dg, float* partial, int32_t d,
                          int32_t Cg, int32_t K, void* stream);

int ca_pack_rows(const void* x, void* y, const int32_t* row_off, int32_t B, int32_t T, int32_t C, int32_t elt_bytes,
                 void* stream);
int ca_unpack_rows(const void* x, void* y, const int32_t* row_off, int32_t B, int32_t T, int32_t C, int32_t elt_bytes,
                   void* stream);

int ca_cast_f32_bf16(const float* x, void* y, int64_t n, void* stream);
int ca_cast_bf16_f32(const void* x, float* y, int64_t n, void* stream);
int ca_transpose_f32_bf16(const float* x, void* y, int32_t rows, int32_t cols, void* stream);
int ca_conv_weight_reorder(const float* w, void* wr, int32_t Co, int32_t Ci, int32_t k,
                           void* stream);
int ca_conv_weight_grad_reorder(const float* dwr, float* dw, int32_t Co, int32_t Ci,
                                int32_t k, void* stream);

int ca_sumsq_f32(const float* g, int64_t n, float* out, int32_t accumulate, float* partial,
                 void* stream);
int ca_clear_ranges(void* base, const int64_t* ranges_bytes, int32_t nranges, int64_t max_bytes, void* stream);
int ca_sumsq_ranges_f32(const float* g, const int64_t* chunks, int32_t nchunks, float* out, int32_t accumulate,
                        float* partial, void* stream);
int ca_sum_f32(const float* x, int64_t n, float* out, int32_t accumulate, float* partial, void* stream);
int ca_adamw_step(float* p, float* m, float* v, const float* g, void* p16, int64_t n,
                  float lr, float beta1, float beta2, float eps, float weight_decay,
                  int32_t step, float grad_scale, float max_norm, const float* gnorm_sq,
                  void* stream);
int ca_adamw_step_ex(float* p, float* m, float* v, const float* g, void* p16, int64_t n,
                     float lr, float beta1, float beta2, float eps, float weight_decay,
                     int32_t step, float grad_scale, float max_norm, const float* gnorm_sq,
                     int32_t max_blocks, void* stream);
int ca_adamw_step_g16(float* p, float* m, float* v, const void* g_bf16, void* p16, int64_t n,
// ... 117 lines not shown
```

Measured before the change: 1112 audio-seconds/sec.

## Compute strided conv data gradient via polyphase GEMMs writing dx directly

Replaces the im2col-style data-gradient GEMM followed by col2im scatter with a polyphase decomposition. The weights are pre-split into stride phases, and the LN/GELU backward writes dy into a padded per-clip layout so each phase is a plain GEMM that writes dx directly. This removes the large dcol intermediate buffer and the col2im pass in the conv feature encoder backward, at the cost of more GEMM launches, an extra weight-phase reorder at refresh, and padded dy buffers.

```diff
diff --git a/coral_amd/_lib.py b/coral_amd/_lib.py
--- a/coral_amd/_lib.py
+++ b/coral_amd/_lib.py
@@ -194,6 +194,10 @@
         C.c_int,
         [_vp, _vp, _vp, _vp, _vp, _vp, _vp, _vp, _vp, _vp, _i64, _i32, _i32, _i32, _vp],
     ),
+    "ca_layernorm_bwd_pitch": (
+        C.c_int,
+        [_vp, _vp, _vp, _vp, _vp, _vp, _vp, _vp, _vp, _i64, _i32, _i32, _i32, _i32, _i32, _vp],
+    ),
     "ca_layernorm_bwd_dropout": (
         C.c_int,
         [_vp, _vp, _vp, _vp, _vp, _vp, _vp, _vp, _f32, _u64, _vp, _vp, _vp, _i64, _i32, _i32, _vp],
@@ -207,6 +211,7 @@
     "ca_colsum_partial_floats": (_i64, [_i64, _i32]),
     "ca_colsum_bf16": (C.c_int, [_vp, _i64, _i64, _i32, _vp, _vp, _i32, _vp, _vp]),
     "ca_dgelu_mul": (C.c_int, [_vp, _vp, _vp, _i64, _vp]),
+    "ca_dgelu_mul_pitch": (C.c_int, [_vp, _vp, _vp, _i64, _i32, _i32, _i32, _i32, _vp]),
     "ca_dropout_bf16": (C.c_int, [_vp, _vp, _i64, _f32, _u64, _vp]),
     "ca_reduce_rows_f32": (C.c_int, [_vp, _i32, _i64, _i32, _vp, _i32, _vp]),
     "ca_reduce_rows_multi": (C.c_int, [C.POINTER(CaReduceDesc), _i32, _vp]),
@@ -226,6 +231,7 @@
         C.c_int,
         [_vp] * 11 + [_i32, _i64, _i32, _i32, _i32, _f32, _vp],
     ),
+    "ca_conv_weight_phases": (C.c_int, [_vp, _vp, _i32, _i32, _i32, _i32, _vp]),
     "ca_col2im_1d": (C.c_int, [_vp, _vp, _i32, _i64, _i64, _i32, _i32, _i32, _vp]),
     "ca_ctc_workspace_bytes": (_i64, [_i32, _i32, _i32]),
     "ca_ctc_loss_fwd_bwd": (
diff --git a/coral_amd/csrc/misc.hip b/coral_amd/csrc/misc.hip
--- a/coral_amd/csrc/misc.hip
+++ b/coral_amd/csrc/misc.hip
@@ -378,6 +378,32 @@
   hipLaunchKernelGGL(conv_w_reorder_kernel, dim3(ew_grid(n, 1)), dim3(256), 0,
                      (hipStream_t)stream, w, (unsigned short*)wr, n, Ci, k);
   CA_CHECK_LAUNCH("ca_conv_weight_reorder");
+  return CA_OK;
+}
+__global__ void conv_w_phase_kernel(const float* __restrict__ w, unsigned short* __restrict__ wp,
+                                    int64_t n, int Co, int Ci, int k, int stride) {
+  for (int64_t i = (int64_t)blockIdx.x * blockDim.x + threadIdx.x; i < n;
+       i += (int64_t)gridDim.x * blockDim.x) {
+    int64_t e = i;
+    int r = 0, nr = (k + stride - 1) / stride;
+    while (e >= (int64_t)Ci * nr * Co) {
+      e -= (int64_t)Ci * nr * Co;
+      ++r;
+      nr = (k - r + stride - 1) / stride;
+    }
+    const int ci = (int)(e / ((int64_t)nr * Co));
+    const int c = (int)(e % ((int64_t)nr * Co));
+    const int j = r + stride * (nr - 1 - c / Co);
+    wp[i] = f2bf(w[((int64_t)(c % Co) * Ci + ci) * k + j]);
+  }
+}
+extern "C" int ca_conv_weight_phases(const float* w, void* wp, int32_t Co, int32_t Ci, int32_t k, int32_t stride,
+                                     void* stream) {
+  CA_CHECK_ARG(w && wp && Co > 0 && Ci > 0 && stride > 0 && k >= stride, "ca_conv_weight_phases: bad argument");
+  const int64_t n = (int64_t)Co * Ci * k;
+  hipLaunchKernelGGL(conv_w_phase_kernel, dim3(ew_grid(n, 1)), dim3(256), 0,
+                     (hipStream_t)stream, w, (unsigned short*)wp, n, Co, Ci, k, stride);
+  CA_CHECK_LAUNCH("ca_conv_weight_phases");
   return CA_OK;
 }
 __global__ void conv_w_grad_reorder_kernel(const float* __restrict__ dwr, float* __restrict__ dw,
diff --git a/coral_amd/csrc/norm.hip b/coral_amd/csrc/norm.hip
--- a/coral_amd/csrc/norm.hip
+++ b/coral_amd/csrc/norm.hip
@@ -299,7 +299,7 @@
     const float* __restrict__ gamma, const float* __restrict__ beta,
     const float* __restrict__ stats, const unsigned short* __restrict__ dres,
     unsigned short* __restrict__ dx, float* __restrict__ partial, int64_t rows, int C,
-    unsigned short* __restrict__ dxd, float drop_p, uint64_t drop_seed) {
+    unsigned short* __restrict__ dxd, float drop_p, uint64_t drop_seed, int clip_rows, int out_pitch, int out_first) {
   extern __shared__ __attribute__((aligned(16))) char smem_raw[];
   float* red = (float*)smem_raw;
   const int lane = threadIdx.x & 63;
@@ -394,7 +394,12 @@
     }
     const float m1 = (DPP ? wave_sum_dpp(s1) : wave_sum(s1)) / (float)C;
     const float m2 = (DPP ? wave_sum_dpp(s2) : wave_sum(s2)) / (float)C;
-    unsigned short* dxr = dx + row * C;
+    int64_t orow = row;
+    if (ACT && out_pitch) {
+      const unsigned b = (unsigned)row / (unsigned)clip_rows;
+      orow = (int64_t)b * out_pitch + out_first + ((unsigned)row - b * (unsigned)clip_rows);
+    }
+    unsigned short* dxr = dx + orow * C;
 #pragma unroll
     for (int c = 0; c < NCH; ++c) {
       const int ch = lane + c * 64;
@@ -531,8 +536,11 @@
 static int ln_bwd_launch(const void* dy, const void* x, const float* gamma, const float* beta, const float* stats,
                          const void* dres, void* dx, void* dxd, float drop_p, uint64_t drop_seed, float* dgamma,
                          float* dbeta, float* partial, int64_t rows, int32_t C, int32_t act, int32_t x_f32,
-                         void* stream) {
+                         void* stream, int32_t clip_rows = 0, int32_t out_pitch = 0, int32_t out_first = 0) {
   CA_CHECK_ARG(dy && x && gamma && stats && dx && partial, "ca_layernorm_bwd: null pointer");
+  CA_CHECK_ARG(out_pitch == 0 || (act && !dres && clip_rows > 0 && out_first >= 0 && out_first + clip_rows <= out_pitch &&
+                                  rows % clip_rows == 0 && rows < ((int64_t)1 << 31)),
+               "ca_layernorm_bwd_pitch: the conv form (act, no dres), rows = clips x clip_rows, first_row + clip_rows <= rows_per_clip");
   CA_CHECK_ARG(!x_f32 || C <= 1024, "ca_layernorm_bwd_ex: fp32 rows are served up to C = 1024 (C=%d)", C);
   CA_CHECK_ARG(!act || beta, "ca_layernorm_bwd: act needs beta");
   CA_CHECK_ARG(rows > 0 && C > 0 && (C % 8) == 0 && C <= LN_MAXCH * 512,
@@ -547,11 +555,13 @@
     if (x_f32 && N <= 2)                                                                              \
       hipLaunchKernelGGL((ln_bwd_kernel<(N <= 2 ? N : 1), A, D, true, R>), grid, block, lds, s,       \
                          (const unsigned short*)dy, x, gamma, beta, stats, (const unsigned short*)dres, \
-                         (unsigned short*)dx, partial, rows, C, (unsigned short*)dxd, drop_p, drop_seed); \
+                         (unsigned short*)dx, partial, rows, C, (unsigned short*)dxd, drop_p, drop_seed, \
+                         clip_rows, out_pitch, out_first);                                            \
     else                                                                                              \
       hipLaunchKernelGGL((ln_bwd_kernel<N, A, D, false, R>), grid, block, lds, s,                     \
                          (const unsigned short*)dy, x, gamma, beta, stats, (const unsigned short*)dres, \
-                         (unsigned short*)dx, partial, rows, C, (unsigned short*)dxd, drop_p, drop_seed); \
+                         (unsigned short*)dx, partial, rows, C, (unsigned short*)dxd, drop_p, drop_seed, \
+                         clip_rows, out_pitch, out_first);                                            \
   } while (0)
   static const int use_dpp = [] { const char* e = getenv("CA_LN_BWD_DPP"); return e ? atoi(e) : 1; }();
 #define LN_BWD(N)                          \
@@ -593,6 +603,13 @@
   return ln_bwd_launch(dy, x, gamma, beta, stats, dres, dx, nullptr, 0.f, 0, dgamma, dbeta, partial, rows, C, act, x_f32,
                        stream);
 }
+extern "C" int ca_layernorm_bwd_pitch(const void* dy, const void* x, const float* gamma, const float* beta,
+                                      const float* stats, void* dx, float* dgamma, float* dbeta, float* partial,
+                                      int64_t rows, int32_t C, int32_t x_f32, int32_t clip_rows, int32_t rows_per_clip,
+                                      int32_t first_row, void* stream) {
+  return ln_bwd_launch(dy, x, gamma, beta, stats, nullptr, dx, nullptr, 0.f, 0, dgamma, dbeta, partial, rows, C, 1, x_f32,
+                       stream, clip_rows, rows_per_clip, first_row);
+}
 extern "C" int ca_layernorm_bwd(const void* dy, const void* x, const float* gamma,
                                 const float* beta, const float* stats, const void* dres,
                                 void* dx, float* dgamma, float* dbeta, float* partial,
@@ -684,7 +701,8 @@
 
 __global__ void dgelu_mul_kernel(const unsigned short* __restrict__ dy,
                                  const unsigned short* __restrict__ u,
-                                 unsigned short* __restrict__ out, int64_t n8) {
+                                 unsigned short* __restrict__ out, int64_t n8, int64_t clip8, int64_t pitch8,
+                                 int64_t first8) {
   for (int64_t i = (int64_t)blockIdx.x * blockDim.x + threadIdx.x; i < n8;
        i += (int64_t)gridDim.x * blockDim.x) {
     const u16x8_t a = *(const u16x8_t*)(dy + i * 8);
@@ -692,18 +710,32 @@
     u16x8_t o;
 #pragma unroll
     for (int e = 0; e < 8; ++e) o[e] = f2bf(bf2f(a[e]) * dgelu_erf(bf2f(b[e])));
-    *(u16x8_t*)(out + i * 8) = o;
-  }
-}
-extern "C" int ca_dgelu_mul(const void* dy, const void* u, void* out, int64_t n, void* stream) {
-  CA_CHECK_ARG(dy && u && out && n > 0 && (n % 8) == 0, "ca_dgelu_mul: n must be a multiple of 8");
+    const int64_t j = clip8 ? (i / clip8) * pitch8 + first8 + i % clip8 : i;
+    *(u16x8_t*)(out + j * 8) = o;
+  }
+}
+static int dgelu_mul_launch(const void* dy, const void* u, void* out, int64_t n, int64_t clip8, int64_t pitch8,
+                            int64_t first8, void* stream) {
   int64_t g = (n / 8 + 255) / 256;
   if (g > 8192) g = 8192;
   hipLaunchKernelGGL(dgelu_mul_kernel, dim3((int)g), dim3(256), 0, (hipStream_t)stream,
                      (const unsigned short*)dy, (const unsigned short*)u, (unsigned short*)out,
-                     n / 8);
+                     n / 8, clip8, pitch8, first8);
   CA_CHECK_LAUNCH("ca_dgelu_mul");
   return CA_OK;
+}
+extern "C" int ca_dgelu_mul(const void* dy, const void* u, void* out, int64_t n, void* stream) {
+  CA_CHECK_ARG(dy && u && out && n > 0 && (n % 8) == 0, "ca_dgelu_mul: n must be a multiple of 8");
+  return dgelu_mul_launch(dy, u, out, n, 0, 0, 0, stream);
+}
+extern "C" int ca_dgelu_mul_pitch(const void* dy, const void* u, void* out, int64_t rows, int32_t C, int32_t clip_rows,
+                                  int32_t rows_per_clip, int32_t first_row, void* stream) {
+  CA_CHECK_ARG(dy && u && out && out != dy && out != u && rows > 0 && C > 0 && (C % 8) == 0 && clip_rows > 0 &&
+                   rows % clip_rows == 0 && first_row >= 0 && first_row + clip_rows <= rows_per_clip,
+               "ca_dgelu_mul_pitch: rows = clips x clip_rows of C (a multiple of 8) elements, first_row + clip_rows <= rows_per_clip, "
+               "out its own buffer");
+  const int64_t c8 = C / 8;
+  return dgelu_mul_launch(dy, u, out, rows * C, clip_rows * c8, rows_per_clip * c8, first_row * c8, stream);
 }
 
 __global__ void dropout_bf16_kernel(const unsigned short* __restrict__ x, unsigned short* __restrict__ y, int64_t n8,
diff --git a/coral_amd/ops.py b/coral_amd/ops.py
--- a/coral_amd/ops.py
+++ b/coral_amd/ops.py
@@ -335,7 +335,13 @@
     return lib().ca_layernorm_bwd_partial_floats(rows, Cn)
 
 
-def layernorm_bwd(dy, x, gamma, beta, stats, dres, dx, dgamma, dbeta, partial, rows, Cn, act=0):
+def layernorm_bwd(dy, x, gamma, beta, stats, dres, dx, dgamma, dbeta, partial, rows, Cn, act=0, out_rows=None):
+    if out_rows is not None:
+        assert act == 1 and dres is None
+        check(lib().ca_layernorm_bwd_pitch(_p(dy), _p(x), _p(gamma), _p(beta), _p(stats), _p(dx), _p(dgamma), _p(dbeta),
+                                           _p(partial), rows, Cn, int(x.dtype == torch.float32), *out_rows, _stream()),
+              "ca_layernorm_bwd_pitch")
+        return
     if x.dtype == torch.float32:
         check(lib().ca_layernorm_bwd_ex(_p(dy), _p(x), _p(gamma), _p(beta), _p(stats), _p(dres), _p(dx), _p(dgamma),
                                         _p(dbeta), _p(partial), rows, Cn, act, 1, _stream()), "ca_layernorm_bwd_ex")
@@ -375,7 +381,10 @@
     check(lib().ca_reduce_rows_multi(arr, len(items), _stream()), "ca_reduce_rows_multi")
 
 
-def dgelu_mul(dy, u, out, n):
+def dgelu_mul(dy, u, out, n, Cn=None, out_rows=None):
+    if out_rows is not None:
+        check(lib().ca_dgelu_mul_pitch(_p(dy), _p(u), _p(out), n // Cn, Cn, *out_rows, _stream()), "ca_dgelu_mul_pitch")
+        return
     check(lib().ca_dgelu_mul(_p(dy), _p(u), _p(out), n, _stream()), "ca_dgelu_mul")
 
 
@@ -573,6 +582,10 @@
           "ca_conv_weight_reorder")
 
 
+def conv_weight_phases(w, wp, Co, Ci, k, stride, w_off=0):
+    check(lib().ca_conv_weight_phases(_p(w, w_off), _p(wp), Co, Ci, k, stride, _stream()), "ca_conv_weight_phases")
+
+
 def conv_weight_grad_reorder(dwr, dw, Co, Ci, k, dw_off=0):
     check(lib().ca_conv_weight_grad_reorder(_p(dwr), _p(dw, dw_off), Co, Ci, k, _stream()),
           "ca_conv_weight_grad_reorder")
diff --git a/coral_amd/stem_blocks.py b/coral_amd/stem_blocks.py
--- a/coral_amd/stem_blocks.py
+++ b/coral_amd/stem_blocks.py
@@ -1,5 +1,7 @@
 
 from __future__ import annotations
+
+import os
 
 import torch
 
@@ -8,6 +10,7 @@
 from .ops import EPI_GELU_RESIDUAL, EPI_RESIDUAL, MNMAJOR
 
 F32 = torch.float32
+DGRAD_COL = os.environ.get("CA_CONV_DGRAD_COL", "0") == "1"
 
 
 class ConvScratch:
@@ -15,8 +18,33 @@
     def __init__(self, z, B, wgrad, dgrad, part):
         nw = max(c.Co * c.k * c.Ci for c in wgrad)
         self.dwr_part, self.dwr = z(B * nw, F32), z(nw, F32)
-        self.dcol = z(max(B * c.T * c.k * c.Ci for c in dgrad))
+        self.dcol = z(max(B * c.T * c.k * c.Ci for c in dgrad)) if dgrad else None
         self.part = part
+
+
+def conv_phases(k, stride, Ci, Co):
+    out, off = [], 0
+    for r in range(stride):
+        n = -(-(k - r) // stride)
+        out.append((r, n, off))
+        off += Ci * n * Co
+    return out
+
+
+def conv_dy_layout(k, stride, rows_in):
+    front = -(-k // stride) - 1
+    return front + -(-rows_in // stride), front
+
+
+def conv_dgrad_gemms(Ci, Co, k, stride, rows_in, B, rows, off):
+    s, R = stride, rows_in
+    T = (R - k) // s + 1
+    per_clip = dict(batch2=B, sA=(0, rows * Co), sC=(0, R * Ci))
+    if k == s:
+        return [dict(M=m, N=n, K=Co, lda=Co, a_off=(off + q0) * Co, b_layout=MNMAJOR, ldb=k * Ci, ldc=k * Ci,
+                     c_off=q0 * k * Ci, **per_clip) for q0, m, n in ((0, T, k * Ci), (T, 1, (R - s * T) * Ci)) if n], False
+    return [dict(M=-(-(R - r) // s), N=Ci, K=n * Co, lda=Co, a_off=(off - n + 1) * Co, ldb=n * Co, b_off=w_off,
+                 ldc=s * Ci, c_off=r * Ci, **per_clip) for r, n, w_off in conv_phases(k, s, Ci, Co)], True
 
 
 class StridedConvBlock:
@@ -26,6 +54,7 @@
         self.st, self.Ci, self.Co, self.k, self.stride, self.y_off = store, Ci, Co, k, stride, y_off
         self.w_off, self.b_off = store.off(weight), store.off(bias)
         self.wr = torch.zeros(Co * k * Ci, dtype=torch.bfloat16, device=store.device)
+        self.wp = torch.zeros(Co * k * Ci, dtype=torch.bfloat16, device=store.device) if k > stride else None
         if rows_in is not None:
             self.set_rows(rows_in, rows_out)
 
@@ -37,6 +66,11 @@
 
     def refresh(self):
         ops.conv_weight_reorder(self.st.p32, self.wr, self.Co, self.Ci, self.k, w_off=self.w_off)
+        if self.wp is not None:
+            ops.conv_weight_phases(self.st.p32, self.wp, self.Co, self.Ci, self.k, self.stride, w_off=self.w_off)
+
+    def dy_layout(self):
+        return conv_dy_layout(self.k, self.stride, self.rows_in)
 
     def forward(self, x, y, B, **epilogue):
         Ci, Co, k = self.Ci, self.Co, self.k
@@ -44,21 +78,37 @@
                  bias=self.st.p32, bias_off=self.b_off, batch2=B, sA=(0, self.rows_in * Ci), sC=(0, self.rows_out * Co),
                  **epilogue)
 
-    def backward(self, dy, x, B, sc: ConvScratch, dx=None):
+    def backward(self, dy, x, B, sc: ConvScratch, dx=None, dy_layout=None):
         Ci, Co, k, T = self.Ci, self.Co, self.k, self.T
         g32, nw = self.st.g32, Co * k * Ci
-        clips, rows = (1, B * T) if self.rows_out == T else (B, T)
-        for b in range(clips):
-            ops.colsum(dy, Co, rows, Co, g32, sc.part, x_off=(b * self.rows_out + self.y_off) * Co, out_off=self.b_off)
-        ops.gemm(dy, x, sc.dwr_part, M=Co, N=k * Ci, K=T, a_layout=MNMAJOR, lda=Co, a_off=self.y_off * Co, b_layout=MNMAJOR,
-                 ldb=self.stride * Ci, ldc=k * Ci, out_f32=True, batch2=B, sA=(0, self.rows_out * Co),
+        rows, off = (self.rows_out, self.y_off) if dy_layout is None else dy_layout
+        assert off + T <= rows
+        if rows == T or dy_layout is not None:
+            ops.colsum(dy, Co, B * rows, Co, g32, sc.part, out_off=self.b_off)
+        else:
+            for b in range(B):
+                ops.colsum(dy, Co, T, Co, g32, sc.part, x_off=(b * rows + off) * Co, out_off=self.b_off)
+        ops.gemm(dy, x, sc.dwr_part, M=Co, N=k * Ci, K=T, a_layout=MNMAJOR, lda=Co, a_off=off * Co, b_layout=MNMAJOR,
+                 ldb=self.stride * Ci, ldc=k * Ci, out_f32=True, batch2=B, sA=(0, rows * Co),
                  sB=(0, self.rows_in * Ci), sC=(0, nw))
         ops.reduce_rows(sc.dwr_part, B, nw, nw, sc.dwr)
         ops.conv_weight_grad_reorder(sc.dwr, g32, Co, Ci, k, dw_off=self.w_off)
-        if dx is not None:
-            assert self.rows_out == T, "the data gradient reads dy as one [B * T, Co] matrix"
-            ops.gemm(dy, self.wr, sc.dcol, M=B * T, N=k * Ci, K=Co, lda=Co, b_layout=MNMAJOR, ldb=k * Ci, ldc=k * Ci)
+        if dx is None:
+            return
+        need = self.dy_layout()
+        if DGRAD_COL or k < self.stride or dy_layout is None or off < need[1] or rows - off < need[0] - need[1]:
+            assert sc.dcol is not None, "this ConvScratch was built without the im2col-layout buffer"
+            if rows == T:
+                ops.gemm(dy, self.wr, sc.dcol, M=B * T, N=k * Ci, K=Co, lda=Co, b_layout=MNMAJOR, ldb=k * Ci, ldc=k * Ci)
+            else:
+                assert dy_layout is not None, "the data gradient reads dy as one [B * T, Co] matrix"
+                ops.gemm(dy, self.wr, sc.dcol, M=T, N=k * Ci, K=Co, lda=Co, a_off=off * Co, b_layout=MNMAJOR, ldb=k * Ci,
+                         ldc=k * Ci, batch2=B, sA=(0, rows * Co), sC=(0, T * k * Ci))
             ops.col2im_1d(sc.dcol, dx, B, T, self.rows_in, Ci, k, self.stride)
+            return
+        gemms, phased = conv_dgrad_gemms(Ci, Co, k, self.stride, self.rows_in, B, rows, off)
+        for kw in gemms:
+            ops.gemm(dy, self.wp if phased else self.wr, dx, **kw)
 
 
 class ConvFeatureEncoder:
@@ -83,9 +133,14 @@
         bf, cdt = torch.bfloat16, F32 if self.f32 else torch.bfloat16
         for i, c in enumerate(self.convs[1:], 1):
             c.set_rows(Ts[i - 1])
+        col = [c for c in self.convs[1:] if DGRAD_COL or c.k < c.stride]
+        dys = [None if c is None or c in col else z(B * c.dy_layout()[0] * c.Co) for c in self.convs]
         return dict(Ts=Ts, a=[z(m, dt=bf) for m in n[:-1]] + [z(n[-1], dt=cdt)], y=[None] + [z(m, dt=cdt) for m in n[1:]],
-                    cstats=[None] + [z(B * T * 2, dt=F32) for T in Ts[1:]], dconv=[z(m) for m in n], dy=z(max(n[1:])),
-                    sc=ConvScratch(z, B, self.convs[1:], self.convs[1:], part))
+                    cstats=[None] + [z(B * T * 2, dt=F32) for T in Ts[1:]], dconv=[z(m) for m in n],
+                    dy=z(max(n[1:]) if col else n[-1]), dys=dys, sc=ConvScratch(z, B, self.convs[1:], col, part))
+
+    def colsum_rows(self, B, Ts):
+        return max(B * max(Ts[i], conv_dy_layout(c.k, c.stride, Ts[i - 1])[0]) for i, c in enumerate(self.convs[1:], 1))
 
     def forward(self, x, sv, B, N):
         a, y, Ts = sv["a"], sv["y"], sv["Ts"]
@@ -97,12 +152,14 @@
         return a[-1]
 
     def backward(self, x, sv, B, N):
-        dconv, dy, sc, Ts = sv["dconv"], sv["dy"], sv["sc"], sv["Ts"]
+        dconv, sc, Ts = sv["dconv"], sv["sc"], sv["Ts"]
         for i in range(len(self.convs) - 1, 0, -1):
             c, (_, _, gamma, beta), (_, _, dgamma, dbeta) = self.convs[i], self.p[i], self.g[i]
+            c.set_rows(Ts[i - 1])
+            dy, lay = (sv["dy"], None) if sv["dys"][i] is None else (sv["dys"][i], c.dy_layout())
             ops.layernorm_bwd(dconv[i], sv["y"][i], gamma, beta, sv["cstats"][i], None, dy, dgamma, dbeta, sc.part,
-                              B * Ts[i], c.Co, act=1)
-            c.backward(dy, sv["a"][i - 1], B, sc, dx=dconv[i - 1])
+                              B * Ts[i], c.Co, act=1, out_rows=None if lay is None else (Ts[i], *lay))
+            c.backward(dy, sv["a"][i - 1], B, sc, dx=dconv[i - 1], dy_layout=lay)
         ops.conv0_bwd(x, *self.p[0], dconv[0], *self.g[0], sc.part, B, N, self.dims[0], self.k0, self.stride0, self.eps)
 
 
diff --git a/coral_amd/wav2vec2.py b/coral_amd/wav2vec2.py
--- a/coral_amd/wav2vec2.py
+++ b/coral_amd/wav2vec2.py
@@ -366,7 +366,8 @@
             w = {"B": B, "N": N, "Ts": Ts, "T": T, "M": M}
             pf = max(
                 ops.layernorm_bwd_partial_floats(B * Ts[1], 512), ops.layernorm_bwd_partial_floats(M, d),
-                ops.colsum_partial_floats(M, max(f, 3 * d)), ops.colsum_partial_floats(B * Ts[1], 512),
+                ops.colsum_partial_floats(M, max(f, 3 * d)),
+                ops.colsum_partial_floats(self.feature_encoder.colsum_rows(B, Ts), 512),
                 ops.conv0_bwd_partial_floats(B, N, s.conv_dim[0], s.conv_kernel[0], s.conv_stride[0]), 4096)
             w["partial"] = z(pf, dt=f32)
             w["fe"] = self.feature_encoder.alloc(B, Ts, z, w["partial"])
diff --git a/coral_amd/whisper_train.py b/coral_amd/whisper_train.py
--- a/coral_amd/whisper_train.py
+++ b/coral_amd/whisper_train.py
@@ -6,6 +6,7 @@
 from . import ops
 from .staging import PinnedStager
 from .blocks import Scratch, _z, encoder_backward, wgrad_stream, zeros_on
+from . import stem_blocks
 from .stem_blocks import ConvScratch
 from .whisper import WhisperEngine, WhisperShape, shift_tokens_right
 
@@ -199,7 +200,9 @@
             ln_part_d=[_z(ops.layernorm_bwd_partial_floats(Md, d), dev, f32) for _ in range(3)],
             bias_ws=_z(ops.COLSUM_PARTS * (5 * d + s.encoder_ffn_dim), dev, f32),
             bias_ws2=_z(ops.COLSUM_PARTS * (5 * d + s.encoder_ffn_dim), dev, f32), denc32=_z(Me * d, dev, f32), dpre=_z(B * (Tin + 2) * d + 64, dev))
-        w["conv_sc"] = ConvScratch(z, B, (self.conv1, self.conv2), (self.conv2,), w["sc_e"].part)
+        col = (self.conv2,) if stem_blocks.DGRAD_COL else ()
+        w["conv_sc"] = ConvScratch(z, B, (self.conv1, self.conv2), col, w["sc_e"].part)
+        w["dpre2"] = None if col else z(B * self.conv2.dy_layout()[0] * s.d_model)
         f8 = self._fp8_train
         if f8 is not None:
             Me = B * s.max_source_positions
@@ -384,9 +387,13 @@
         done("encf")
         if ep > 0.0:
             ops.dropout(cur, cur, Me * d, ep, eseed)
-        dpre2 = other
-        ops.dgelu_mul(cur, w["pre2"], dpre2, Me * d)
-        self.conv2.backward(dpre2, w["c1"], B, w["conv_sc"], dx=w["dpre"])
+        if w["dpre2"] is None:
+            dpre2, lay = other, None
+            ops.dgelu_mul(cur, w["pre2"], dpre2, Me * d)
+        else:
+            dpre2, lay = w["dpre2"], self.conv2.dy_layout()
+            ops.dgelu_mul(cur, w["pre2"], dpre2, Me * d, Cn=d, out_rows=(self.conv2.T, *lay))
+        self.conv2.backward(dpre2, w["c1"], B, w["conv_sc"], dx=w["dpre"], dy_layout=lay)
         ops.dgelu_mul(w["dpre"], w["pre1"], w["dpre"], B * (Tin + 2) * d)
         self.conv1.backward(w["dpre"], w["xin"], B, w["conv_sc"])
         done("front")
diff --git a/include/coral_amd.h b/include/coral_amd.h
--- a/include/coral_amd.h
+++ b/include/coral_amd.h
@@ -118,6 +118,11 @@
                         float* dbeta, float* partial, int64_t rows, int32_t C, int32_t act,
                         int32_t x_f32, void* stream);
 
+int ca_layernorm_bwd_pitch(const void* dy, const void* x, const float* gamma, const float* beta,
+                           const float* stats, void* dx, float* dgamma, float* dbeta, float* partial,
+                           int64_t rows, int32_t C, int32_t x_f32, int32_t clip_rows, int32_t rows_per_clip,
+                           int32_t first_row, void* stream);
+
 int ca_layernorm_bwd_dropout(const void* dy, const void* x, const float* gamma, const float* beta,
                              const float* stats, const void* dres, void* dx, void* dx_drop, float p, uint64_t seed,
                              float* dgamma, float* dbeta, float* partial, int64_t rows, int32_t C, int32_t x_f32,
@@ -137,6 +142,8 @@
 } CaReduceDesc;
 int ca_reduce_rows_multi(const CaReduceDesc* descs, int32_t count, void* stream);
 int ca_dgelu_mul(const void* dy, const void* u, void* out, int64_t n, void* stream);
+int ca_dgelu_mul_pitch(const void* dy, const void* u, void* out, int64_t rows, int32_t C, int32_t clip_rows,
+                       int32_t rows_per_clip, int32_t first_row, void* stream);
 int ca_dropout_bf16(const void* x, void* y, int64_t n, float p, uint64_t seed, void* stream);
 
 int ca_wave_normalize(const float* x, const int32_t* lengths, float* y, int32_t B,
@@ -167,6 +174,8 @@
                          float* dbias, float* dgamma, float* dbeta, float* partial,
                          int32_t B, int64_t N, int32_t C, int32_t k, int32_t stride,
                          float eps, void* stream);
+
+int ca_conv_weight_phases(const float* w, void* wp, int32_t Co, int32_t Ci, int32_t k, int32_t stride, void* stream);
 
 int ca_col2im_1d(const void* dcol, void* dx, int32_t B, int64_t T, int64_t L, int32_t C,
                  int32_t k, int32_t stride, void* stream);
```

Result: no change. 1115 audio-seconds/sec, median of 6 (+0.3%).
